# Intelligent-Microsystems-Lab/SNNQuantPrune

Measured on AMD Instinct MI355X. Metric: samples/sec/node (DVS128 T=20, 4-bit/90%-pruned), higher is better.
Workload: dtype fp6*fp4->f32 (integer-exact); 1 GPU; C3 topology: 3x(qconv3x3+BN+LIF+pool2) + qdense(32768->110)+LIF + vote, DVS128 128x128x2, T=20, bits 4/4/4/4, 90% pruned; batch_per_gpu=1024, global_batch=1024, frames=20, parallelism=dp1 (batch-sharded, all-gather logits)

## Files before the change

include/snnqp.h:

```cpp
#ifndef SNNQP_H_
#define SNNQP_H_

#include <stdint.h>

#ifdef __cplusplus
extern "C" {
#endif

typedef void *snnqp_stream_t;

enum {
  SNNQP_OK = 0,
  SNNQP_EINVAL = -1,
  SNNQP_EUNSUPPORTED = -2,
  SNNQP_EHIP = -3
};

enum { SNNQP_F32 = 0, SNNQP_U8 = 1, SNNQP_BITS = 2, SNNQP_EV1 = 3, SNNQP_EV4 = 4 };
enum { SNNQP_W_F32 = 0, SNNQP_W_I8 = 1 };
enum {
  SNNQP_NEURON_NONE = 0,
  SNNQP_NEURON_MULTI_STEP_LIF = 1,
  SNNQP_NEURON_PARAMETRIC_LEAKY_IF = 2,
  SNNQP_NEURON_LIF = 3
};
enum {
  SNNQP_SURR_FAST_SIGMOID = 0,
  SNNQP_SURR_ATAN = 1,
  SNNQP_SURR_SLAYER = 2,
  SNNQP_SURR_SMOOTH_STEP = 3,
  SNNQP_SURR_PIECEWISE_LINEAR = 4
};
enum {
  SNNQP_Q_DUQ = 0,
  SNNQP_Q_UNIFORM_STATIC = 1,
  SNNQP_Q_PARAMETRIC_D = 2,
  SNNQP_Q_PARAMETRIC_D_XMAX = 3
};
enum { SNNQP_IMPL_AUTO = 0, SNNQP_IMPL_GENERIC = 1, SNNQP_IMPL_MFMA = 2 };

enum {
  SNNQP_FLAG_CODE_OVERFLOW = 1,
  SNNQP_FLAG_MASK_NOT_BINARY = 2,
  SNNQP_FLAG_NOT_INTEGER = 4,
  SNNQP_FLAG_GT_ONE = 8,
  SNNQP_FLAG_GT_127 = 16,
  SNNQP_FLAG_GT_15 = 32
};

typedef struct {
  int32_t wtype;
  const void *w;
  float L;
  float m;
  int32_t abs_sum_max;
  int32_t code_max;
  const int32_t *col_sum;
  const void *wt_fp6;
  uint32_t min_current_bits;
  int32_t ch_stack_max;
  const int32_t *ch_slots;
  int32_t wt_cin;
} snnqp_weight_t;

#define SNNQP_BN_MEAN_ZERO 1
#define SNNQP_BN_BIAS_ZERO 2
#define SNNQP_BN_MUL_UNIFORM 4
typedef struct {
  const float *mean;
  const float *mul;
  const float *bias;
  int32_t flags;
} snnqp_bn_t;

typedef struct {
  int32_t kind;
  float k;
  float v_threshold;
  float v_reset;
  const float *decay;
} snnqp_neuron_t;

typedef struct {
  int32_t H, W, Cin, Cout;
  int32_t KH, KW;
  int32_t stride_h, stride_w;
  int32_t pad_h_lo, pad_h_hi, pad_w_lo, pad_w_hi;
  int32_t in_dil_h, in_dil_w;
  int32_t k_dil_h, k_dil_w;
  int32_t groups;
} snnqp_conv_geom_t;

typedef struct {
  int32_t D, H, W, Cin, Cout;
  int32_t KD, KH, KW;
  int32_t stride[3];
  int32_t pad_lo[3], pad_hi[3];
  int32_t in_dil[3];
  int32_t k_dil[3];
  int32_t groups;
} snnqp_conv3d_geom_t;

#define SNNQP_VERSION 505
int snnqp_version(void);
const char *snnqp_last_error(void);
const char *snnqp_build_flags(void);

int snnqp_conv_out_shape(const snnqp_conv_geom_t *g, int32_t *OH, int32_t *OW);

int snnqp_quantize(int kind, const float *w, const float *mask, int64_t n,
                   int bits, float p0, float p1, float *fq_out,
                   int8_t *codes_out, int32_t *flags, snnqp_stream_t stream);
int snnqp_quantize_ex(int kind, const float *w, const float *mask, int64_t n,
                      int bits, int sign, float p0, float p1, float *fq_out,
                      int8_t *codes_out, int32_t *flags, snnqp_stream_t stream);

int snnqp_pack_codes_mfma(const int8_t *w, int64_t K, int32_t N, int32_t Npad,
                          int8_t *wt, snnqp_stream_t stream);

int snnqp_pack_codes_fp6(const int8_t *w, int64_t K, int32_t N, int32_t Npad, void *wt6,
                         snnqp_stream_t stream);

int snnqp_inspect_f32(const float *x, int64_t n, int32_t *flags,
                      snnqp_stream_t stream);
int snnqp_inspect_u8(const uint8_t *x, int64_t n, int32_t *flags,
                     snnqp_stream_t stream);
int snnqp_f32_to_u8(const float *x, uint8_t *y, int64_t n,
                    snnqp_stream_t stream);
int snnqp_narrow_f32(const float *x, uint8_t *y, int64_t n, int32_t *flags,
                     snnqp_stream_t stream);
int snnqp_pack_frames(const uint8_t *x, int64_t frames, int32_t H, int32_t W, int fmt,
                      void *y, int32_t *flags, snnqp_stream_t stream);
int snnqp_unpack_frames(const void *x, int fmt, int64_t frames, int32_t H, int32_t W,
                        uint8_t *y, snnqp_stream_t stream);
int snnqp_pack_frames_checked(const void *x, int in_type, int64_t frames, int32_t H, int32_t W,
                              uint32_t *y, int32_t *flags, snnqp_stream_t stream);
int snnqp_pack_bits(const void *x, int in_type, int64_t rows, int32_t C,
                    uint32_t *bits, snnqp_stream_t stream);
int snnqp_pack_bits_checked(const void *x, int in_type, int64_t rows, int32_t C,
                            uint32_t *bits, int32_t *flags, snnqp_stream_t stream);
int snnqp_unpack_bits(const uint32_t *bits, int64_t rows, int32_t C, float *y,
                      snnqp_stream_t stream);

int snnqp_conv_forward(const void *x, int in_type, int64_t NB,
                       const snnqp_conv_geom_t *g, const snnqp_weight_t *w,
                       float *y, int32_t *acc, snnqp_stream_t stream);
int snnqp_conv_forward_if(const int32_t *pred, const void *x, int in_type, int64_t NB,
                          const snnqp_conv_geom_t *g, const snnqp_weight_t *w, float *y,
                          snnqp_stream_t stream);

int snnqp_conv3d_out_shape(const snnqp_conv3d_geom_t *g, int32_t *OD, int32_t *OH, int32_t *OW);
int snnqp_conv3d_lif_forward(const int32_t *pred, const void *x, int in_type, int64_t x_stride_t,
                             int64_t x_stride_b, int32_t T, int32_t B,
                             const snnqp_conv3d_geom_t *g, const snnqp_weight_t *w,
                             const snnqp_bn_t *bn, const snnqp_neuron_t *nrn, const float *u0,
                             float *u_out, void *s_out, int s_type, snnqp_stream_t stream);

int64_t snnqp_conv_gated_packed_bytes(int32_t Cin, int32_t Cout);
int snnqp_pack_codes_gated(const int8_t *w, int32_t Cin, int32_t Cout, void *packed,
                           snnqp_stream_t stream);
int64_t snnqp_conv_gated_packed_bytes_ex(int32_t Cin, int32_t Cout, int32_t code_max);
int snnqp_pack_codes_gated_ex(const int8_t *w, int32_t Cin, int32_t Cout, int32_t code_max,
                              void *packed, snnqp_stream_t stream);
int snnqp_conv_gated_forward(const uint32_t *s, const float *gate, int64_t NB,
                             const snnqp_conv_geom_t *g, const snnqp_weight_t *w,
                             const void *packed, float *y, snnqp_stream_t stream);

int64_t snnqp_dense_gated_packed_bytes(int32_t C, int32_t N);
int snnqp_pack_codes_dense_gated(const int8_t *w, int32_t C, int32_t HW, int32_t N, void *packed,
                                 snnqp_stream_t stream);
int64_t snnqp_dense_gated_packed_bytes_ex(int32_t C, int32_t N, int32_t code_max);
int snnqp_pack_codes_dense_gated_ex(const int8_t *w, int32_t C, int32_t HW, int32_t N, int32_t code_max,
                                    void *packed, snnqp_stream_t stream);
int snnqp_dense_gated_forward(const uint32_t *s, const float *gate, int64_t NB, int32_t HW,
                              int32_t C, int32_t N, const snnqp_weight_t *w,
                              const void *packed, float *y, snnqp_stream_t stream);

int snnqp_conv_lif_forward(const void *x, int in_type, int64_t x_stride_t,
                           int64_t x_stride_b, int32_t T, int32_t B,
                           const snnqp_conv_geom_t *g, const snnqp_weight_t *w,
                           const int8_t *wt, const snnqp_bn_t *bn,
                           const snnqp_neuron_t *nrn, const float *u0,
                           float *u_out, void *s_out, int s_type, int pool,
                           int impl, int x_max, int32_t *x_seen, int32_t *x_flags,
                           snnqp_stream_t stream);

int snnqp_conv_lif_forward_pred(const int32_t *pred, const void *x, int in_type, int64_t x_stride_t,
                                int64_t x_stride_b, int32_t T, int32_t B,
                                const snnqp_conv_geom_t *g, const snnqp_weight_t *w,
                                const int8_t *wt, const snnqp_bn_t *bn,
                                const snnqp_neuron_t *nrn, const float *u0,
                                float *u_out, void *s_out, int s_type, int pool,
                                int x_max, int32_t *x_seen, int32_t *x_flags,
                                snnqp_stream_t stream);

int snnqp_conv_lif_forward_if(const int32_t *pred, const void *x, int in_type, int64_t x_stride_t,
                              int64_t x_stride_b, int32_t T, int32_t B,
                              const snnqp_conv_geom_t *g, const snnqp_weight_t *w,
                              const snnqp_bn_t *bn, const snnqp_neuron_t *nrn, const float *u0,
                              float *u_out, void *s_out, int s_type, int pool,
                              snnqp_stream_t stream);

int snnqp_fallback_counts(int64_t *conv_blocks, int64_t *dense_blocks, char *reason,
                          int32_t reason_len, int reset);

#define SNNQP_STATUS_QUEUE_CORRUPT 1u
#define SNNQP_STATUS_TICKET 2u
#define SNNQP_STATUS_BOUND 4u
int snnqp_device_status(int device, uint32_t *codes, int reset);
int snnqp_workqueue_capture_mark(int device, int64_t *mark);
int snnqp_workqueue_capture_release(int device, int64_t mark_begin, int64_t mark_end);
int snnqp_workqueue_stats(int64_t *captured_static, int64_t *busy_static,
                          int64_t *dequant_fallbacks, int reset);
int snnqp_debug_workqueue_poke(int device, int64_t mark, int word, uint32_t value);

#define SNNQP_DQ_ARITH 1
#define SNNQP_DQ_ONE 2
#define SNNQP_DQ_TABLE 3
int snnqp_conv_dequant_form(const snnqp_weight_t *w, const snnqp_neuron_t *nrn);

int snnqp_current_min(const snnqp_weight_t *w, const snnqp_bn_t *bn, int32_t bound,
                      int32_t Cout, uint32_t *out_bits, snnqp_stream_t stream);

int snnqp_dense_lif_forward(const void *x, int in_type, int64_t x_stride_t,
                            int64_t x_stride_b, int32_t T, int32_t B, int32_t K,
                            int32_t N, const snnqp_weight_t *w,
                            const int8_t *wt, const snnqp_bn_t *bn,
                            const snnqp_neuron_t *nrn, const float *u0,
                            float *u_out, void *s_out, int s_type, int impl,
                            snnqp_stream_t stream);

int64_t snnqp_dense_workspace_bytes(int in_type, int32_t T, int32_t B, int32_t K, int32_t N,
                                    const snnqp_weight_t *w);
int snnqp_dense_lif_forward_ws(const void *x, int in_type, int64_t x_stride_t,
                               int64_t x_stride_b, int32_t T, int32_t B, int32_t K,
                               int32_t N, const snnqp_weight_t *w,
                               const int8_t *wt, const snnqp_bn_t *bn,
                               const snnqp_neuron_t *nrn, const float *u0,
                               float *u_out, void *s_out, int s_type, int impl,
                               int32_t *x_flags, void *ws, int64_t ws_bytes, snnqp_stream_t stream);
int snnqp_dense_lif_forward_if(const int32_t *pred, const void *x, int in_type, int64_t x_stride_t,
                               int64_t x_stride_b, int32_t T, int32_t B, int32_t K, int32_t N,
                               const snnqp_weight_t *w, const snnqp_bn_t *bn,
                               const snnqp_neuron_t *nrn, const float *u0, float *u_out,
                               void *s_out, int s_type, snnqp_stream_t stream);

int64_t snnqp_dense_head_workspace_bytes(int32_t T, int32_t B, int32_t N1);
int snnqp_dense_head_forward(const void *x, int in_type, int64_t x_stride_t,
                             int64_t x_stride_b, int32_t T, int32_t B, int32_t K,
                             int32_t N1, const snnqp_weight_t *w1, const int8_t *wt1,
                             const snnqp_neuron_t *nrn1, int32_t N2,
                             const snnqp_weight_t *w2, const int8_t *wt2,
                             const snnqp_neuron_t *nrn2, int32_t group,
                             uint32_t *s1_out, uint32_t *s2_out, float *logits,
                             int32_t *x_flags, void *ws, int64_t ws_bytes, snnqp_stream_t stream);

int snnqp_lif_forward(const float *x, int32_t T, int64_t R, int32_t C,
                      const snnqp_bn_t *bn, const snnqp_neuron_t *nrn,
                      const float *u0, float *u_out, void *s_out, int s_type,
                      snnqp_stream_t stream);

int snnqp_batchnorm_forward(const float *x, int64_t rows, int32_t C,
                            const snnqp_bn_t *bn, float *y,
                            snnqp_stream_t stream);

int snnqp_maxpool2x2(const void *x, int type, int64_t NB, int32_t H, int32_t W,
                     int32_t C, void *y, snnqp_stream_t stream);

int snnqp_spatial_mean(const void *x, int type, int64_t NB, int32_t HW, int32_t C,
                       float *y, snnqp_stream_t stream);
int snnqp_sigmoid_gate(const float *a, const float *b, int64_t n, float *g,
                       snnqp_stream_t stream);
int snnqp_apply_gate(const void *x, int type, const float *g, int64_t NB, int32_t HW,
                     int32_t C, float *y, snnqp_stream_t stream);

int snnqp_events_to_frames(const int32_t *ex, const int32_t *ey, const int32_t *ep,
                           int64_t N, int32_t T, int32_t H, int32_t W, float scale,
                           int32_t *counts, uint8_t *frames_u8, snnqp_stream_t stream);
int snnqp_density(const void *x, int type, int64_t NB, int64_t n, int32_t C, int32_t *nnz,
                  snnqp_stream_t stream);

int snnqp_vote(const void *s, int type, int32_t T, int32_t B, int32_t N,
               int32_t group, float *logits, snnqp_stream_t stream);
int snnqp_vote_if(const int32_t *pred, const void *s, int type, int32_t T, int32_t B, int32_t N,
                  int32_t group, float *logits, snnqp_stream_t stream);

int snnqp_scatter_spike_channels(const uint32_t *s, int64_t npix, int32_t cin, const int32_t *map,
                                 int32_t cout, uint32_t *out, snnqp_stream_t stream);

int snnqp_lif_forward_save(const float *x, int32_t T, int64_t R, int32_t C,
                           const snnqp_neuron_t *nrn, float *h_out, float *s_out,
                           snnqp_stream_t stream);
int snnqp_lif_backward(const float *h, const float *gs, const float *glogits, int32_t group,
                       int32_t T, int64_t R, int32_t C, const snnqp_neuron_t *nrn,
                       int surrogate, float *gI, snnqp_stream_t stream);
int snnqp_dense_weight_grad(const float *x, const float *gI, int64_t M, int32_t K, int32_t N,
                            float *gw, snnqp_stream_t stream);
int snnqp_dense_input_grad(const float *gI, const float *w, const float *mask, int64_t M,
                           int32_t K, int32_t N, float *gx, snnqp_stream_t stream);

#ifdef __cplusplus
}
#endif
#endif
```

snnquantprune_amd/_lib.py:

```python

from __future__ import annotations

import ctypes
import os
from ctypes import (POINTER, Structure, c_char_p, c_float, c_int, c_int8,
                    c_int32, c_uint32, c_int64, c_void_p)

_HERE = os.path.dirname(os.path.abspath(__file__))
LIB_PATH = os.path.join(_HERE, "csrc", "libsnnqp.so")

ABI_VERSION = 505

F32, U8, BITS, EV1, EV4 = 0, 1, 2, 3, 4
W_F32, W_I8 = 0, 1
NEURON_NONE, NEURON_MULTI_STEP_LIF, NEURON_PARAMETRIC_LEAKY_IF, NEURON_LIF = 0, 1, 2, 3
SURR_FAST_SIGMOID, SURR_ATAN, SURR_SLAYER, SURR_SMOOTH_STEP, SURR_PIECEWISE_LINEAR = 0, 1, 2, 3, 4
Q_DUQ, Q_UNIFORM_STATIC, Q_PARAMETRIC_D, Q_PARAMETRIC_D_XMAX = 0, 1, 2, 3
IMPL_AUTO, IMPL_GENERIC, IMPL_MFMA = 0, 1, 2
FLAG_CODE_OVERFLOW, FLAG_MASK_NOT_BINARY = 1, 2
FLAG_NOT_INTEGER, FLAG_GT_ONE, FLAG_GT_127, FLAG_GT_15 = 4, 8, 16, 32
OK, EINVAL, EUNSUPPORTED, EHIP = 0, -1, -2, -3
STATUS_QUEUE_CORRUPT, STATUS_TICKET, STATUS_BOUND = 1, 2, 4


class WeightT(Structure):
  _fields_ = [("wtype", c_int32), ("w", c_void_p), ("L", c_float), ("m", c_float),
              ("abs_sum_max", c_int32), ("code_max", c_int32), ("col_sum", c_void_p),
              ("wt_fp6", c_void_p), ("min_current_bits", c_uint32), ("ch_stack_max", c_int32),
              ("ch_slots", c_void_p), ("wt_cin", c_int32)]


BN_MEAN_ZERO, BN_BIAS_ZERO, BN_MUL_UNIFORM = 1, 2, 4


class BnT(Structure):
  _fields_ = [("mean", c_void_p), ("mul", c_void_p), ("bias", c_void_p), ("flags", c_int32)]


class NeuronT(Structure):
  _fields_ = [("kind", c_int32), ("k", c_float), ("v_threshold", c_float),
              ("v_reset", c_float), ("decay", c_void_p)]


class ConvGeomT(Structure):
  _fields_ = [(n, c_int32) for n in (
      "H", "W", "Cin", "Cout", "KH", "KW", "stride_h", "stride_w",
      "pad_h_lo", "pad_h_hi", "pad_w_lo", "pad_w_hi",
      "in_dil_h", "in_dil_w", "k_dil_h", "k_dil_w", "groups")]


class Conv3dGeomT(Structure):
  _fields_ = ([(n, c_int32) for n in ("D", "H", "W", "Cin", "Cout", "KD", "KH", "KW")]
              + [(n, c_int32 * 3) for n in ("stride", "pad_lo", "pad_hi", "in_dil", "k_dil")]
              + [("groups", c_int32)])


_PROTOTYPES = {
    "snnqp_version": (c_int, []),
    "snnqp_last_error": (c_char_p, []),
    "snnqp_build_flags": (c_char_p, []),
    "snnqp_conv_out_shape": (c_int, [POINTER(ConvGeomT), POINTER(c_int32),
                                     POINTER(c_int32)]),
    "snnqp_quantize": (c_int, [c_int, c_void_p, c_void_p, c_int64, c_int, c_float,
                               c_float, c_void_p, c_void_p, c_void_p, c_void_p]),
    "snnqp_quantize_ex": (c_int, [c_int, c_void_p, c_void_p, c_int64, c_int, c_int, c_float,
                                  c_float, c_void_p, c_void_p, c_void_p, c_void_p]),
    "snnqp_pack_codes_mfma": (c_int, [c_void_p, c_int64, c_int32, c_int32, c_void_p,
                                      c_void_p]),
    "snnqp_pack_codes_fp6": (c_int, [c_void_p, c_int64, c_int32, c_int32, c_void_p, c_void_p]),
    "snnqp_inspect_f32": (c_int, [c_void_p, c_int64, c_void_p, c_void_p]),
    "snnqp_inspect_u8": (c_int, [c_void_p, c_int64, c_void_p, c_void_p]),
    "snnqp_f32_to_u8": (c_int, [c_void_p, c_void_p, c_int64, c_void_p]),
    "snnqp_narrow_f32": (c_int, [c_void_p, c_void_p, c_int64, c_void_p, c_void_p]),
    "snnqp_pack_frames": (c_int, [c_void_p, c_int64, c_int32, c_int32, c_int, c_void_p, c_void_p,
                                  c_void_p]),
    "snnqp_unpack_frames": (c_int, [c_void_p, c_int, c_int64, c_int32, c_int32, c_void_p,
                                    c_void_p]),
    "snnqp_pack_bits": (c_int, [c_void_p, c_int, c_int64, c_int32, c_void_p,
                                c_void_p]),
    "snnqp_pack_bits_checked": (c_int, [c_void_p, c_int, c_int64, c_int32, c_void_p, c_void_p,
                                        c_void_p]),
    "snnqp_unpack_bits": (c_int, [c_void_p, c_int64, c_int32, c_void_p, c_void_p]),
    "snnqp_conv_forward": (c_int, [c_void_p, c_int, c_int64, POINTER(ConvGeomT),
                                   POINTER(WeightT), c_void_p, c_void_p, c_void_p]),
    "snnqp_conv_forward_if": (c_int, [c_void_p, c_void_p, c_int, c_int64, POINTER(ConvGeomT),
                                      POINTER(WeightT), c_void_p, c_void_p]),
    "snnqp_conv3d_out_shape": (c_int, [POINTER(Conv3dGeomT), POINTER(c_int32), POINTER(c_int32),
                                       POINTER(c_int32)]),
    "snnqp_conv3d_lif_forward": (c_int, [
        c_void_p, c_void_p, c_int, c_int64, c_int64, c_int32, c_int32, POINTER(Conv3dGeomT),
        POINTER(WeightT), POINTER(BnT), POINTER(NeuronT), c_void_p, c_void_p, c_void_p, c_int, c_void_p]),
    "snnqp_conv_gated_packed_bytes": (c_int64, [c_int32, c_int32]),
    "snnqp_pack_codes_gated": (c_int, [c_void_p, c_int32, c_int32, c_void_p, c_void_p]),
    "snnqp_conv_gated_packed_bytes_ex": (c_int64, [c_int32, c_int32, c_int32]),
    "snnqp_pack_codes_gated_ex": (c_int, [c_void_p, c_int32, c_int32, c_int32, c_void_p, c_void_p]),
    "snnqp_conv_gated_forward": (c_int, [c_void_p, c_void_p, c_int64, POINTER(ConvGeomT),
                                         POINTER(WeightT), c_void_p, c_void_p, c_void_p]),
    "snnqp_dense_gated_packed_bytes": (c_int64, [c_int32, c_int32]),
    "snnqp_pack_codes_dense_gated": (c_int, [c_void_p, c_int32, c_int32, c_int32, c_void_p, c_void_p]),
    "snnqp_dense_gated_packed_bytes_ex": (c_int64, [c_int32, c_int32, c_int32]),
    "snnqp_pack_codes_dense_gated_ex": (c_int, [c_void_p, c_int32, c_int32, c_int32, c_int32, c_void_p, c_void_p]),
    "snnqp_dense_gated_forward": (c_int, [c_void_p, c_void_p, c_int64, c_int32, c_int32, c_int32,
                                          POINTER(WeightT), c_void_p, c_void_p, c_void_p]),
    "snnqp_conv_lif_forward": (c_int, [
        c_void_p, c_int, c_int64, c_int64, c_int32, c_int32, POINTER(ConvGeomT),
        POINTER(WeightT), c_void_p, POINTER(BnT), POINTER(NeuronT), c_void_p,
        c_void_p, c_void_p, c_int, c_int, c_int, c_int, c_void_p, c_void_p, c_void_p]),
    "snnqp_conv_lif_forward_pred": (c_int, [
        c_void_p, c_void_p, c_int, c_int64, c_int64, c_int32, c_int32, POINTER(ConvGeomT),
        POINTER(WeightT), c_void_p, POINTER(BnT), POINTER(NeuronT), c_void_p,
        c_void_p, c_void_p, c_int, c_int, c_int, c_void_p, c_void_p, c_void_p]),
    "snnqp_pack_frames_checked": (c_int, [c_void_p, c_int, c_int64, c_int32, c_int32, c_void_p, c_void_p,
                                          c_void_p]),
    "snnqp_conv_lif_forward_if": (c_int, [
        c_void_p, c_void_p, c_int, c_int64, c_int64, c_int32, c_int32, POINTER(ConvGeomT),
        POINTER(WeightT), POINTER(BnT), POINTER(NeuronT), c_void_p, c_void_p, c_void_p, c_int, c_int,
        c_void_p]),
    "snnqp_dense_lif_forward_if": (c_int, [
        c_void_p, c_void_p, c_int, c_int64, c_int64, c_int32, c_int32, c_int32, c_int32,
        POINTER(WeightT), POINTER(BnT), POINTER(NeuronT), c_void_p, c_void_p, c_void_p, c_int,
        c_void_p]),
    "snnqp_dense_lif_forward": (c_int, [
        c_void_p, c_int, c_int64, c_int64, c_int32, c_int32, c_int32, c_int32,
        POINTER(WeightT), c_void_p, POINTER(BnT), POINTER(NeuronT), c_void_p,
        c_void_p, c_void_p, c_int, c_int, c_void_p]),
    "snnqp_dense_workspace_bytes": (c_int64, [c_int, c_int32, c_int32, c_int32, c_int32, POINTER(WeightT)]),
    "snnqp_dense_lif_forward_ws": (c_int, [
        c_void_p, c_int, c_int64, c_int64, c_int32, c_int32, c_int32, c_int32,
        POINTER(WeightT), c_void_p, POINTER(BnT), POINTER(NeuronT), c_void_p,
        c_void_p, c_void_p, c_int, c_int, c_void_p, c_void_p, c_int64, c_void_p]),
    "snnqp_dense_head_workspace_bytes": (c_int64, [c_int32, c_int32, c_int32]),
    "snnqp_dense_head_forward": (c_int, [
        c_void_p, c_int, c_int64, c_int64, c_int32, c_int32, c_int32, c_int32, POINTER(WeightT),
        c_void_p, POINTER(NeuronT), c_int32, POINTER(WeightT), c_void_p, POINTER(NeuronT), c_int32,
        c_void_p, c_void_p, c_void_p, c_void_p, c_void_p, c_int64, c_void_p]),
    "snnqp_device_status": (c_int, [c_int, POINTER(c_uint32), c_int]),
    "snnqp_workqueue_capture_mark": (c_int, [c_int, POINTER(c_int64)]),
    "snnqp_workqueue_capture_release": (c_int, [c_int, c_int64, c_int64]),
    "snnqp_workqueue_stats": (c_int, [POINTER(c_int64), POINTER(c_int64), POINTER(c_int64), c_int]),
    "snnqp_debug_workqueue_poke": (c_int, [c_int, c_int64, c_int, c_uint32]),
    "snnqp_fallback_counts": (c_int, [POINTER(c_int64), POINTER(c_int64), c_char_p, c_int32, c_int]),
    "snnqp_conv_dequant_form": (c_int, [POINTER(WeightT), POINTER(NeuronT)]),
    "snnqp_current_min": (c_int, [POINTER(WeightT), POINTER(BnT), c_int32, c_int32, c_void_p, c_void_p]),
    "snnqp_lif_forward": (c_int, [c_void_p, c_int32, c_int64, c_int32, POINTER(BnT),
                                  POINTER(NeuronT), c_void_p, c_void_p, c_void_p,
                                  c_int, c_void_p]),
    "snnqp_batchnorm_forward": (c_int, [c_void_p, c_int64, c_int32, POINTER(BnT),
                                        c_void_p, c_void_p]),
    "snnqp_maxpool2x2": (c_int, [c_void_p, c_int, c_int64, c_int32, c_int32, c_int32,
                                 c_void_p, c_void_p]),
    "snnqp_spatial_mean": (c_int, [c_void_p, c_int, c_int64, c_int32, c_int32, c_void_p,
                                   c_void_p]),
    "snnqp_sigmoid_gate": (c_int, [c_void_p, c_void_p, c_int64, c_void_p, c_void_p]),
    "snnqp_apply_gate": (c_int, [c_void_p, c_int, c_void_p, c_int64, c_int32, c_int32,
                                 c_void_p, c_void_p]),
    "snnqp_events_to_frames": (c_int, [c_void_p, c_void_p, c_void_p, c_int64, c_int32, c_int32,
                                       c_int32, c_float, c_void_p, c_void_p, c_void_p]),
    "snnqp_density": (c_int, [c_void_p, c_int, c_int64, c_int64, c_int32, c_void_p, c_void_p]),
    "snnqp_vote": (c_int, [c_void_p, c_int, c_int32, c_int32, c_int32, c_int32,
                           c_void_p, c_void_p]),
    "snnqp_vote_if": (c_int, [c_void_p, c_void_p, c_int, c_int32, c_int32, c_int32, c_int32,
                              c_void_p, c_void_p]),
    "snnqp_scatter_spike_channels": (c_int, [c_void_p, c_int64, c_int32, c_void_p, c_int32,
                                             c_void_p, c_void_p]),
    "snnqp_lif_forward_save": (c_int, [c_void_p, c_int32, c_int64, c_int32, POINTER(NeuronT),
                                       c_void_p, c_void_p, c_void_p]),
    "snnqp_lif_backward": (c_int, [c_void_p, c_void_p, c_void_p, c_int32, c_int32, c_int64,
                                   c_int32, POINTER(NeuronT), c_int, c_void_p, c_void_p]),
    "snnqp_dense_weight_grad": (c_int, [c_void_p, c_void_p, c_int64, c_int32, c_int32, c_void_p,
                                        c_void_p]),
    "snnqp_dense_input_grad": (c_int, [c_void_p, c_void_p, c_void_p, c_int64, c_int32, c_int32,
                                       c_void_p, c_void_p]),
}

EXPORTED_SYMBOLS = tuple(_PROTOTYPES)

_lib = None


class SnnqpError(RuntimeError):
  def __init__(self, code, msg):
    super().__init__("libsnnqp error %d: %s" % (code, msg))
    self.code = code


def lib():
  global _lib
  if _lib is None:
    path = os.environ.get("SNNQP_DIAG_LIB") or LIB_PATH
    if not os.path.exists(path):
      raise ImportError(
          "HIP extension %s not found: build it with `python __graft_entry__.py` "
          "(hipcc --offload-arch=gfx950); there is no CPU fallback." % path)
    import torch
    handle = ctypes.CDLL(path)
    if path != LIB_PATH:
      import sys
      print("snnquantprune_amd: DIAGNOSTIC library %s" % path, file=sys.stderr)
    for name, (res, args) in _PROTOTYPES.items():
      fn = getattr(handle, name)
      fn.restype = res
      fn.argtypes = args
    if handle.snnqp_version() != ABI_VERSION:
      raise ImportError(
          "%s has ABI version %d, this binding was written against %d (include/snnqp.h "
          "SNNQP_VERSION): rebuild it with `python __graft_entry__.py`"
          % (path, handle.snnqp_version(), ABI_VERSION))
    _lib = handle
  return _lib


def build_flags() -> str:
  return lib().snnqp_build_flags().decode("utf-8", "replace")


def require_product_build():
  flags = build_flags()
  if flags or os.environ.get("SNNQP_DIAG_LIB"):
    raise RuntimeError("libsnnqp is a diagnostic build (%s): rebuild with "
                       "`python snnquantprune_amd/csrc/build.py --force`" % (flags or "SNNQP_DIAG_LIB"))


def check(rc):
  if rc != 0:
    raise SnnqpError(rc, lib().snnqp_last_error().decode("utf-8", "replace"))
```

snnquantprune_amd/csrc/conv3x3_u8c2.hip:

```cpp
#include <atomic>
#include <map>
#include <mutex>
#include <tuple>
#include <type_traits>
#include <utility>

#include <vector>

#include "conv_tile.h"

namespace snnqp {

constexpr int HROW2 = 24;
constexpr int HCOPY2 = HALO * HROW2;
constexpr int HCONST2 = 2 * HCOPY2;
constexpr int HIMG2 = 496;
constexpr int TCHUNK = 32;
constexpr int U8C2_WPS = 4;
constexpr int STG_N = TCHUNK / 2;

typedef int v2i_a4 __attribute__((ext_vector_type(2), aligned(4)));
typedef __attribute__((address_space(3))) const v2i_a4 lds_cv2i_t;

__host__ __device__ inline int u8c2_table_bytes(int lutm, int bound, int rows) {
  const int b = lutm == LUT_CHANNEL ? rows * 128 : lutm == LUT_SHARED ? (2 * bound + 2) * 4 : 0;
  return (b + 15) & ~15;
}

#ifndef SNNQP_U8C2_EV1_WPS
#define SNNQP_U8C2_EV1_WPS 5
#endif
#ifndef SNNQP_U8C2_ONE_WPS
#define SNNQP_U8C2_ONE_WPS 4
#endif
#ifndef SNNQP_U8C2_EV1_ONE_WPS
#define SNNQP_U8C2_EV1_ONE_WPS 6
#endif
template <int NF, bool POOL, int LUTM, int IN, bool ONE>
constexpr int u8c2_waves() {
  if (IN == SNNQP_EV1 && ONE && LUTM == LUT_CHANNEL && NF == NF_MUL0 && POOL) return SNNQP_U8C2_EV1_ONE_WPS;
  if (IN == SNNQP_EV1) return SNNQP_U8C2_EV1_WPS;
  return ONE ? SNNQP_U8C2_ONE_WPS : U8C2_WPS;
}
template <int NF, bool POOL, int LUTM, int IN = SNNQP_U8, bool ONE = false>
__global__ void __launch_bounds__(256, (u8c2_waves<NF, POOL, LUTM, IN, ONE>()))
conv3x3_u8c2_kernel(ConvMfmaArgs a) {
  constexpr int FL = OutStage<POOL>::FL;
  constexpr bool EV1 = IN == SNNQP_EV1;
  constexpr bool EV4 = IN == SNNQP_EV4;
  constexpr bool F32IN = IN == SNNQP_F32;
  static_assert(TCHUNK % FL == 0, "flush period must divide the staging chunk");
  if constexpr (!EV1) {
    if (a.pred && *(const volatile int32_t *)a.pred == 0) return;
  }
  extern __shared__ __attribute__((aligned(16))) uint8_t lds[];
  const int tc = a.tchunk;
  const int lut_off = tc * HIMG2;
  uint32_t *obuf = (uint32_t *)(lds + lut_off + u8c2_table_bytes(LUTM, a.lut_bound, a.lut_rows));
  const int tid = threadIdx.x, lane = tid & 63;
  const int wave = __builtin_amdgcn_readfirstlane(tid >> 6);
  const int n = lane & 31, h = lane >> 5;
  const int cout_base = blockIdx.y * 128 + wave * 32;
  const bool wave_on = cout_base < a.Cout;
  const int cout = wave_on ? cout_base + n : n;
  const int cpar = cout < a.Cout ? cout : a.Cout - 1;
  const uint32_t cmask = chan_mask(cout_base, a.Cout);
  uint32_t *wgw = obuf + OutStage<POOL>::BYTES / 4;
  if (tid == 0) { wgw[0] = 0x7F800000u; wgw[1] = 0u; }
  typedef int v2i_a8 __attribute__((ext_vector_type(2)));
  v2i_a8 *xtab = (v2i_a8 *)(wgw + 4);
  if (EV1) {
    const uint32_t one = LUTM == LUT_CHANNEL ? 16u : LUTM == LUT_SHARED ? 4u : 0x81u;
    const uint32_t zero = LUTM == LUT_NONE ? 0x80u : 0u;
    uint32_t e[2] = {0, 0};
#pragma unroll
    for (int j = 0; j < 8; ++j) e[j >> 2] |= (((uint32_t)tid >> j) & 1u ? one : zero) << (8 * (j & 3));
    xtab[tid] = v2i_a8{(int)e[0], (int)e[1]};
  }
  if (LUTM != LUT_NONE) lds_barrier();
  if (LUTM == LUT_SHARED) {
    build_lut((float *)(lds + lut_off), a.lut_bound, a.dq, tid);
    if (NF == NF_MUL0) {
      lds_barrier();
      atomicMin(wgw, lut_bn_min_bits((const float *)(lds + lut_off), a.lut_bound, a.bn,
                                     blockIdx.y * 128, a.Cout, tid, 256));
    }
  }
  int ch_row0 = 0, ch_col = 0;
  if (LUTM == LUT_CHANNEL) {
    int pos = 0, neg = 0;
#pragma unroll
    for (int j = 0; j < 16; ++j) {
      const int k = 16 * h + j, dy = k >> 3, b = k & 7;
      if (k < 24 && b < 6 && wave_on && cout < a.Cout) {
        const int code = a.w[(int64_t)(6 * dy + b) * a.Cout + cout];
        pos += code > 0 ? code : 0;
        neg += code < 0 ? -code : 0;
      }
    }
    pos += __shfl_xor(pos, 32);
    neg += __shfl_xor(neg, 32);
    uint32_t *scr = obuf;
    int slot = 4 * n + wave;
    if (a.ch_slots) slot = a.ch_slots[blockIdx.y * 128 + wave * 32 + n] & 127;
    if (h == 0) {
      scr[slot] = (uint32_t)((pos + neg) * a.x_limit + 1);
      scr[128 + wave * 32 + n] = (uint32_t)(neg * a.x_limit);
      scr[256 + wave * 32 + n] = (uint32_t)slot;
    }
    lds_barrier();
    ch_col = slot >> 2;
    const int start = lut_column_start(scr, slot);
    int total = 0;
#pragma unroll
    for (int k = 0; k < 4; ++k) total += (int)scr[(slot & ~3) + k];
    ch_row0 = start + neg * a.x_limit;
    if (total > a.lut_rows && a.status) *(volatile uint32_t *)a.status = SNNQP_STATUS_BOUND;
    const uint32_t mb = build_lut_channel((float *)(lds + lut_off), scr, a.lut_rows, a.dq, a.bn,
                                          blockIdx.y * 128, a.Cout, tid);
    atomicMin(wgw, mb);
    lds_barrier();
  }
  if (tid < tc) {
    *(uint32_t *)(lds + tid * HIMG2 + HCONST2) = 0x7F7F7F7Fu;
    *(uint32_t *)(lds + tid * HIMG2 + HCONST2 + 4) = 0x00000001u;
  }

  float acc_off = 0.0f;
  v4i bf, bfg;
  {
    int bias = 0;
    if (LUTM == LUT_SHARED) bias = (int)lds_addr(lds) + lut_off + 4 * a.lut_bound;
    if (LUTM == LUT_CHANNEL)
      bias = (int)lds_addr(lds) + lut_off + 4 * (ch_row0 * 32 + ch_col);
    int q = bias / 127;
    const int r = bias - 127 * q;
    int wsum = 0;
    int v[4], vg[4];
#pragma unroll
    for (int d = 0; d < 4; ++d) {
      uint32_t pk = 0, pkg = 0;
#pragma unroll
      for (int j = 0; j < 4; ++j) {
        const int k = 16 * h + 4 * d + j;
        uint32_t bv = 0, bg = 0;
        if (k < 24) {
          const int dy = k >> 3, b = k & 7;
          if (b < 6 && cout < a.Cout) {
            const int code = a.w[(int64_t)(6 * dy + b) * a.Cout + cout];
            wsum += code;
            bg = (uint8_t)code;
            bv = (uint8_t)(LUTM == LUT_CHANNEL ? code * 8 : code);
          }
        } else if (k < 28) {
          const int part = q < 127 ? q : 127;
          q -= part;
          bv = (uint32_t)part;
        } else if (k == 28) {
          bv = (uint32_t)r;
        }
        pk |= bv << (8 * j);
        pkg |= bg << (8 * j);
      }
      v[d] = (int)pk;
      vg[d] = (int)pkg;
    }
    bf = v4i{v[0], v[1], v[2], v[3]};
    bfg = v4i{vg[0], vg[1], vg[2], vg[3]};
    acc_off = 128.0f * (float)(wsum + __shfl_xor(wsum, 32));
  }

  LaneConsts lc = {0.f, 1.f, 0.f, 0.f, a.nrn.vr};
  if (a.bn.mean) { lc.bmean = a.bn.mean[cpar]; lc.bmul = a.bn.mul[cpar]; lc.bbias = a.bn.bias[cpar]; }
  if (a.nrn.kind == SNNQP_NEURON_LIF) lc.dec = a.nrn.decay[cpar];

  const int ty = ((n >> 2) & 1) | ((n >> 4) << 1);
  const int tx = (n & 3) | (((n >> 3) & 1) << 2);
  const int cpy = tx & 1;
  const int px0 = (int)lds_addr(lds) + cpy * HCOPY2 + 2 * tx + 2 * cpy;
  int offA[2], offB[2];
#pragma unroll
  for (int tl = 0; tl < 2; ++tl) {
    offA[tl] = px0 + (ty + 4 * tl + (h ? 2 : 0)) * HROW2;
    offB[tl] = h ? (int)lds_addr(lds) + HCONST2 : px0 + (ty + 4 * tl + 1) * HROW2;
  }
  const uint8_t *xb = (const uint8_t *)a.x;
  const int ob0 = out_pix<POOL>(0, lane) * 4 + wave;
  const int ob1 = out_pix<POOL>(1, lane) * 4 + wave;
  const bool store_lane = POOL ? lane < 8 : lane < 32;
  uint32_t seen = 0;
  uint32_t hist[6] = {0, 0, 0, 0, 0, 0};
  const int s_pix = tid & 127;
  const bool s_task = s_pix < HALO * HALO;
  const int s_half = __builtin_amdgcn_readfirstlane(tid >> 7);
  const int s_dst = (s_pix / HALO) * HROW2 + (s_pix % HALO) * 2;

  PatchWalk pw(a);
  int r = __builtin_amdgcn_readfirstlane((int)pw.first);
  uint32_t processed = 0;
  while (r < (int)pw.count) {
    ++processed;
    int claimed = 0;
    if (pw.queue && tid == 0) claimed = (int)pw.claim();
    int b, y0, x0;
    pw.decode(a, r, b, y0, x0);

    float u[2][16];
    if constexpr (!ONE) {
      if (a.u0 && wave_on) u_io<true>(u, a, b, y0, x0, cout, h);
      else zero_u(u);
    }
    uint32_t pseen = 0;
    const int s_gy = y0 + s_pix / HALO - 1, s_gx = x0 + s_pix % HALO - 1;
    const bool s_valid = s_task && s_gy >= 0 && s_gy < a.H && s_gx >= 0 && s_gx < a.W;
    const uint32_t s_off = s_valid ? (uint32_t)(s_gy * a.W + s_gx) * (EV4 ? 1u : F32IN ? 8u : 2u) : 0u;
    const uint8_t *s_frames = xb + (int64_t)b * a.xs_b * (F32IN ? 4 : 1);
    const uint32_t e_lead = x0 > 0 ? 2u : 0u;
    const int e_hi = min(HALO - 1, a.W - x0);
    const uint32_t e_colmask = ((1u << (2 * (e_hi + 1))) - 1u) & ~((1u << (2 - (int)e_lead)) - 1u);
    const uint32_t e_fwords = (uint32_t)(((int64_t)a.H * a.W * 2 + 31) >> 5);
    const uint32_t *e_frames = (const uint32_t *)a.x + (int64_t)b * a.xs_b;

    for (int t0 = 0; t0 < a.T; t0 += tc) {
      const int nt = min(tc, a.T - t0);
      bool general = LUTM == LUT_NONE;
      if constexpr (EV1) {
        lds_barrier();
        for (int task = tid; task < nt * HALO; task += 256) {
          const int tt = task / HALO, hy = task - tt * HALO;
          const int gy = y0 + hy - 1;
          const bool rv = gy >= 0 && gy < a.H;
          const uint32_t start = (uint32_t)((rv ? gy : 0) * a.W + x0) * 2u - e_lead;
          const uint32_t wi = start >> 5;
          const uint32_t *f = e_frames + (int64_t)(t0 + tt) * a.xs_t;
          const uint32_t lo = f[wi], hi = f[min(wi + 1u, e_fwords - 1u)];
          uint32_t v = __builtin_amdgcn_alignbit(hi, lo, start & 31u);
          v = (v << (2u - e_lead)) & (rv ? e_colmask : 0u);
          const v2i_a8 d0 = xtab[v & 0xFFu], d1 = xtab[(v >> 8) & 0xFFu], d2 = xtab[(v >> 16) & 0xFu];
          uint8_t *row = lds + tt * HIMG2 + hy * HROW2;
          *(v2i_a8 *)row = d0;
          *(v2i_a8 *)(row + 8) = d1;
          *(v2i_a8 *)(row + 16) = d2;
          const uint32_t q0 = (uint32_t)d0.x, q1 = (uint32_t)d0.y, q2 = (uint32_t)d1.x,
                         q3 = (uint32_t)d1.y, q4 = (uint32_t)d2.x, q5 = (uint32_t)d2.y;
          uint8_t *row1 = row + HCOPY2;
          *(v2i_a8 *)row1 = v2i_a8{(int)(q0 << 16), (int)__builtin_amdgcn_alignbit(q1, q0, 16)};
          *(v2i_a8 *)(row1 + 8) = v2i_a8{(int)__builtin_amdgcn_alignbit(q2, q1, 16),
                                         (int)__builtin_amdgcn_alignbit(q3, q2, 16)};
          *(v2i_a8 *)(row1 + 16) = v2i_a8{(int)__builtin_amdgcn_alignbit(q4, q3, 16),
                                          (int)__builtin_amdgcn_alignbit(q5, q4, 16)};
        }
        lds_barrier();
      } else {
      uint32_t v[STG_N];
      uint32_t mx = 0;
      if constexpr (F32IN) {
        uint32_t fbad = 0;
#pragma unroll
        for (int r0 = 0; r0 < STG_N; r0 += STG_N / 2) {
          typedef float f2v __attribute__((ext_vector_type(2)));
          f2v raw[STG_N / 2];
#pragma unroll
          for (int i = r0; i < r0 + STG_N / 2; ++i) {
            const int tt = 2 * i + s_half;
            raw[i - r0] = f2v{0.0f, 0.0f};
            if (tt < nt) raw[i - r0] = *(const f2v *)(s_frames + (int64_t)(t0 + tt) * a.xs_t * 4 + s_off);
          }
#pragma unroll
          for (int i = r0; i < r0 + STG_N / 2; ++i) {
            const f2v f = raw[i - r0];
            const uint32_t ua = __float2uint_rz(f.x), ub = __float2uint_rz(f.y);
            fbad |= __float_as_uint(__uint2float_rn(ua) - f.x) | __float_as_uint(__uint2float_rn(ub) - f.y);
            fbad |= (ua | ub) >> 8;
            v[i] = (ua & 0xFFu) | ((ub & 0xFFu) << 8);
          }
        }
        fbad = s_valid ? fbad : 0u;
        if (__ballot(fbad != 0u) != 0ull && lane == 0 && a.x_flags) atomicOr(a.x_flags, SNNQP_FLAG_NOT_INTEGER);
      } else {
#pragma unroll
      for (int i = 0; i < STG_N; ++i) {
        const int tt = 2 * i + s_half;
        v[i] = 0;
        if (tt < nt) {
          if constexpr (EV4) {
            const uint32_t pb = *(s_frames + (int64_t)(t0 + tt) * a.xs_t + s_off);
            v[i] = (pb | (pb << 4)) & 0x0F0Fu;
          } else {
            v[i] = *(const uint16_t *)(s_frames + (int64_t)(t0 + tt) * a.xs_t + s_off);
          }
        }
      }
      }
#pragma unroll
      for (int i = 0; i < STG_N; ++i) {
        v[i] = s_valid ? v[i] : 0u;
        mx = max(mx, max(v[i] & 0xFFu, v[i] >> 8));
      }
#pragma unroll
      for (int off = 32; off > 0; off >>= 1) mx = max(mx, (uint32_t)__shfl_xor((int)mx, off));
      if (tid == 0) wgw[1] = 0u;
      lds_barrier();
      if (s_task) {
#pragma unroll
        for (int i = 0; i < STG_N; ++i) {
          const int tt = 2 * i + s_half;
          if (tt < nt) {
            const uint16_t val = (uint16_t)(LUTM == LUT_NONE      ? v[i] ^ 0x8080u
                                            : LUTM == LUT_CHANNEL ? v[i] << 4
                                                                  : v[i] << 2);
            uint8_t *p = lds + tt * HIMG2 + s_dst;
            *(uint16_t *)p = val;
            *(uint16_t *)(p + HCOPY2 + 2) = val;
          }
        }
      }
      if (lane == 0 && mx != 0) atomicMax(&wgw[1], mx);
      lds_barrier();
      const uint32_t cmax = (uint32_t)__builtin_amdgcn_readfirstlane((int)wgw[1]);
      seen = max(seen, cmax);
      pseen = max(pseen, cmax);
      hist[0] += cmax <= 1u;
      hist[1] += cmax == 2u;
      hist[2] += cmax > 2u && cmax <= 7u;
      hist[3] += cmax > 7u && cmax <= 31u;
      hist[4] += cmax > 31u;
      hist[5] += cmax == 3u;
      general = LUTM == LUT_NONE || cmax > (uint32_t)a.x_limit;
      if (LUTM != LUT_NONE && general) {
        if (s_task) {
#pragma unroll 1
          for (int tt = s_half; tt < nt; tt += 2) {
            uint32_t w2 = 0;
            if (s_valid) {
              if constexpr (F32IN) {
                typedef float f2v __attribute__((ext_vector_type(2)));
                const f2v f = *(const f2v *)(s_frames + (int64_t)(t0 + tt) * a.xs_t * 4 + s_off);
                w2 = (__float2uint_rz(f.x) & 0xFFu) | ((__float2uint_rz(f.y) & 0xFFu) << 8);
              } else if constexpr (EV4) {
                const uint32_t pb = *(s_frames + (int64_t)(t0 + tt) * a.xs_t + s_off);
                w2 = (pb | (pb << 4)) & 0x0F0Fu;
              } else {
                w2 = *(const uint16_t *)(s_frames + (int64_t)(t0 + tt) * a.xs_t + s_off);
              }
            }
            const uint16_t val = (uint16_t)(w2 ^ 0x8080u);
            uint8_t *p = lds + tt * HIMG2 + s_dst;
            *(uint16_t *)p = val;
            *(uint16_t *)(p + HCOPY2 + 2) = val;
          }
        }
        lds_barrier();
      }
      }
      auto run_chunk = [&](auto mode_tag, auto fma_tag) {
      constexpr int MODE = decltype(mode_tag)::value;
      constexpr bool FMA = decltype(fma_tag)::value;
      constexpr bool OFFS = MODE == LUT_NONE;
      const v4i bw = OFFS ? bfg : bf;
      for (int tf = 0; tf < nt; tf += FL) {
        const int nf = min(FL, nt - tf);
#pragma unroll 1
        for (int tt = tf; tt < (wave_on ? tf + nf : tf); ++tt) {
          const uint32_t img = (uint32_t)(tt * HIMG2);
          uint32_t words[2];
#pragma unroll
          for (int tl = 0; tl < 2; ++tl) {
            const v2i_a4 lo = *(lds_cv2i_t *)(uintptr_t)(img + (uint32_t)offA[0] + (uint32_t)(tl * 4 * HROW2));
            const v2i_a4 hi = *(lds_cv2i_t *)(uintptr_t)(img + (uint32_t)offB[tl]);
            v16i acc = splat16(0);
            acc = __builtin_amdgcn_mfma_i32_32x32x32_i8(v4i{lo.x, lo.y, hi.x, hi.y}, bw, acc,
                                                        0, 0, 0);
            if constexpr (u8c2_waves<NF, POOL, LUTM, IN, ONE>() >= 6)
              words[tl] = tile_epilogue_halves<NF, POOL, MODE, FMA, OFFS>(acc, u[tl], a.dq, lc, a.nrn,
                                                                            lane, acc_off);
            else
              words[tl] = tile_epilogue<NF, POOL, MODE, FMA, OFFS>(acc, u[tl], a.dq, lc, a.nrn,
                                                                     lane, acc_off);
          }
          if (store_lane) {
            uint32_t *o = obuf + ((t0 + tt) % FL) * (OutStage<POOL>::NPIX * 4);
            o[ob0] = words[0] & cmask;
            o[ob0 + (POOL ? 32 : 128)] = words[1] & cmask;
          }
        }
        lds_barrier();
        flush_out<POOL>(obuf, a, t0 + tf, nf, b, y0, x0, tid);
        lds_barrier();
      }
      };
      if constexpr (ONE) zero_u(u);
      if (general) {
        run_chunk(std::integral_constant<int, LUT_NONE>{}, std::false_type{});
      } else if constexpr (LUTM != LUT_NONE) {
        const bool fma_ok = NF == NF_MUL0 && pseen <= (uint32_t)a.x_limit &&
                            lif_fma_is_exact(wgw[0], a.nrn.k_log2, a.T, a.u0 != nullptr);
        if (fma_ok) run_chunk(std::integral_constant<int, LUTM>{}, std::true_type{});
        else run_chunk(std::integral_constant<int, LUTM>{}, std::false_type{});
      }
      if constexpr (ONE) break;
    }
    if (!ONE && a.u_out && wave_on) u_io<false>(u, a, b, y0, x0, cout, h);
    int r_next = r + (int)pw.stride;
    if (pw.queue) {
      if (tid == 0) wgw[2] = (uint32_t)claimed;
      lds_barrier();
      r_next = __builtin_amdgcn_readfirstlane((int)wgw[2]);
    }
    r = r_next;
  }
  if (a.x_seen && tid == 0) {
    if (seen != 0) atomicMax(a.x_seen, seen);
#pragma unroll
    for (int k = 0; k < 6; ++k)
      if (hist[k] != 0) atomicAdd((uint32_t *)a.x_seen + 1 + k, hist[k]);
  }
  if (pw.queue && tid == 0) pw.finish(processed, a.npatch, a.status);
}


__global__ void __launch_bounds__(256)
current_min_kernel(Dequant dq, BnP bn, int bound, int Cout, uint32_t *out) {
  const int c = blockIdx.x * 64 + (threadIdx.x & 63);
  uint32_t mb = 0x7F800000u;
  if (c < Cout) {
    float mean = 0.f, mul = 1.f, bias = 0.f;
    if (bn.mean) { mean = bn.mean[c]; mul = bn.mul[c]; bias = bn.bias[c]; }
    for (int i = (int)(threadIdx.x >> 6) + 4 * (int)blockIdx.y - bound; i <= bound; i += 4 * (int)gridDim.y) {
      float x = dequant_acc_nb(i, dq) - mean;
      x = x * mul;
      x = x + bias;
      const uint32_t b = __float_as_uint(x) & 0x7FFFFFFFu;
      if (b != 0 && b < mb) mb = b;
    }
  }
  for (int off = 32; off > 0; off >>= 1) {
    const uint32_t o = (uint32_t)__shfl_xor((int)mb, off);
    mb = o < mb ? o : mb;
  }
  if ((threadIdx.x & 63) == 0 && mb != 0x7F800000u) atomicMin(out, mb);
}

namespace {
struct SchedPool {
  uint32_t *words = nullptr;
  hipEvent_t busy[SCHED_SLOTS] = {};
  bool has_event[SCHED_SLOTS] = {};
  bool retired[SCHED_SLOTS] = {};
  unsigned next = 0;
  unsigned next_capture = 0;
  std::vector<int> capture_log;
  std::vector<int> capture_free;
};
std::atomic<int64_t> g_static_captured{0}, g_static_busy{0};
std::mutex g_sched_mu;
SchedPool g_sched[64];

struct DeviceGuard {
  int prev = -1;
  bool ok = true;
  explicit DeviceGuard(int dev) {
    int cur = -1;
    if (hipGetDevice(&cur) != hipSuccess) { (void)hipGetLastError(); ok = false; return; }
    if (cur == dev) return;
    if (hipSetDevice(dev) != hipSuccess) { (void)hipGetLastError(); ok = false; return; }
    prev = cur;
  }
  ~DeviceGuard() {
    if (prev >= 0 && hipSetDevice(prev) != hipSuccess) (void)hipGetLastError();
  }
};
}

uint32_t *sched_acquire(hipStream_t st, int *dev_out, int *slot_out) {
  int dev = 0;
  hipStreamCaptureStatus cap = hipStreamCaptureStatusNone;
  if (hipStreamIsCapturing(st, &cap) != hipSuccess) { (void)hipGetLastError(); return nullptr; }
  const bool capturing = cap != hipStreamCaptureStatusNone;
  hipDevice_t sdev;
  if (hipStreamGetDevice(st, &sdev) == hipSuccess) dev = (int)sdev;
  else if (hipGetDevice(&dev) != hipSuccess) return nullptr;
  if (dev < 0 || dev >= 64) return nullptr;
  std::lock_guard<std::mutex> lock(g_sched_mu);
  SchedPool &p = g_sched[dev];
  if (capturing) {
    if (!p.words) { g_static_captured.fetch_add(1, std::memory_order_relaxed); return nullptr; }
    int slot;
    if (!p.capture_free.empty()) {
      slot = p.capture_free.back();
      p.capture_free.pop_back();
    } else if (p.next_capture < (unsigned)SCHED_CAPTURE_SLOTS) {
      slot = SCHED_SLOTS + (int)p.next_capture++;
    } else {
      g_static_captured.fetch_add(1, std::memory_order_relaxed);
      return nullptr;
    }
    p.capture_log.push_back(slot);
    *dev_out = dev;
    *slot_out = slot;
    return p.words + (size_t)slot * SCHED_WORDS;
  }
  if (!p.words) {
    DeviceGuard on(dev);
    if (!on.ok) return nullptr;
    uint32_t *w = nullptr;
    if (hipMalloc((void **)&w, (size_t)(SCHED_SLOTS + SCHED_CAPTURE_SLOTS) * SCHED_WORDS *
                                   sizeof(uint32_t)) != hipSuccess) {
      (void)hipGetLastError();
      return nullptr;
    }
    if (hipMemset(w, 0, (size_t)(SCHED_SLOTS + SCHED_CAPTURE_SLOTS) * SCHED_WORDS * sizeof(uint32_t)) !=
        hipSuccess) {
      (void)hipGetLastError();
      (void)hipFree(w);
      return nullptr;
    }
    p.words = w;
  }
  const int slot = (int)(p.next++ % SCHED_SLOTS);
  if (p.retired[slot]) return nullptr;
  if (!p.has_event[slot]) {
    DeviceGuard on(dev);
    if (!on.ok || hipEventCreateWithFlags(&p.busy[slot], hipEventDisableTiming) != hipSuccess) {
      (void)hipGetLastError();
      p.retired[slot] = true;
      return nullptr;
    }
    p.has_event[slot] = true;
  } else if (hipEventQuery(p.busy[slot]) != hipSuccess) {
    (void)hipGetLastError();
    g_static_busy.fetch_add(1, std::memory_order_relaxed);
    return nullptr;
  }
  uint32_t *words = p.words + (size_t)slot * SCHED_WORDS;
  if (hipMemsetAsync(words, 0, SCHED_WORDS * sizeof(uint32_t), st) != hipSuccess) {
    (void)hipGetLastError();
    return nullptr;
  }
  *dev_out = dev;
  *slot_out = slot;
  return words;
}

void sched_release(int dev, int slot, hipStream_t st) {
  if (slot >= SCHED_SLOTS) return;
  std::lock_guard<std::mutex> lock(g_sched_mu);
  SchedPool &p = g_sched[dev];
  if (hipEventRecord(p.busy[slot], st) != hipSuccess) {
    (void)hipGetLastError();
    p.retired[slot] = true;
  }
}

int stream_device(hipStream_t st) {
  int dev = 0;
  hipDevice_t sdev;
  if (hipStreamGetDevice(st, &sdev) == hipSuccess) return (int)sdev;
  (void)hipGetLastError();
  if (hipGetDevice(&dev) != hipSuccess) { (void)hipGetLastError(); dev = 0; }
  return dev;
}

void persistent_limits(const void *kernel, int threads, size_t dyn_lds, int dev, int *cus_out,
                       int *occ_out) {
  typedef std::tuple<const void *, int, size_t, int> Key;
  static std::mutex mu;
  static std::map<Key, std::pair<int, int>> cache;
  const Key key(kernel, threads, dyn_lds, dev);
  std::lock_guard<std::mutex> lock(mu);
  auto it = cache.find(key);
  if (it == cache.end()) {
    int cus = 256, occ = 1;
    DeviceGuard on(dev);
    if (hipDeviceGetAttribute(&cus, hipDeviceAttributeMultiprocessorCount, dev) != hipSuccess) {
      (void)hipGetLastError();
      cus = 256;
    }
    if (hipOccupancyMaxActiveBlocksPerMultiprocessor(&occ, kernel, threads, dyn_lds) != hipSuccess) {
      (void)hipGetLastError();
      occ = 1;
    }
    if (occ < 1) occ = 1;
    if (occ > 8) occ = 8;
    it = cache.emplace(key, std::make_pair(cus, occ)).first;
  }
  *cus_out = it->second.first;
  *occ_out = it->second.second;
}

int run_current_min(const snnqp_weight_t *w, const snnqp_bn_t *bn, int32_t bound, int32_t Cout,
                    uint32_t *out_bits, hipStream_t st) {
  SNNQP_REQUIRE(w && out_bits && Cout > 0 && bound >= 0, SNNQP_EINVAL, "current_min: bad argument");
  SNNQP_REQUIRE(w->L >= 1.0f, SNNQP_EINVAL, "dequant L must be >= 1");
  SNNQP_CHECK_BN(bn);
  const int slices = bound >= 256 ? 16 : 1;
  hipLaunchKernelGGL(current_min_kernel, dim3((Cout + 63) / 64, slices), dim3(256), 0, st,
                     make_dequant(w->L, w->m), make_bn(bn), bound, Cout, out_bits);
  SNNQP_CHECK_LAUNCH("current_min_kernel");
  return SNNQP_OK;
}

const char *conv3x3_mfma_unsupported(int in_type, const snnqp_conv_geom_t *g,
                                     const snnqp_weight_t *w, const int8_t *wt,
                                     const snnqp_neuron_t *nrn, int s_type) {
  if (w->wtype != SNNQP_W_I8) return "weights are not int8 codes";
  if (g->KH != 3 || g->KW != 3) return "kernel is not 3x3";
  if (g->stride_h != 1 || g->stride_w != 1) return "stride is not 1";
  if (g->pad_h_lo != 1 || g->pad_h_hi != 1 || g->pad_w_lo != 1 || g->pad_w_hi != 1)
    return "padding is not ((1,1),(1,1))";
  if (g->in_dil_h != 1 || g->in_dil_w != 1 || g->k_dil_h != 1 || g->k_dil_w != 1)
    return "dilated convolution";
  if (g->groups != 1) return "grouped convolution";
  if (g->H <= 0 || g->W <= 0) return "empty image";
  if (g->Cout <= 0) return "no output channels";
  if (s_type != SNNQP_BITS) return "spike output must be bit-packed";
  if (in_type == SNNQP_BITS) {
    if (g->Cin < 1 || g->Cin > 128) return "bit input needs Cin <= 128";
  } else if (in_type == SNNQP_U8) {
    if (g->Cin != 2) return "u8 input needs Cin == 2";
    if ((int64_t)g->H * g->W * 2 >= (int64_t)1 << 31) return "u8 frame of 2 GiB or more";
  } else if (in_type == SNNQP_EV1) {
    if (g->Cin != 2) return "EV1 frames have Cin == 2";
    if ((int64_t)g->H * g->W * 2 >= (int64_t)1 << 31) return "EV1 frame of 2^31 bits or more";
  } else if (in_type == SNNQP_EV4) {
    if (g->Cin != 2) return "EV4 frames have Cin == 2";
    if ((int64_t)g->H * g->W >= (int64_t)1 << 31) return "EV4 frame of 2 GiB or more";
  } else if (in_type == SNNQP_F32) {
    if (g->Cin != 2) return "float32 input into integer codes needs Cin == 2";
    if ((int64_t)g->H * g->W * 8 >= (int64_t)1 << 31) return "float32 frame of 2 GiB or more";
  } else {
    return "input must be BITS, U8, EV1, EV4 or (Cin == 2) F32";
  }
  if (nrn->kind == SNNQP_NEURON_LIF && !nrn->decay) return "LIF without decay";
  if (in_type == SNNQP_BITS && !wt) return "MFMA-tiled codes `wt` not given";
  return nullptr;
}

int conv3x3_bits_dequant_form(const snnqp_weight_t *w, const snnqp_neuron_t *nrn) {
  if (w->L == 1.0f) return DQ_ONE;
  const bool fp6 = w->code_max > 0 && w->code_max <= 7;
  const bool tab = fp6 && neuron_form(make_neuron(nrn)) == NF_MUL0 && w->abs_sum_max > 0 &&
                   w->abs_sum_max <= DQT_MAXA;
  return tab ? DQ_TABLE : DQ_ARITH;
}

int run_conv3x3_mfma(const void *x, int in_type, int64_t xs_t, int64_t xs_b,
                     int32_t T, int32_t B, const snnqp_conv_geom_t *g,
                     const snnqp_weight_t *w, const int8_t *wt,
                     const snnqp_bn_t *bn, const snnqp_neuron_t *nrn,
                     const float *u0, float *u_out, uint32_t *s_out, int pool,
                     int x_max, int32_t *x_seen, int32_t *x_flags, hipStream_t st, const int32_t *pred) {
  SNNQP_REQUIRE(w->w && ((x && s_out) || T == 0 || B == 0), SNNQP_EINVAL, "conv3x3 mfma: null pointer");
  SNNQP_REQUIRE(!pred || in_type == SNNQP_U8 || in_type == SNNQP_F32 || in_type == SNNQP_EV4, SNNQP_EUNSUPPORTED,
                "conv3x3 mfma: only the event layer on byte / nibble / float32 frames takes a predicate");
  SNNQP_REQUIRE(in_type != SNNQP_BITS || wt, SNNQP_EINVAL,
                "conv3x3 mfma: bit input needs the MFMA-tiled codes `wt`");
  const int cin_pad = w->wt_cin ? w->wt_cin : (g->Cin + 31) / 32 * 32;
  SNNQP_REQUIRE(in_type != SNNQP_BITS || (cin_pad % 32 == 0 && cin_pad >= g->Cin && cin_pad <= 128),
                SNNQP_EINVAL, "conv3x3 mfma: wt_cin must be a multiple of 32 in [Cin, 128]");
  SNNQP_REQUIRE(T >= 0 && B >= 0, SNNQP_EINVAL, "conv3x3 mfma: negative T/B");
  SNNQP_REQUIRE(w->L >= 1.0f, SNNQP_EINVAL, "dequant L must be >= 1");
  SNNQP_CHECK_BN(bn);
  if (T == 0 || B == 0) return SNNQP_OK;
  SNNQP_REQUIRE((int64_t)B * ((g->H + 3) / 4) * ((g->W + 7) / 8) < ((int64_t)1 << 30),
                SNNQP_EUNSUPPORTED, "conv3x3 mfma: more than 2^30 patches in one launch");
  ConvMfmaArgs a;
  a.x = x; a.xs_t = xs_t; a.xs_b = xs_b; a.T = T; a.B = B;
  a.H = g->H; a.W = g->W; a.Cin = g->Cin; a.Cout = g->Cout;
  a.w = (const int8_t *)w->w;
  a.wt = wt;
  a.dq = make_dequant(w->L, w->m);
  a.bn = make_bn(bn);
  a.nrn = make_neuron(nrn);
  a.u0 = u0; a.u_out = u_out; a.s_out = s_out; a.pool = pool;
  a.x_seen = x_seen;
  a.x_flags = nullptr;
  a.pred = pred;
  if (in_type == SNNQP_F32) {
    SNNQP_REQUIRE(x_flags != nullptr && (((uintptr_t)x) & 7) == 0 && xs_t % 2 == 0 && xs_b % 2 == 0,
                  SNNQP_EINVAL, "conv3x3 mfma: float32 frames need x_flags and 8-byte aligned pixels");
    if (int rc = zero_words_async((uint32_t *)x_flags, 1, st)) return rc;
    a.x_flags = x_flags;
  }
  a.patch_h = 8;
  a.tiles_y = (g->H + 7) / 8; a.tiles_x = (g->W + 7) / 8;
  a.npatch = (int64_t)B * a.tiles_y * a.tiles_x;
  const int nf = neuron_form(a.nrn);
  const bool pl = pool == 2;
  const unsigned gy = (unsigned)((g->Cout + 127) / 128);
  const bool ev1 = in_type == SNNQP_EV1;
  const int64_t xm = (in_type == SNNQP_BITS || ev1) ? 1 : (x_max > 0 ? x_max : 1);
  a.x_limit = (int32_t)(xm > 255 ? 255 : xm);
  const int64_t bound = (int64_t)w->abs_sum_max * xm;
  const bool lut = w->abs_sum_max > 0 && xm > 0 && xm <= LUT_XMAX && bound <= LUT_CAP;
  a.lut_bound = lut ? (int32_t)bound : 0;
  a.tchunk = T >= TCHUNK ? TCHUNK : T;
  const size_t lds_fixed = (size_t)a.tchunk * HIMG2 + 16 + (ev1 ? 2048 : 0) +
                           (pl ? OutStage<true>::BYTES : OutStage<false>::BYTES);
  const int64_t stack = w->ch_stack_max > 0 ? (int64_t)w->ch_stack_max : 8 * (int64_t)w->abs_sum_max;
  const int64_t crows = stack * xm + 4;
  const bool lutc = lut && in_type != SNNQP_BITS && crows <= LUT2_ROWS && xm <= 7 &&
                    w->code_max > 0 && w->code_max <= 15;
  a.lut_rows = lutc ? (int32_t)crows : 0;
  a.ch_slots = lutc && w->ch_stack_max > 0 ? w->ch_slots : nullptr;
#define SNNQP_CONV_LAUNCH_IN(KERN, NFV, PL, LM, LDS)                               \
  do {                                                                             \
    if (ev1 && one) launch_persistent(KERN<NFV, PL, LM, SNNQP_EV1, true>, a, gy, st, LDS); \
    else if (ev1) launch_persistent(KERN<NFV, PL, LM, SNNQP_EV1>, a, gy, st, LDS);       \
    else if (in_type == SNNQP_EV4 && one) launch_persistent(KERN<NFV, PL, LM, SNNQP_EV4, true>, a, gy, st, LDS); \
    else if (in_type == SNNQP_EV4) launch_persistent(KERN<NFV, PL, LM, SNNQP_EV4>, a, gy, st, LDS); \
    else if (in_type == SNNQP_F32 && one) launch_persistent(KERN<NFV, PL, LM, SNNQP_F32, true>, a, gy, st, LDS); \
    else if (in_type == SNNQP_F32) launch_persistent(KERN<NFV, PL, LM, SNNQP_F32>, a, gy, st, LDS); \
    else if (one) launch_persistent(KERN<NFV, PL, LM, SNNQP_U8, true>, a, gy, st, LDS);            \
    else launch_persistent(KERN<NFV, PL, LM, SNNQP_U8>, a, gy, st, LDS);            \
  } while (0)
#define SNNQP_CONV_LAUNCH_NF(KERN, NFV, LM, LDS)                                   \
  do {                                                                             \
    if (pl) SNNQP_CONV_LAUNCH_IN(KERN, NFV, true, LM, LDS);                         \
    else SNNQP_CONV_LAUNCH_IN(KERN, NFV, false, LM, LDS);                           \
  } while (0)
#define SNNQP_CONV_LAUNCH(KERN, LM, LDS)                                           \
  do {                                                                             \
    if (nf == NF_MUL0) SNNQP_CONV_LAUNCH_NF(KERN, NF_MUL0, LM, LDS);                \
    else if (nf == NF_MUL) SNNQP_CONV_LAUNCH_NF(KERN, NF_MUL, LM, LDS);             \
    else if (nf == NF_DIV) SNNQP_CONV_LAUNCH_NF(KERN, NF_DIV, LM, LDS);             \
    else SNNQP_CONV_LAUNCH_NF(KERN, NF_DECAY, LM, LDS);                             \
  } while (0)
  if (in_type == SNNQP_BITS) {
    const bool fma = nf == NF_MUL0 && w->min_current_bits != 0 && w->abs_sum_max > 0 &&
                     lif_fma_is_exact(w->min_current_bits, a.nrn.k_log2, T, u0 != nullptr);
    const bool i8 = !(w->code_max > 0 && w->code_max <= 7);
    int dq = conv3x3_bits_dequant_form(w, nrn);
    if (dq == DQ_TABLE && !dq_table_trusted(stream_device(st), st)) dq = DQ_ARITH;
    const bool tab = dq == DQ_TABLE;
    const bool bnf = (a.bn.flags & (SNNQP_BN_MEAN_ZERO | SNNQP_BN_BIAS_ZERO)) ==
                     (SNNQP_BN_MEAN_ZERO | SNNQP_BN_BIAS_ZERO);
    a.lut_bound = tab ? (int32_t)w->abs_sum_max : 0;
    if (tab) check_code_bound_once(stream_device(st), (const int8_t *)w->w, (int64_t)9 * g->Cin, g->Cout,
                                   w->abs_sum_max, st);
    launch_conv3x3_bits(a, cin_pad, i8, nf, pl, dq, fma, bnf, gy, st);
  } else {
    const int lm = lutc ? LUT_CHANNEL : lut ? LUT_SHARED : LUT_NONE;
    if (lut) check_code_bound_once(stream_device(st), (const int8_t *)w->w, (int64_t)9 * g->Cin, g->Cout,
                                   w->abs_sum_max, st);
    const size_t lds_rest = lds_fixed - (size_t)a.tchunk * HIMG2 + u8c2_table_bytes(lm, a.lut_bound, a.lut_rows);
    for (int wgs = 4; wgs >= 2; --wgs) {
      const size_t per_wg = (size_t)(160 * 1024) / wgs - 512;
      int tc = a.tchunk;
      while (tc > 16 && (size_t)tc * HIMG2 + lds_rest > per_wg) tc -= 1;
      if ((size_t)tc * HIMG2 + lds_rest <= per_wg) {
        a.tchunk = tc;
        break;
      }
    }
    const size_t ldsb = (size_t)a.tchunk * HIMG2 + lds_rest;
    const bool one = !a.u0 && !a.u_out && a.T <= a.tchunk;
    if (lutc) SNNQP_CONV_LAUNCH(conv3x3_u8c2_kernel, LUT_CHANNEL, ldsb);
    else if (lut) SNNQP_CONV_LAUNCH(conv3x3_u8c2_kernel, LUT_SHARED, ldsb);
    else SNNQP_CONV_LAUNCH(conv3x3_u8c2_kernel, LUT_NONE, ldsb);
  }
#undef SNNQP_CONV_LAUNCH
#undef SNNQP_CONV_LAUNCH_NF
#undef SNNQP_CONV_LAUNCH_IN
  SNNQP_CHECK_LAUNCH("conv3x3 mfma kernel");
  return SNNQP_OK;
}

}

extern "C" int snnqp_workqueue_capture_mark(int device, int64_t *mark) {
  using namespace snnqp;
  SNNQP_REQUIRE(device >= 0 && device < 64 && mark, SNNQP_EINVAL, "workqueue_capture_mark: bad argument");
  std::lock_guard<std::mutex> lock(g_sched_mu);
  *mark = (int64_t)g_sched[device].capture_log.size();
  return SNNQP_OK;
}

extern "C" int snnqp_workqueue_capture_release(int device, int64_t mark_begin, int64_t mark_end) {
  using namespace snnqp;
  SNNQP_REQUIRE(device >= 0 && device < 64, SNNQP_EINVAL, "workqueue_capture_release: bad device");
  std::lock_guard<std::mutex> lock(g_sched_mu);
  SchedPool &p = g_sched[device];
  SNNQP_REQUIRE(0 <= mark_begin && mark_begin <= mark_end && mark_end <= (int64_t)p.capture_log.size(),
                SNNQP_EINVAL, "workqueue_capture_release: marks out of range");
  for (int64_t i = mark_begin; i < mark_end; ++i) {
    const int slot = p.capture_log[(size_t)i];
    if (slot < 0) continue;
    p.capture_free.push_back(slot);
    p.capture_log[(size_t)i] = -1;
  }
  return SNNQP_OK;
}

extern "C" int snnqp_workqueue_stats(int64_t *captured_static, int64_t *busy_static,
                                     int64_t *dequant_fallbacks, int reset) {
  using namespace snnqp;
  if (captured_static) *captured_static = g_static_captured.load(std::memory_order_relaxed);
  if (busy_static) *busy_static = g_static_busy.load(std::memory_order_relaxed);
  if (dequant_fallbacks) *dequant_fallbacks = dq_table_fallbacks(reset != 0);
  if (reset) { g_static_captured = 0; g_static_busy = 0; }
  return SNNQP_OK;
}

extern "C" int snnqp_debug_workqueue_poke(int device, int64_t mark, int word, uint32_t value) {
  using namespace snnqp;
  SNNQP_REQUIRE(device >= 0 && device < 64 && word >= 0 && word < SCHED_WORDS, SNNQP_EINVAL,
                "debug_workqueue_poke: bad argument");
  std::lock_guard<std::mutex> lock(g_sched_mu);
  SchedPool &p = g_sched[device];
  SNNQP_REQUIRE(p.words && mark >= 0 && mark < (int64_t)p.capture_log.size() && p.capture_log[(size_t)mark] >= 0,
                SNNQP_EINVAL, "debug_workqueue_poke: no live capture slot at mark %lld", (long long)mark);
  SNNQP_HIP(hipMemcpy(p.words + (size_t)p.capture_log[(size_t)mark] * SCHED_WORDS + word, &value, 4,
                      hipMemcpyHostToDevice));
  return SNNQP_OK;
}
```

snnquantprune_amd/csrc/conv_tile.h:

```cpp
#pragma once
#include "kernels.h"

namespace snnqp {


typedef int v4i __attribute__((ext_vector_type(4)));
typedef int v16i __attribute__((ext_vector_type(16)));
struct v2f {
  float x, y;
};
__device__ __forceinline__ v2f operator+(v2f a, v2f b) { return v2f{a.x + b.x, a.y + b.y}; }
__device__ __forceinline__ v2f operator-(v2f a, v2f b) { return v2f{a.x - b.x, a.y - b.y}; }
__device__ __forceinline__ v2f operator*(v2f a, v2f b) { return v2f{a.x * b.x, a.y * b.y}; }
__device__ __forceinline__ v2f operator+(v2f a, float b) { return v2f{a.x + b, a.y + b}; }
__device__ __forceinline__ v2f operator-(v2f a, float b) { return v2f{a.x - b, a.y - b}; }
__device__ __forceinline__ v2f operator*(v2f a, float b) { return v2f{a.x * b, a.y * b}; }
__device__ __forceinline__ v2f operator-(v2f a) { return v2f{-a.x, -a.y}; }
__device__ __forceinline__ v2f fma2(v2f a, v2f b, v2f c) {
  return v2f{__builtin_fmaf(a.x, b.x, c.x), __builtin_fmaf(a.y, b.y, c.y)};
}


enum { LUT_NONE = 0, LUT_SHARED = 1, LUT_CHANNEL = 2 };
constexpr int LUT_CAP = 4095;
constexpr int LUT2_ROWS = 256;
constexpr int LUT_XMAX = 31;

constexpr int HALO = 10;
constexpr int HPITCH = 12;
constexpr int HPLANE = HALO * HPITCH * 32;

struct ConvMfmaArgs {
  const void *x;
  int64_t xs_t, xs_b;
  int32_t T, B, H, W, Cin, Cout;
  const int8_t *w;
  const int8_t *wt;
  Dequant dq;
  BnP bn;
  NeuronP nrn;
  const float *u0;
  float *u_out;
  uint32_t *s_out;
  int32_t pool;
  int32_t tiles_y, tiles_x;
  int64_t npatch;
  int32_t lut_bound;
  int32_t lut_rows;
  const int32_t *ch_slots;
  int32_t x_limit;
  int32_t *x_seen;
  int32_t *x_flags;
  int32_t xcd_split;
  int32_t tchunk;
  uint32_t *sched;
  uint32_t *status;
  int32_t patch_h;
  const int32_t *pred;
};

constexpr int SCHED_Y = 8;
constexpr int SCHED_WORDS = SCHED_Y * 16;
constexpr int SCHED_SLOTS = 64;
constexpr int SCHED_CAPTURE_SLOTS = 960;

template <bool X4>
__device__ __forceinline__ v4i expand16(uint32_t b) {
  constexpr uint32_t MUL = X4 ? 0x00810204u : 0x00204081u;
  constexpr uint32_t AND = X4 ? 0x04040404u : 0x01010101u;
  v4i o;
  o.x = (int)((((b >> 0) & 0xFu) * MUL) & AND);
  o.y = (int)((((b >> 4) & 0xFu) * MUL) & AND);
  o.z = (int)((((b >> 8) & 0xFu) * MUL) & AND);
  o.w = (int)((((b >> 12) & 0xFu) * MUL) & AND);
  return o;
}

struct PatchWalk {
  int64_t first, count, stride;
  int ppb, xcd;
  bool split;
  uint32_t *queue;
  uint32_t *done;
  __device__ __forceinline__ explicit PatchWalk(const ConvMfmaArgs &a) {
    ppb = a.tiles_y * a.tiles_x;
    split = a.xcd_split != 0;
    if (split) {
      xcd = blockIdx.x & 7;
      first = blockIdx.x >> 3;
      stride = gridDim.x >> 3;
      count = (int64_t)((a.B - xcd + 7) >> 3) * ppb;
    } else {
      xcd = 0;
      first = blockIdx.x;
      stride = gridDim.x;
      count = a.npatch;
    }
    queue = a.sched ? a.sched + blockIdx.y * 16 + xcd : nullptr;
    done = a.sched ? a.sched + blockIdx.y * 16 + 8 : nullptr;
  }
  __device__ __forceinline__ int64_t claim() const {
    const int64_t r = stride + (int64_t)atomicAdd(queue, 1u);
    return r < count ? r : count;
  }
  __device__ __forceinline__ void finish(uint32_t processed, int64_t npatch, uint32_t *status) const {
    atomicAdd(done + 1, processed);
    __threadfence();
    const uint32_t total = gridDim.x;
    if (atomicAdd(done, 1u) + 1u == total) {
      __threadfence();
      const uint32_t tally = atomicAdd(done + 1, 0u);
      if (tally != (uint32_t)npatch && status) *(volatile uint32_t *)status = SNNQP_STATUS_QUEUE_CORRUPT;
      for (int i = 0; i < 8; ++i) done[i - 8] = 0u;
      done[1] = 0u;
      __threadfence();
      *done = 0u;
    }
  }
  __device__ __forceinline__ void decode(const ConvMfmaArgs &a, int64_t r, int &b, int &y0,
                                         int &x0) const {
    const int within = (int)(r % ppb);
    const int bi = (int)(r / ppb);
    b = split ? xcd + 8 * bi : bi;
    y0 = (within / a.tiles_x) * a.patch_h;
    x0 = (within % a.tiles_x) * 8;
  }
};

__device__ __forceinline__ void lds_barrier() {
  __builtin_amdgcn_fence(__ATOMIC_RELEASE, "workgroup", "local");
  __builtin_amdgcn_s_barrier();
  __builtin_amdgcn_fence(__ATOMIC_ACQUIRE, "workgroup", "local");
}

extern "C" __device__ uint32_t snnqp_writelane_i32(uint32_t, uint32_t, uint32_t)
    __asm("llvm.amdgcn.writelane.i32");
__device__ __forceinline__ uint32_t writelane_u32(uint32_t val, int lane, uint32_t old) {
  return snnqp_writelane_i32(val, (uint32_t)lane, old);
}

__device__ __forceinline__ float reset_where(float u, unsigned long long mask) {
  float r;
  asm("v_cndmask_b32_e64 %0, %1, 0, %2" : "=v"(r) : "v"(u), "s"(mask));
  return r;
}

struct LaneConsts {
  float bmean, bmul, bbias, dec;
  float vr;
};

__device__ __forceinline__ uint32_t chan_mask(int cout_base, int Cout) {
  const int valid = Cout - cout_base;
  return valid >= 32 ? 0xFFFFFFFFu : valid <= 0 ? 0u : (1u << valid) - 1u;
}

enum { NF_MUL0 = 1, NF_MUL = 2, NF_DIV = 3, NF_DECAY = 4 };

__host__ inline int neuron_form(const NeuronP &n) {
  if (n.kind == SNNQP_NEURON_LIF) return NF_DECAY;
  if (n.inv_k == 0.0f) return NF_DIV;
  return n.vr == 0.0f ? NF_MUL0 : NF_MUL;
}

typedef __attribute__((address_space(3))) const float lds_cfloat_t;
typedef __attribute__((address_space(3))) const uint8_t lds_cu8_t;
__device__ __forceinline__ uint32_t lds_addr(const void *p) {
  return (uint32_t)(uintptr_t)(lds_cu8_t *)p;
}
__device__ __forceinline__ float lds_read_f32(uint32_t addr) {
  return *(lds_cfloat_t *)(uintptr_t)addr;
}

__device__ __forceinline__ void build_lut(float *lut, int bound, const Dequant &dq,
                                          int tid, int nthreads = 256) {
  for (int i = tid; i <= 2 * bound; i += nthreads) lut[i] = dequant_acc_nb(i - bound, dq);
}

__device__ __forceinline__ int lut_column_start(const uint32_t *scr, int slot) {
  int st = 0;
  for (int k = 0; k < (slot & 3); ++k) st += (int)scr[(slot & ~3) + k];
  return st;
}
__device__ __forceinline__ uint32_t build_lut_channel(float *lut, const uint32_t *scr, int max_rows,
                                                      const Dequant &dq, const BnP &bn, int cout0,
                                                      int Cout, int tid) {
  uint32_t minbits = 0x7F800000u;
  const int c = tid & 127, hf = tid >> 7;
  const int slot = (int)scr[256 + c], col = slot >> 2;
  const int st = lut_column_start(scr, slot);
  const int rows = (int)scr[slot], negx = (int)scr[128 + c];
  if (st + rows > max_rows) return minbits;
  const int co = cout0 + c < Cout ? cout0 + c : Cout - 1;
  float bm = 0.f, bmul = 1.f, bb = 0.f;
  if (bn.mean) { bm = bn.mean[co]; bmul = bn.mul[co]; bb = bn.bias[co]; }
  for (int i = hf; i < rows; i += 2) {
    const float y = bn_apply(dequant_acc_nb(i - negx, dq), bm, bmul, bb);
    lut[(st + i) * 32 + col] = y;
    const uint32_t mag = __float_as_uint(y) & 0x7FFFFFFFu;
    if (mag != 0u && mag < minbits) minbits = mag;
  }
  return minbits;
}

__host__ __device__ __forceinline__ bool lif_fma_is_exact(uint32_t min_x_bits, int j, int T, bool has_u0) {
  if (has_u0 || j < 0) return false;
  const long long e = (long long)j * (T + 1) - 126;
  if (e > 100) return false;
  const uint32_t need = e <= -126 ? 0x00800000u : (uint32_t)(e + 127) << 23;
  return min_x_bits >= need;
}

__device__ __forceinline__ uint32_t lut_bn_min_bits(const float *lut, int bound, const BnP &bn,
                                                    int cout0, int Cout, int tid, int nthreads) {
  int c = cout0 + (tid & 127);
  if (c >= Cout) c = Cout - 1;
  float mean = 0.f, mul = 1.f, bias = 0.f;
  if (bn.mean) { mean = bn.mean[c]; mul = bn.mul[c]; bias = bn.bias[c]; }
  uint32_t mb = 0x7F800000u;
  for (int i = tid >> 7; i <= 2 * bound; i += nthreads >> 7) {
    float x = lut[i] - mean;
    x = x * mul;
    x = x + bias;
    const uint32_t b = __float_as_uint(x) & 0x7FFFFFFFu;
    if (b != 0 && b < mb) mb = b;
  }
  return mb;
}

template <int LUTM, bool OFFS = false>
__device__ __forceinline__ v2f dequant_pair(int a0, int a1, const Dequant &dq, float off = 0.0f) {
  if (LUTM != LUT_NONE) return v2f{lds_read_f32((uint32_t)a0), lds_read_f32((uint32_t)a1)};
  v2f a = {(float)a0, (float)a1};
  if (OFFS) a = a + off;
  const v2f q = fma2(a, v2f{dq.rL, dq.rL}, a * dq.rLlo);
  return q * dq.m;
}

template <int NF, bool FMA = false, bool PACKED = true>
__device__ __forceinline__ v2f neuron_update(v2f x, v2f u, const LaneConsts &lc,
                                             const NeuronP &nrn) {
  if (NF == NF_DECAY) {
    const v2f ud = u * lc.dec;
    return ud + x;
  }
  if (FMA && PACKED) {
    typedef float v2fp __attribute__((ext_vector_type(2)));
    const v2fp up = {u.x, u.y}, xp = {x.x, x.y};
    const v2fp dp = NF == NF_MUL0 ? xp - up : xp - (up - lc.vr);
    const v2fp r = __builtin_elementwise_fma(dp, v2fp{nrn.inv_k, nrn.inv_k}, up);
    return v2f{r.x, r.y};
  }
  const v2f d = NF == NF_MUL0 ? x - u : x - (u - lc.vr);
  if (NF == NF_DIV) return u + v2f{d.x / nrn.k, d.y / nrn.k};
  if (FMA) return fma2(d, v2f{nrn.inv_k, nrn.inv_k}, u);
  const v2f dk = d * nrn.inv_k;
  return u + dk;
}

template <int NF>
__device__ __forceinline__ float neuron_reset(float u, unsigned long long mask,
                                              const LaneConsts &lc) {
  if (NF == NF_MUL0) return reset_where(u, mask);
  float r;
  asm("v_cndmask_b32_e64 %0, %1, %2, %3" : "=v"(r) : "v"(u), "v"(lc.vr), "s"(mask));
  return r;
}

template <int NF, bool BNDONE, bool FMA = false>
__device__ __forceinline__ void neuron_pair(v2f y, float &u0, float &u1,
                                            const LaneConsts &lc, const NeuronP &nrn,
                                            unsigned long long &m0,
                                            unsigned long long &m1) {
  v2f x = y;
  if (!BNDONE) {
    x = x - lc.bmean;
    x = x * lc.bmul;
    x = x + lc.bbias;
  }
  const v2f uu = neuron_update<NF, FMA>(x, v2f{u0, u1}, lc, nrn);
  m0 = __ballot(uu.x >= nrn.vth);
  m1 = __ballot(uu.y >= nrn.vth);
  u0 = neuron_reset<NF>(uu.x, m0, lc);
  u1 = neuron_reset<NF>(uu.y, m1, lc);
}

template <int NF, bool POOL, bool BNDONE, bool FMA = false>
__device__ __forceinline__ uint32_t tile_neurons(const v2f (&y)[8], float (&u)[16],
                                                 const LaneConsts &lc, const NeuronP &nrn) {
  uint32_t myw = 0;
#pragma unroll
  for (int i = 0; i < 16; i += 2) {
    unsigned long long m0, m1;
    neuron_pair<NF, BNDONE, FMA>(y[i >> 1], u[i], u[i + 1], lc, nrn, m0, m1);
    if (POOL) {
      const unsigned long long o = m0 | m1;
      const uint32_t pw = (uint32_t)o | (uint32_t)(o >> 32);
      myw = writelane_u32(pw, i >> 1, myw);
    } else {
      const int r0 = (i & 3) + 8 * (i >> 2);
      myw = writelane_u32((uint32_t)m0, r0, myw);
      myw = writelane_u32((uint32_t)(m0 >> 32), r0 + 4, myw);
      myw = writelane_u32((uint32_t)m1, r0 + 1, myw);
      myw = writelane_u32((uint32_t)(m1 >> 32), r0 + 5, myw);
    }
  }
  return myw;
}

template <int NF, bool POOL, int LUTM, bool FMA = false, bool OFFS = false>
__device__ __forceinline__ uint32_t tile_epilogue(const v16i &acc, float (&u)[16],
                                                  const Dequant &dq,
                                                  const LaneConsts &lc,
                                                  const NeuronP &nrn, int lane,
                                                  float off = 0.0f) {
  v2f y[8];
#pragma unroll
  for (int j = 0; j < 8; ++j) y[j] = dequant_pair<LUTM, OFFS>(acc[2 * j], acc[2 * j + 1], dq, off);
  return tile_neurons<NF, POOL, LUTM == LUT_CHANNEL, FMA>(y, u, lc, nrn);
}

template <int NF, bool POOL, int LUTM, bool FMA = false, bool OFFS = false>
__device__ __forceinline__ uint32_t tile_epilogue_halves(const v16i &acc, float (&u)[16],
                                                         const Dequant &dq, const LaneConsts &lc,
                                                         const NeuronP &nrn, int lane, float off = 0.0f) {
  uint32_t myw = 0;
#pragma unroll
  for (int g = 0; g < 2; ++g) {
    v2f y[4];
#pragma unroll
    for (int j = 0; j < 4; ++j) y[j] = dequant_pair<LUTM, OFFS>(acc[8 * g + 2 * j], acc[8 * g + 2 * j + 1], dq, off);
#pragma unroll
    for (int j = 0; j < 4; ++j) {
      const int i = 8 * g + 2 * j;
      unsigned long long m0, m1;
      neuron_pair<NF, LUTM == LUT_CHANNEL, FMA>(y[j], u[i], u[i + 1], lc, nrn, m0, m1);
      if (POOL) {
        const unsigned long long o = m0 | m1;
        const uint32_t pw = (uint32_t)o | (uint32_t)(o >> 32);
        myw = writelane_u32(pw, i >> 1, myw);
      } else {
        const int r0 = (i & 3) + 8 * (i >> 2);
        myw = writelane_u32((uint32_t)m0, r0, myw);
        myw = writelane_u32((uint32_t)(m0 >> 32), r0 + 4, myw);
        myw = writelane_u32((uint32_t)m1, r0 + 1, myw);
        myw = writelane_u32((uint32_t)(m1 >> 32), r0 + 5, myw);
      }
    }
    __builtin_amdgcn_sched_barrier(0);
  }
  return myw;
}

template <bool POOL>
struct OutStage {
  static constexpr int NPIX = POOL ? 16 : 64;
  static constexpr int FL = POOL ? 32 : 8;
  static constexpr int BYTES = FL * NPIX * 16;
};

template <bool POOL>
__device__ __forceinline__ int out_pix(int tl, int lane) {
  if (POOL) return (tl * 2 + ((lane >> 2) & 1)) * 4 + (lane & 3);
  const int ty = ((lane >> 2) & 1) | (((lane >> 4) & 1) << 1);
  const int tx = (lane & 3) | (((lane >> 3) & 1) << 2);
  return (tl * 4 + ty) * 8 + tx;
}

template <bool POOL, int SLOTS, int NT, int NPIX = OutStage<POOL>::NPIX>
__device__ __forceinline__ void flush_ring(const uint32_t *obuf, const ConvMfmaArgs &a,
                                           int t0, int n, int b, int y0, int x0, int tid) {
  constexpr int PW = POOL ? 4 : 8;
  const int CW = (a.Cout + 31) >> 5;
  const int cwb = blockIdx.y * 4;
  const int nw = min(4, CW - cwb);
  const int OH = POOL ? a.H >> 1 : a.H, OW = POOL ? a.W >> 1 : a.W;
  const int oy0 = POOL ? y0 >> 1 : y0, ox0 = POOL ? x0 >> 1 : x0;
  for (int i = tid; i < n * NPIX; i += NT) {
    const int slot = i / NPIX, pix = i % NPIX;
    const int t = t0 + slot;
    const uint32_t *src = obuf + ((t % SLOTS) * NPIX + pix) * 4;
    const int oy = oy0 + pix / PW, ox = ox0 + pix % PW;
    if (oy >= OH || ox >= OW) continue;
    uint32_t *dst = a.s_out + ((((int64_t)t * a.B + b) * OH + oy) * OW + ox) * CW + cwb;
    if (nw == 4 && (CW & 3) == 0) {
      *(v4i *)dst = *(const v4i *)src;
    } else {
      for (int w = 0; w < nw; ++w) dst[w] = src[w];
    }
  }
}

template <bool POOL>
__device__ __forceinline__ void flush_out(const uint32_t *obuf, const ConvMfmaArgs &a,
                                          int t0, int n, int b, int y0, int x0, int tid) {
  flush_ring<POOL, OutStage<POOL>::FL, 256>(obuf, a, t0, n, b, y0, x0, tid);
}

template <bool LOAD>
__device__ __forceinline__ void u_io_tile(float (&u)[16], const ConvMfmaArgs &a, int b,
                                          int y0, int x0, int cout, int h, int tl) {
  float *uo = a.u_out;
  const float *ui = a.u0;
#pragma unroll
  for (int i = 0; i < 16; ++i) {
    const int y = y0 + tl * 4 + (h | ((i >> 3) << 1));
    const int x = x0 + (i & 7);
    const int64_t o = (((int64_t)b * a.H + y) * a.W + x) * a.Cout + cout;
    const bool in = y < a.H && x < a.W && cout < a.Cout;
    if (LOAD) u[i] = in ? ui[o] : 0.0f;
    else if (in) uo[o] = u[i];
  }
}

template <bool LOAD>
__device__ __forceinline__ void u_io(float (&u)[2][16], const ConvMfmaArgs &a,
                                     int b, int y0, int x0, int cout, int h) {
  float *uo = a.u_out;
  const float *ui = a.u0;
#pragma unroll
  for (int tl = 0; tl < 2; ++tl)
#pragma unroll
    for (int i = 0; i < 16; ++i) {
      const int y = y0 + tl * 4 + (h | ((i >> 3) << 1));
      const int x = x0 + (i & 7);
      const int64_t o = (((int64_t)b * a.H + y) * a.W + x) * a.Cout + cout;
      const bool in = y < a.H && x < a.W && cout < a.Cout;
      if (LOAD) u[tl][i] = in ? ui[o] : 0.0f;
      else if (in) uo[o] = u[tl][i];
    }
}

__device__ __forceinline__ void zero_u(float (&u)[2][16]) {
#pragma unroll
  for (int tl = 0; tl < 2; ++tl)
#pragma unroll
    for (int i = 0; i < 16; ++i) u[tl][i] = 0.0f;
}

__device__ __forceinline__ v16i splat16(int v) {
  return v16i{v, v, v, v, v, v, v, v, v, v, v, v, v, v, v, v};
}

uint32_t *sched_acquire(hipStream_t st, int *dev, int *slot);
void sched_release(int dev, int slot, hipStream_t st);
uint32_t *device_status_word(int dev);

void persistent_limits(const void *kernel, int threads, size_t dyn_lds, int dev, int *cus, int *occ);
int stream_device(hipStream_t st);

template <typename K>
static inline void launch_persistent(K kernel, ConvMfmaArgs a, unsigned gy, hipStream_t st,
                                     size_t dyn_lds = 0, int threads = 256) {
  int dev = 0, cus = 256, occ = 2, slot = -1;
  a.sched = gy <= (unsigned)SCHED_Y ? sched_acquire(st, &dev, &slot) : nullptr;
  if (!a.sched) dev = stream_device(st);
  a.status = a.sched ? device_status_word(dev) : nullptr;
  persistent_limits((const void *)kernel, threads, dyn_lds, dev, &cus, &occ);
  const int64_t gmax = (int64_t)cus * occ;
  unsigned gx = (unsigned)(a.npatch < gmax ? a.npatch : gmax);
  a.xcd_split = 0;
  if (gx >= 64 && a.B >= 8) {
    gx &= ~7u;
    a.xcd_split = 1;
  }
  hipLaunchKernelGGL(kernel, dim3(gx, gy), dim3(threads), dyn_lds, st, a);
  if (a.sched) sched_release(dev, slot, st);
}

enum { DQ_ARITH = 1, DQ_ONE = 2, DQ_TABLE = 3 };
constexpr int DQT_MAXA = 2047;
void launch_conv3x3_bits(const ConvMfmaArgs &a, int cin_pad, bool i8, int nf, bool pool, int dq,
                         bool fma, bool bnf, unsigned gy, hipStream_t st);

}
```

snnquantprune_amd/linen.py:

```python

from __future__ import annotations

import dataclasses
import functools
import hashlib
import math
import threading
from collections.abc import MutableMapping
from typing import Any, Callable, Dict, Iterable, Optional, Sequence

import torch

_tls = threading.local()


def _stack():
  if not hasattr(_tls, "stack"):
    _tls.stack = []
  return _tls.stack


class ConfigDict(MutableMapping):

  def __init__(self, *args, **kwargs):
    object.__setattr__(self, "_d", {})
    for k, v in dict(*args, **kwargs).items():
      self[k] = v

  def __getitem__(self, k):
    return self._d[k]

  def __setitem__(self, k, v):
    if isinstance(v, dict):
      v = ConfigDict(v)
    self._d[k] = v

  def __delitem__(self, k):
    del self._d[k]

  def __iter__(self):
    return iter(self._d)

  def __len__(self):
    return len(self._d)

  def __contains__(self, k):
    return k in self._d

  def __getattr__(self, k):
    try:
      return self._d[k]
    except KeyError:
      raise AttributeError(k)

  def __setattr__(self, k, v):
    self[k] = v

  def __delattr__(self, k):
    del self._d[k]

  def __hash__(self):
    return id(self)

  def __eq__(self, other):
    return self is other

  def __repr__(self):
    return "ConfigDict(%r)" % (self._d,)

  def to_dict(self):
    return {k: (v.to_dict() if isinstance(v, ConfigDict) else v)
            for k, v in self._d.items()}


FrozenConfigDict = ConfigDict



_DTYPE_POLICY = "strict"
_dtype_warned = False


def set_compute_dtype_policy(policy: str):
  global _DTYPE_POLICY
  if policy not in ("strict", "float32"):
    raise ValueError("compute dtype policy must be 'strict' or 'float32'")
  _DTYPE_POLICY = policy


_CHANNEL_COMPACTION = True


def set_channel_compaction(enabled: bool):
  global _CHANNEL_COMPACTION
  _CHANNEL_COMPACTION = bool(enabled)


def channel_compaction() -> bool:
  return _CHANNEL_COMPACTION


_CONV_KPACK = True


def set_conv_kpack(enabled: bool):
  global _CONV_KPACK
  _CONV_KPACK = bool(enabled)


def conv_kpack() -> bool:
  return _CONV_KPACK


def check_compute_dtype(dtype, who: str):
  global _dtype_warned
  if dtype in (torch.float32, None, "float32"):
    return
  if _DTYPE_POLICY == "float32":
    if not _dtype_warned:
      import sys
      print("snnquantprune_amd: %s asked for %r; computing in float32 (nn.set_compute_dtype_policy)"
            % (who, dtype), file=sys.stderr)
      _dtype_warned = True
    return
  raise NotImplementedError(
      "%s computes in float32 (got %r); nn.set_compute_dtype_policy('float32') runs such a "
      "request in float32 instead of refusing it" % (who, dtype))




def _default_device():
  return torch.device("cuda") if torch.cuda.is_available() else torch.device("cpu")


def zeros(key, shape, dtype=torch.float32):
  return torch.zeros(tuple(shape), dtype=dtype, device=_default_device())


def ones(key, shape, dtype=torch.float32):
  return torch.ones(tuple(shape), dtype=dtype, device=_default_device())


def constant(value):
  def init(key, shape, dtype=torch.float32):
    return torch.full(tuple(shape), float(value), dtype=dtype, device=_default_device())
  return init


def lecun_normal():
  def init(key, shape, dtype=torch.float32):
    shape = tuple(shape)
    fan_in = 1
    for d in shape[:-1]:
      fan_in *= d
    std = math.sqrt(1.0 / max(fan_in, 1)) / 0.87962566103423978
    w = torch.empty(shape, dtype=torch.float32)
    torch.nn.init.trunc_normal_(w, mean=0.0, std=std, a=-2 * std, b=2 * std,
                                generator=key)
    return w.to(dtype).to(_default_device())
  return init


class Variable:
  def __init__(self, module, col, name):
    self._m, self._col, self._name = module, col, name

  @property
  def value(self):
    return self._m._get(self._col, self._name)

  @value.setter
  def value(self, v):
    root = self._m._root
    if not (root.initializing or self._col in root.mutable):
      raise RuntimeError("collection %r is immutable" % self._col)
    self._m._set(self._col, self._name, v)


class _Root:
  def __init__(self, variables, mutable, initializing, rngs):
    self.variables = variables
    self.mutable = set(mutable)
    self.initializing = initializing
    self.rngs = rngs
    self.rng_count = 0


def _seed_of(rngs, name):
  key = None
  if isinstance(rngs, dict):
    key = rngs.get(name, rngs.get("params"))
  else:
    key = rngs
  if key is None:
    return 0
  if isinstance(key, torch.Generator):
    return key.initial_seed()
  if isinstance(key, torch.Tensor):
    return int(key.reshape(-1)[0].item())
  return int(key)


class Module:

  name: Optional[str] = dataclasses.field(default=None, kw_only=True)

  def __init_subclass__(cls, **kw):
    super().__init_subclass__(**kw)
    if "__call__" in cls.__dict__:
      cls.__call__ = _wrap_call(cls.__dict__["__call__"])
    dataclasses.dataclass(cls, eq=False, repr=False)

  def __post_init__(self):
    object.__setattr__(self, "_parent", None)
    object.__setattr__(self, "_root", None)
    object.__setattr__(self, "_path", None)
    object.__setattr__(self, "_autoname", {})
    st = _stack()
    if st:
      self._adopt(st[-1], None)

  def _adopt(self, parent, attr_name):
    name = self.name or attr_name
    if name is None:
      base = type(self).__name__
      idx = parent._autoname.get(base, 0)
      parent._autoname[base] = idx + 1
      name = "%s_%d" % (base, idx)
    object.__setattr__(self, "_parent", parent)
    object.__setattr__(self, "_root", parent._root)
    object.__setattr__(self, "_path", parent._path + (name,))

  def _bind_root(self, root):
    object.__setattr__(self, "_parent", None)
    object.__setattr__(self, "_root", root)
    object.__setattr__(self, "_path", ())

  @property
  def is_bound(self):
    return self._root is not None

  def _node(self, col, create):
    d = self._root.variables
    if col not in d:
      if not create:
        return None
      d[col] = {}
    d = d[col]
    for p in self._path:
      if p not in d:
        if not create:
          return None
        d[p] = {}
      d = d[p]
    return d

  def _get(self, col, name):
    node = self._node(col, False)
    if node is None or name not in node:
      raise KeyError("no variable %s/%s/%s" % (col, "/".join(self._path), name))
    return node[name]

  def _set(self, col, name, value):
    self._node(col, True)[name] = value

  def has_variable(self, col, name):
    node = self._node(col, False)
    return node is not None and name in node

  def make_rng(self, name="params"):
    root = self._root
    root.rng_count += 1
    h = hashlib.sha256(("%d/%s/%s/%d" % (_seed_of(root.rngs, name), name,
                                         "/".join(self._path), root.rng_count)
                        ).encode()).digest()
    g = torch.Generator()
    g.manual_seed(int.from_bytes(h[:8], "little") & ((1 << 63) - 1))
    return g

  def param(self, name, init_fn, *init_args):
    if not self.is_bound:
      raise RuntimeError("module %s is not bound; use init()/apply()" % type(self).__name__)
    if not self.has_variable("params", name):
      if not self._root.initializing:
        raise KeyError("parameter %s/%s not found in variables" %
                       ("/".join(self._path), name))
      self._set("params", name, init_fn(self.make_rng("params"), *init_args))
    return self._get("params", name)

  def variable(self, col, name, init_fn=None, *init_args):
    if not self.has_variable(col, name):
      if not (self._root.initializing or col in self._root.mutable):
        raise KeyError("variable %s/%s/%s not found" % (col, "/".join(self._path), name))
      self._set(col, name, init_fn(*init_args) if init_fn is not None else None)
    return Variable(self, col, name)

  def is_mutable_collection(self, col):
    return self._root.initializing or col in self._root.mutable

  def sow(self, col, name, value):
    if not self.is_bound or not (col in self._root.mutable):
      return False
    node = self._node(col, True)
    node[name] = tuple(node.get(name, ())) + (value,)
    return True

  def init(self, rngs, *args, **kwargs):
    root = _Root({}, mutable=(), initializing=True, rngs=rngs)
    return self._run(root, args, kwargs)[1]

  def init_with_output(self, rngs, *args, **kwargs):
    root = _Root({}, mutable=(), initializing=True, rngs=rngs)
    return self._run(root, args, kwargs)

  def apply(self, variables, *args, rngs=None, mutable=False, **kwargs):
    if mutable is True:
      mcols = set(variables.keys()) | {"intermediates"}
    elif not mutable:
      mcols = set()
    elif isinstance(mutable, str):
      mcols = {mutable}
    else:
      mcols = set(mutable)
    vars_copy = {c: (_copy_tree(v) if c in mcols else v) for c, v in variables.items()}
    root = _Root(vars_copy, mutable=mcols, initializing=False, rngs=rngs)
    out, allvars = self._run(root, args, kwargs)
    if mutable:
      return out, {c: allvars.get(c, {}) for c in mcols if c in allvars}
    return out

  def _run(self, root, args, kwargs):
    saved = (self._parent, self._root, self._path)
    st = _stack()
    saved_stack = list(st)
    del st[:]
    self._bind_root(root)
    try:
      out = self(*args, **kwargs)
    finally:
      object.__setattr__(self, "_parent", saved[0])
      object.__setattr__(self, "_root", saved[1])
      object.__setattr__(self, "_path", saved[2])
      st[:] = saved_stack
    return out, root.variables

  def __repr__(self):
    fs = ", ".join("%s=%r" % (f.name, getattr(self, f.name))
                   for f in dataclasses.fields(self)
                   if f.name != "name" and not isinstance(getattr(self, f.name), Module))
    return "%s(%s)" % (type(self).__name__, fs)


dataclasses.dataclass(Module, eq=False, repr=False)


def _copy_tree(t):
  if isinstance(t, dict):
    return {k: _copy_tree(v) for k, v in t.items()}
  return t


def _wrap_call(fn):
  @functools.wraps(fn)
  def wrapped(self, *args, **kwargs):
    st = _stack()
    if not self.is_bound:
      if not st:
        raise RuntimeError(
            "%s called outside init()/apply(): modules are stateless, use "
            "module.apply(variables, ...)" % type(self).__name__)
      parent = st[-1]
      attr = None
      for f in dataclasses.fields(parent):
        if getattr(parent, f.name, None) is self:
          attr = f.name
          break
      self._adopt(parent, attr)
    elif st and self._root is not st[-1]._root:
      parent = st[-1]
      object.__setattr__(self, "_root", parent._root)
    self._autoname.clear()
    st.append(self)
    try:
      return fn(self, *args, **kwargs)
    finally:
      st.pop()
  return wrapped


def compact(fn):
  return fn


compact_method = _wrap_call



from ._cache import TensorCache

_bn_cache = TensorCache(256)


class BatchNorm(Module):
  use_running_average: Optional[bool] = None
  axis: int = -1
  momentum: float = 0.99
  epsilon: float = 1e-5
  dtype: Any = torch.float32
  use_bias: bool = True
  use_scale: bool = True

  @compact_method
  def coeffs(self, features: int):
    from . import ops
    import numpy as np
    feat = (int(features),)
    mean = self.variable("batch_stats", "mean", lambda: zeros(None, feat)).value
    var = self.variable("batch_stats", "var", lambda: ones(None, feat)).value
    scale = self.param("scale", ones, feat) if self.use_scale else None
    bias = self.param("bias", zeros, feat) if self.use_bias else None
    hit = _bn_cache.get((mean, var, scale, bias), float(self.epsilon))
    if hit is not None:
      return hit
    dev = mean.device
    m = mean.detach().cpu().numpy().astype(np.float32)
    v = var.detach().cpu().numpy().astype(np.float32)
    mul = np.float32(1) / np.sqrt(v + np.float32(self.epsilon))
    if scale is not None:
      mul = mul * scale.detach().cpu().numpy().astype(np.float32)
    b = (bias.detach().cpu().numpy().astype(np.float32) if bias is not None
         else np.zeros_like(m))
    from . import _lib as L
    flags = (0 if m.any() else L.BN_MEAN_ZERO) | (0 if b.any() else L.BN_BIAS_ZERO)
    mul32 = mul.astype(np.float32)
    if mul32.size and np.all(mul32.view(np.uint32) == mul32.view(np.uint32).flat[0]) and np.isfinite(mul32.flat[0]):
      flags |= L.BN_MUL_UNIFORM
    out = ops.BnCoeffs(torch.from_numpy(m).to(dev),
                       torch.from_numpy(mul.astype(np.float32)).to(dev),
                       torch.from_numpy(b).to(dev), flags)
    return _bn_cache.put((mean, var, scale, bias), float(self.epsilon), out)

  def __call__(self, x, use_running_average: Optional[bool] = None):
    from . import ops
    ura = self.use_running_average if use_running_average is None else use_running_average
    if ura is None:
      raise ValueError("BatchNorm needs use_running_average")
    if not ura:
      raise NotImplementedError(
          "BatchNorm batch statistics (training mode) are out of scope: this "
          "package implements the eval forward pass")
    if self.axis not in (-1, x.ndim - 1):
      raise NotImplementedError("BatchNorm over a non-last axis")
    return ops.batchnorm_forward(x, self.coeffs(x.shape[-1]))




class CapturedApply:

  def __init__(self, module, variables, example, **kwargs):
    from . import ops
    self._ops = ops
    dev = example.device if not isinstance(example, torch.Tensor) else example.device
    if torch.device(dev).type != "cuda":
      raise RuntimeError("capture needs the inputs on the GPU")
    self.static_input = self._clone(example)
    self._stream = torch.cuda.Stream(device=dev)
    self._graph = torch.cuda.CUDAGraph()
    cur = torch.cuda.current_stream(dev)
    self._stream.wait_stream(cur)
    self._device = torch.device(dev)
    self._slots = None
    with torch.cuda.stream(self._stream):
      for _ in range(2):
        module.apply(variables, self.static_input, **kwargs)
      self._stream.synchronize()
      mark = ops.workqueue_capture_mark(self._device)
      self._workspaces, outer = [], ops._CAPTURE_KEEP
      ops._CAPTURE_KEEP = self._workspaces
      try:
        with torch.cuda.graph(self._graph, stream=self._stream):
          self.static_output = module.apply(variables, self.static_input, **kwargs)
      finally:
        ops._CAPTURE_KEEP = outer
        self._slots = (mark, ops.workqueue_capture_mark(self._device))
    cur.wait_stream(self._stream)

  def close(self):
    slots, self._slots = self._slots, None
    if slots is None or slots[0] == slots[1]:
      self._graph = None
      return
    try:
      torch.cuda.synchronize(self._device)
      self._graph = None
      self._ops.workqueue_capture_release(self._device, slots[0], slots[1])
    except Exception:
      pass

  def __del__(self):
    self.close()

  def _clone(self, x):
    ops = self._ops
    if isinstance(x, ops.PackedFrames):
      return ops.PackedFrames(x.data.clone(), x.H, x.W, x.fmt)
    if isinstance(x, ops.PackedSpikes):
      return ops.PackedSpikes(x.bits.clone(), x.channels)
    return x.clone()

  def _raw(self, x):
    ops = self._ops
    return x.data if isinstance(x, ops.PackedFrames) else x.bits if isinstance(x, ops.PackedSpikes) else x

  def __call__(self, inputs=None):
    if inputs is not None and inputs is not self.static_input:
      src, dst = self._raw(inputs), self._raw(self.static_input)
      if src.shape != dst.shape or src.dtype != dst.dtype:
        raise ValueError("captured for inputs %s %s, got %s %s"
                         % (tuple(dst.shape), dst.dtype, tuple(src.shape), src.dtype))
      dst.copy_(src, non_blocking=True)
    if self._graph is None:
      raise RuntimeError("this CapturedApply has been closed")
    self._graph.replay()
    return self.static_output


def capture(module, variables, example, **kwargs) -> CapturedApply:
  return CapturedApply(module, variables, example, **kwargs)




def tree_map(fn, tree):
  if isinstance(tree, dict):
    return {k: tree_map(fn, v) for k, v in tree.items()}
  if isinstance(tree, (tuple, list)):
    return type(tree)(tree_map(fn, v) for v in tree)
  return fn(tree)


def tree_to_device(tree, device):
  return tree_map(lambda x: x.to(device) if isinstance(x, torch.Tensor) else x, tree)


def tree_from_numpy(tree, device=None):
  import numpy as np
  device = device or _default_device()
  return tree_map(lambda x: torch.as_tensor(np.asarray(x)).to(device)
                  if not isinstance(x, torch.Tensor) else x.to(device), tree)
```

snnquantprune_amd/ops.py:

```python

from __future__ import annotations

import ctypes
from dataclasses import dataclass
from typing import Optional, Sequence, Tuple

import torch

from . import _lib as L




class PackedSpikes:

  def __init__(self, bits: torch.Tensor, channels: int):
    assert bits.dtype == torch.int32 and bits.is_contiguous()
    assert bits.shape[-1] == (channels + 31) // 32
    self.bits = bits
    self.channels = int(channels)
    self.flat_perm = None
    self.chan_map = None

  @property
  def shape(self):
    return tuple(self.bits.shape[:-1]) + (self.channels,)

  @property
  def device(self):
    return self.bits.device

  @property
  def ndim(self):
    return self.bits.ndim

  def __getitem__(self, idx):
    if not isinstance(idx, tuple):
      idx = (idx,)
    assert len(idx) < self.bits.ndim, "cannot index the packed channel axis"
    out = PackedSpikes(self.bits[idx].contiguous(), self.channels)
    out.chan_map = self.chan_map
    return out

  def reshape_leading(self, *lead):
    out = PackedSpikes(self.bits.reshape(*lead, self.bits.shape[-1]), self.channels)
    out.chan_map = self.chan_map
    return out

  def to_dense(self) -> torch.Tensor:
    return unpack_bits(self)

  def __repr__(self):
    return "PackedSpikes(shape=%s, device=%s)" % (self.shape, self.device)


class PackedFrames:

  def __init__(self, data: torch.Tensor, H: int, W: int, fmt: int):
    assert fmt in (L.EV1, L.EV4), fmt
    unit = frame_units(H, W, fmt)
    assert data.dtype == (torch.int32 if fmt == L.EV1 else torch.uint8), data.dtype
    assert data.shape[-1] == unit and data.is_contiguous(), (tuple(data.shape), unit)
    self.data, self.H, self.W, self.fmt = data, int(H), int(W), int(fmt)

  @property
  def shape(self):
    return tuple(self.data.shape[:-1]) + (self.H, self.W, 2)

  @property
  def device(self):
    return self.data.device

  @property
  def ndim(self):
    return self.data.ndim + 2

  @property
  def dtype(self):
    return torch.uint8

  @property
  def is_cuda(self):
    return self.data.is_cuda

  def __getitem__(self, idx):
    if not isinstance(idx, tuple):
      idx = (idx,)
    assert len(idx) < self.data.ndim, "cannot index inside a packed frame"
    return PackedFrames(self.data[idx].contiguous(), self.H, self.W, self.fmt)

  def narrow(self, dim, start, length):
    assert dim < self.data.ndim - 1
    return PackedFrames(self.data.narrow(dim, start, length).contiguous(), self.H, self.W, self.fmt)

  def to(self, device, non_blocking=False):
    return PackedFrames(self.data.to(device, non_blocking=non_blocking), self.H, self.W, self.fmt)

  def to_u8(self) -> torch.Tensor:
    return unpack_frames(self)

  def __repr__(self):
    return "PackedFrames(%s, shape=%s, device=%s)" % (
        "EV1" if self.fmt == L.EV1 else "EV4", self.shape, self.device)


class GatedSpikes:

  def __init__(self, spikes: "PackedSpikes", gate: torch.Tensor, flat: bool = False):
    assert isinstance(spikes, PackedSpikes) and spikes.ndim == 5, "spikes [T, B, H, W, C], bit-packed"
    assert gate.dtype == torch.float32 and tuple(gate.shape) == (spikes.shape[0], spikes.shape[1], spikes.channels)
    self.spikes, self.gate = spikes, gate.contiguous()
    self.flat = bool(flat)

  @property
  def shape(self):
    if self.flat:
      T, B, H, W, C = self.spikes.shape
      return (T, B, C * H * W)
    return self.spikes.shape

  @property
  def ndim(self):
    return 3 if self.flat else 5

  @property
  def device(self):
    return self.spikes.device

  def flattened(self) -> "GatedSpikes":
    return GatedSpikes(self.spikes, self.gate, flat=True)

  def to_dense(self) -> torch.Tensor:
    x = apply_gate(self.spikes, self.gate)
    if self.flat:
      x = x.permute(0, 1, 4, 2, 3)
      x = x.reshape(x.shape[0], x.shape[1], x.shape[2] * x.shape[3] * x.shape[4]).contiguous()
    return x


class ChannelMap:

  def __init__(self, index, live, full: int):
    import numpy as np
    self.index = np.asarray(index, np.int64)
    self.live = np.asarray(live, bool)
    self.full = int(full)
    self._dev = {}

  def device_index(self, device) -> torch.Tensor:
    key = str(device)
    t = self._dev.get(key)
    if t is None:
      t = self._dev[key] = torch.from_numpy(self.index.astype("int32")).to(device)
    return t

  def __repr__(self):
    return "ChannelMap(%d of %d, %d live)" % (self.index.size, self.full, int(self.live.sum()))


def scatter_spike_channels(s: "PackedSpikes", channel_map: torch.Tensor, cout: int) -> "PackedSpikes":
  bits = s.bits.contiguous()
  _require_gpu(bits, channel_map)
  assert channel_map.dtype == torch.int32 and channel_map.numel() == s.channels
  cw = (int(cout) + 31) // 32
  npix = bits.numel() // max(bits.shape[-1], 1) if bits.ndim else 0
  out = torch.empty(tuple(bits.shape[:-1]) + (cw,), dtype=torch.int32, device=bits.device)
  L.check(L.lib().snnqp_scatter_spike_channels(_ptr(bits), npix, s.channels,
                                                _ptr(channel_map.contiguous()), int(cout), _ptr(out),
                                                _stream()))
  return PackedSpikes(out, int(cout))


def expand_channels(x):
  cm = getattr(x, "chan_map", None)
  if cm is None:
    return x
  flat = x.flat_perm
  if flat is not None:
    c, h, w = flat
    lead = tuple(x.bits.shape[:-1])
    blk = PackedSpikes(x.bits.reshape(*lead, h, w, c // 32).contiguous(), c)
    full = scatter_spike_channels(blk, cm.device_index(x.device), cm.full)
    out = PackedSpikes(full.bits.reshape(*lead, h * w * ((cm.full + 31) // 32)), h * w * cm.full)
    out.flat_perm = (cm.full, h, w)
    return out
  return scatter_spike_channels(x, cm.device_index(x.device), cm.full)


def frame_units(H: int, W: int, fmt: int) -> int:
  return (H * W * 2 + 31) // 32 if fmt == L.EV1 else H * W


def pack_frames_host(x, fmt: int) -> PackedFrames:
  import numpy as np
  a = x.numpy() if isinstance(x, torch.Tensor) else np.asarray(x)
  if a.dtype != np.uint8 or a.ndim < 3 or a.shape[-1] != 2:
    raise ValueError("event frames must be uint8 [..., H, W, 2], got %s %s" % (a.dtype, a.shape))
  H, W = a.shape[-3], a.shape[-2]
  lead = a.shape[:-3]
  limit = 1 if fmt == L.EV1 else 15
  if a.size and int(a.max()) > limit:
    raise ValueError("event count %d does not fit the %s frame format (max %d)"
                     % (int(a.max()), "EV1" if fmt == L.EV1 else "EV4", limit))
  if fmt == L.EV1:
    flat = np.ascontiguousarray(a).reshape(lead + (H * W * 2,))
    b = np.packbits(flat, axis=-1, bitorder="little")
    nbytes = frame_units(H, W, fmt) * 4
    if b.shape[-1] != nbytes:
      b = np.concatenate([b, np.zeros(lead + (nbytes - b.shape[-1],), np.uint8)], -1)
    data = torch.from_numpy(np.ascontiguousarray(b).view(np.int32))
  else:
    data = torch.from_numpy(np.ascontiguousarray(a[..., 0] | (a[..., 1] << 4)).reshape(lead + (H * W,)))
  return PackedFrames(data, H, W, fmt)


def pack_frames(x: torch.Tensor, fmt: int, flags: Optional[torch.Tensor] = None) -> PackedFrames:
  _require_gpu(x, flags)
  assert x.dtype == torch.uint8 and x.shape[-1] == 2 and x.ndim >= 3, (x.dtype, tuple(x.shape))
  x = x.contiguous()
  H, W = x.shape[-3], x.shape[-2]
  lead = tuple(x.shape[:-3])
  frames = 1
  for d in lead:
    frames *= d
  data = torch.empty(lead + (frame_units(H, W, fmt),),
                     dtype=torch.int32 if fmt == L.EV1 else torch.uint8, device=x.device)
  L.check(L.lib().snnqp_pack_frames(_ptr(x), frames, H, W, fmt, _ptr(data), _ptr(flags), _stream()))
  return PackedFrames(data, H, W, fmt)


def pack_frames_checked(x: torch.Tensor) -> Tuple[PackedFrames, torch.Tensor]:
  _require_gpu(x)
  assert x.dtype in (torch.uint8, torch.float32) and x.shape[-1] == 2 and x.ndim >= 3, (x.dtype, tuple(x.shape))
  x = x.contiguous()
  H, W = x.shape[-3], x.shape[-2]
  lead = tuple(x.shape[:-3])
  frames = 1
  for d in lead:
    frames *= d
  data = torch.empty(lead + (frame_units(H, W, L.EV1),), dtype=torch.int32, device=x.device)
  flags = torch.empty(1, dtype=torch.int32, device=x.device)
  L.check(L.lib().snnqp_pack_frames_checked(_ptr(x), L.U8 if x.dtype == torch.uint8 else L.F32, frames, H, W,
                                            _ptr(data), _ptr(flags), _stream()))
  return PackedFrames(data, H, W, L.EV1), flags


def unpack_frames(p: PackedFrames) -> torch.Tensor:
  _require_gpu(p.data)
  lead = tuple(p.data.shape[:-1])
  frames = 1
  for d in lead:
    frames *= d
  y = torch.empty(lead + (p.H, p.W, 2), dtype=torch.uint8, device=p.device)
  L.check(L.lib().snnqp_unpack_frames(_ptr(p.data), p.fmt, frames, p.H, p.W, _ptr(y), _stream()))
  return y




def _stream():
  return ctypes.c_void_p(torch.cuda.current_stream().cuda_stream)


def _ptr(t: Optional[torch.Tensor]):
  return None if t is None else ctypes.c_void_p(t.data_ptr())


def _require_gpu(*ts):
  for t in ts:
    if t is None:
      continue
    if not t.is_cuda:
      raise RuntimeError(
          "snnquantprune_amd ops run on the GPU only (tensor on %s); there is no "
          "CPU fallback" % t.device)


def _f32c(t: torch.Tensor) -> torch.Tensor:
  if t.dtype != torch.float32:
    t = t.to(torch.float32)
  return t.contiguous()


def is_pow2(x: float) -> bool:
  import math
  if not (x > 0) or math.isinf(x):
    return False
  m, _ = math.frexp(x)
  return m == 0.5


@dataclass
class Weight:
  wtype: int
  w: torch.Tensor
  L: float = 1.0
  m: float = 1.0
  wt: Optional[torch.Tensor] = None
  abs_sum_max: int = 0
  code_max: int = 0
  min_current_bits: int = 0
  col_sum: Optional[torch.Tensor] = None
  wt6: Optional[torch.Tensor] = None
  ch_stack_max: int = 0
  ch_slots: Optional[torch.Tensor] = None
  wt_cin: int = 0

  def struct(self) -> L.WeightT:
    st = self.__dict__.get("_cstruct")
    if st is None:
      st = L.WeightT(self.wtype, self.w.data_ptr(), float(self.L), float(self.m),
                     int(self.abs_sum_max), int(self.code_max),
                     None if self.col_sum is None else self.col_sum.data_ptr(),
                     None if self.wt6 is None else self.wt6.data_ptr(),
                     int(self.min_current_bits), int(self.ch_stack_max),
                     None if self.ch_slots is None else self.ch_slots.data_ptr(), int(self.wt_cin))
      self.__dict__["_cstruct"] = st
    return st

  @property
  def is_int(self):
    return self.wtype == L.W_I8


@dataclass
class Neuron:
  kind: int
  k: float = 2.0
  v_threshold: float = 1.0
  v_reset: float = 0.0
  decay: Optional[torch.Tensor] = None

  def struct(self) -> L.NeuronT:
    return L.NeuronT(self.kind, float(self.k), float(self.v_threshold),
                     float(self.v_reset),
                     None if self.decay is None else self.decay.data_ptr())


@dataclass
class BnCoeffs:
  mean: torch.Tensor
  mul: torch.Tensor
  bias: torch.Tensor
  flags: int = 0

  def struct(self) -> L.BnT:
    return L.BnT(self.mean.data_ptr(), self.mul.data_ptr(), self.bias.data_ptr(), int(self.flags))


@dataclass
class ConvGeom:
  H: int
  W: int
  Cin: int
  Cout: int
  KH: int
  KW: int
  stride: Tuple[int, int] = (1, 1)
  pad: Tuple[Tuple[int, int], Tuple[int, int]] = ((0, 0), (0, 0))
  in_dil: Tuple[int, int] = (1, 1)
  k_dil: Tuple[int, int] = (1, 1)
  groups: int = 1

  def struct(self) -> L.ConvGeomT:
    return L.ConvGeomT(self.H, self.W, self.Cin, self.Cout, self.KH, self.KW,
                       self.stride[0], self.stride[1], self.pad[0][0],
                       self.pad[0][1], self.pad[1][0], self.pad[1][1],
                       self.in_dil[0], self.in_dil[1], self.k_dil[0],
                       self.k_dil[1], self.groups)

  def tag(self) -> str:
    return "%dx%dx%d->%d" % (self.H, self.W, self.Cin, self.Cout)

  def out_hw(self) -> Tuple[int, int]:
    oh, ow = ctypes.c_int32(), ctypes.c_int32()
    g = self.struct()
    L.check(L.lib().snnqp_conv_out_shape(ctypes.byref(g), ctypes.byref(oh),
                                         ctypes.byref(ow)))
    return oh.value, ow.value


@dataclass(frozen=True)
class Conv3dGeom:
  D: int
  H: int
  W: int
  Cin: int
  Cout: int
  KD: int
  KH: int
  KW: int
  stride: Tuple[int, int, int] = (1, 1, 1)
  pad: Tuple[Tuple[int, int], Tuple[int, int], Tuple[int, int]] = ((0, 0), (0, 0), (0, 0))
  in_dil: Tuple[int, int, int] = (1, 1, 1)
  k_dil: Tuple[int, int, int] = (1, 1, 1)
  groups: int = 1

  def struct(self) -> L.Conv3dGeomT:
    i3 = ctypes.c_int32 * 3
    return L.Conv3dGeomT(self.D, self.H, self.W, self.Cin, self.Cout, self.KD, self.KH, self.KW,
                         i3(*self.stride), i3(*[p[0] for p in self.pad]), i3(*[p[1] for p in self.pad]),
                         i3(*self.in_dil), i3(*self.k_dil), self.groups)

  def tag(self) -> str:
    return "%dx%dx%dx%d->%d" % (self.D, self.H, self.W, self.Cin, self.Cout)

  def out_dhw(self) -> Tuple[int, int, int]:
    od, oh, ow = ctypes.c_int32(), ctypes.c_int32(), ctypes.c_int32()
    g = self.struct()
    L.check(L.lib().snnqp_conv3d_out_shape(ctypes.byref(g), ctypes.byref(od), ctypes.byref(oh), ctypes.byref(ow)))
    return od.value, oh.value, ow.value


def _in_desc(x):
  if isinstance(x, PackedSpikes):
    return x.bits, L.BITS
  if isinstance(x, PackedFrames):
    return x.data, x.fmt
  if x.dtype == torch.uint8:
    return x, L.U8
  if x.dtype == torch.float32:
    return x, L.F32
  raise TypeError("activation dtype %s not supported (float32, uint8 or "
                  "PackedSpikes)" % x.dtype)




def quantize(kind: int, w: torch.Tensor, mask: Optional[torch.Tensor], bits: int,
             p0: float, p1: float = 0.0, want_fq: bool = True,
             want_codes: bool = False, sign: bool = True):
  w = _f32c(w)
  _require_gpu(w, mask)
  if mask is not None:
    mask = _f32c(mask)
    assert mask.shape == w.shape
  fq = torch.empty_like(w) if want_fq else None
  codes = torch.empty(w.shape, dtype=torch.int8, device=w.device) if want_codes else None
  flags = torch.zeros(1, dtype=torch.int32, device=w.device) if (
      want_codes or mask is not None) else None
  L.check(L.lib().snnqp_quantize_ex(kind, _ptr(w), _ptr(mask), w.numel(), int(bits), 1 if sign else 0,
                                    float(p0), float(p1), _ptr(fq), _ptr(codes),
                                    _ptr(flags), _stream()))
  return fq, codes, flags


def pack_codes_mfma(codes: torch.Tensor, n_pad: Optional[int] = None) -> torch.Tensor:
  _require_gpu(codes)
  assert codes.dtype == torch.int8
  c2 = codes.reshape(-1, codes.shape[-1]).contiguous()
  K, N = c2.shape
  n_pad = (N + 31) // 32 * 32 if n_pad is None else n_pad
  if K % 32:
    raise ValueError("MFMA tiling needs K % 32 == 0 (K = %d)" % K)
  wt = torch.empty((n_pad // 32, K // 32, 64, 16), dtype=torch.int8, device=codes.device)
  L.check(L.lib().snnqp_pack_codes_mfma(_ptr(c2), K, N, n_pad, _ptr(wt), _stream()))
  return wt


def pack_codes_fp6(codes: torch.Tensor, n_pad: Optional[int] = None) -> torch.Tensor:
  _require_gpu(codes)
  assert codes.dtype == torch.int8
  c2 = codes.reshape(-1, codes.shape[-1]).contiguous()
  K, N = c2.shape
  n_pad = (N + 31) // 32 * 32 if n_pad is None else n_pad
  wt6 = torch.empty((n_pad // 32, (K + 63) // 64, 1536), dtype=torch.uint8, device=codes.device)
  L.check(L.lib().snnqp_pack_codes_fp6(_ptr(c2), K, N, n_pad, _ptr(wt6), _stream()))
  return wt6




class NotCapturable(RuntimeError):
  """The step needs a value on the host and is being recorded into a hipGraph, which cannot wait
  for one.  (Nothing in this package does any more -- float32 inputs are checked on the device,
  snnqp.h x_flags -- the class stays for callers that catch it.)"""


@dataclass
class FloatFallback:
  weight: "Weight"
  x: Optional[torch.Tensor] = None
  pred: Optional[torch.Tensor] = None


def forget_inputs():
  """Kept for callers of earlier versions (bench.py called it each step to drop cached facts about
  the last batch): nothing about an activation tensor is cached on the host any more."""


class CountHint:

  BOUNDS = (1, 2, 3, 7, 31)
  COST = (1.0, 1.0, 1.0, 1.19, 1.19)
  GENERAL = 1.85

  def __init__(self, device):
    self.value = 1
    self.word = torch.zeros(8, dtype=torch.int32, device=device)
    self._host = torch.zeros(8, dtype=torch.int32).pin_memory()
    self._event = None
    self.max_seen = 0
    self.saw_counts = False

  def binary_so_far(self) -> bool:
    return self.current() == 1 and not self.saw_counts

  @staticmethod
  def capturing() -> bool:
    return torch.cuda.is_current_stream_capturing()

  @classmethod
  def choose(cls, words) -> int:
    w = list(words) + [0] * (6 - len(words))
    hist = [w[0], w[1], w[5], w[2] - w[5], w[3], w[4]]
    total = sum(hist)
    if total == 0:
      return 1
    best, best_cost = 255, cls.GENERAL * total
    below = 0
    for k, (bound, cost) in enumerate(zip(cls.BOUNDS, cls.COST)):
      below += hist[k]
      c = cost * below + cls.GENERAL * (total - below)
      if c < best_cost - 1e-9:
        best, best_cost = bound, c
    return best

  def current(self) -> int:
    if self.capturing():
      return self.value
    if self._event is not None and self._event.query():
      self._event = None
      words = [int(v) for v in self._host]
      self.max_seen = words[0]
      if self.max_seen > 1:
        self.saw_counts = True
      if sum(words[1:6]) > 0:
        self.value = max(1, min(self.choose(words[1:7]), self.max_seen))
    return self.value

  def seen_word(self):
    return None if self.capturing() else self.word

  def launched(self):
    if self.capturing():
      return
    if self._event is None:
      self._host.copy_(self.word, non_blocking=True)
      self.word.zero_()
      self._event = torch.cuda.Event()
      self._event.record()


_count_hints = {}


def count_hint(device) -> CountHint:
  key = torch.device(device).index if torch.device(device).index is not None else torch.cuda.current_device()
  h = _count_hints.get(key)
  if h is None:
    h = _count_hints[key] = CountHint(device)
  return h


def reset_count_hints(device=None):
  if device is None:
    _count_hints.clear()
  else:
    d = torch.device(device)
    _count_hints.pop(d.index if d.index is not None else torch.cuda.current_device(), None)


def f32_to_u8(x: torch.Tensor) -> torch.Tensor:
  x = _f32c(x)
  _require_gpu(x)
  y = torch.empty(x.shape, dtype=torch.uint8, device=x.device)
  L.check(L.lib().snnqp_f32_to_u8(_ptr(x), _ptr(y), x.numel(), _stream()))
  return y


def narrow_f32_async(x: torch.Tensor):
  x = _f32c(x)
  _require_gpu(x)
  y = torch.empty(x.shape, dtype=torch.uint8, device=x.device)
  flags = torch.zeros(2, dtype=torch.int32, device=x.device)
  L.check(L.lib().snnqp_narrow_f32(_ptr(x), _ptr(y), x.numel(), _ptr(flags), _stream()))
  return y, flags[1:2]


def pack_bits_checked(x: torch.Tensor):
  _require_gpu(x)
  if x.dtype not in (torch.float32, torch.uint8):
    x = x.to(torch.float32)
  x = x.contiguous()
  C = x.shape[-1]
  rows = x.numel() // C if C else 0
  bits = torch.empty(tuple(x.shape[:-1]) + ((C + 31) // 32,), dtype=torch.int32, device=x.device)
  flags = torch.zeros(1, dtype=torch.int32, device=x.device)
  L.check(L.lib().snnqp_pack_bits_checked(_ptr(x), L.F32 if x.dtype == torch.float32 else L.U8,
                                          rows, C, _ptr(bits), _ptr(flags), _stream()))
  return PackedSpikes(bits, C), flags


def pack_bits(x: torch.Tensor) -> PackedSpikes:
  _require_gpu(x)
  if x.dtype not in (torch.float32, torch.uint8):
    x = x.to(torch.float32)
  x = x.contiguous()
  C = x.shape[-1]
  rows = x.numel() // C if C else 0
  bits = torch.empty(tuple(x.shape[:-1]) + ((C + 31) // 32,), dtype=torch.int32,
                     device=x.device)
  L.check(L.lib().snnqp_pack_bits(_ptr(x), L.F32 if x.dtype == torch.float32 else L.U8,
                                  rows, C, _ptr(bits), _stream()))
  return PackedSpikes(bits, C)


def unpack_bits(s: PackedSpikes) -> torch.Tensor:
  _require_gpu(s.bits)
  y = torch.empty(s.shape, dtype=torch.float32, device=s.device)
  rows = y.numel() // s.channels
  L.check(L.lib().snnqp_unpack_bits(_ptr(s.bits), rows, s.channels, _ptr(y), _stream()))
  return y




def fseq_gemm_supported(geom: ConvGeom) -> bool:
  (pt, pb), (pl, pr) = geom.pad
  return (geom.groups == 1 and tuple(geom.stride) == (1, 1) and tuple(geom.in_dil) == (1, 1)
          and tuple(geom.k_dil) == (1, 1)
          and pt + pb == geom.KH - 1 and pl + pr == geom.KW - 1)


def conv_forward(x, geom: ConvGeom, weight: Weight, want_acc: bool = False):
  xt, in_type = _in_desc(x)
  xt = xt.contiguous()
  _require_gpu(xt, weight.w)
  NB = xt.shape[0]
  OH, OW = geom.out_hw()
  y = torch.empty((NB, OH, OW, geom.Cout), dtype=torch.float32, device=xt.device)
  acc = torch.empty(y.shape, dtype=torch.int32, device=xt.device) if want_acc else None
  g, w = geom.struct(), weight.struct()
  L.check(L.lib().snnqp_conv_forward(_ptr(xt), in_type, NB, ctypes.byref(g),
                                     ctypes.byref(w), _ptr(y), _ptr(acc), _stream()))
  return (y, acc) if want_acc else y


def conv3d_lif_forward(x, geom: Conv3dGeom, weight: Weight, neuron: Optional[Neuron] = None,
                       bn: Optional[BnCoeffs] = None, u0: Optional[torch.Tensor] = None, want_u: bool = True,
                       packed_out: bool = False, pred: Optional[torch.Tensor] = None, out=None):
  xt, in_type = _in_desc(x)
  xt = xt.contiguous()
  _require_gpu(xt, weight.w, u0)
  OD, OH, OW = geom.out_dhw()
  dev = xt.device
  unit = geom.D * geom.H * geom.W * xt.shape[-1]
  g, w = geom.struct(), weight.struct()
  b = bn.struct() if bn is not None else None
  if neuron is None:
    NB = xt.shape[0]
    y = out if out is not None else torch.empty((NB, OD, OH, OW, geom.Cout), dtype=torch.float32, device=dev)
    with _timed("conv3d[%s]" % geom.tag()):
      L.check(L.lib().snnqp_conv3d_lif_forward(_ptr(pred), _ptr(xt), in_type, 0, unit, 1, NB, ctypes.byref(g),
                                               ctypes.byref(w), None, None, None, None, _ptr(y), L.F32, _stream()))
    return y
  T, B = xt.shape[0], xt.shape[1]
  if out is not None:
    u_out, s = out
    s = s.bits if isinstance(s, PackedSpikes) else s
  else:
    u_out = torch.empty((B, OD, OH, OW, geom.Cout), dtype=torch.float32, device=dev) if want_u else None
    oshape = (T, B, OD, OH, OW)
    s = torch.empty(oshape + (((geom.Cout + 31) // 32,) if packed_out else (geom.Cout,)),
                    dtype=torch.int32 if packed_out else torch.float32, device=dev)
  if u0 is not None:
    u0 = _f32c(u0)
    assert tuple(u0.shape) == (B, OD, OH, OW, geom.Cout), (u0.shape, (B, OD, OH, OW, geom.Cout))
  _zero_step_carry(u_out, u0, T)
  n = neuron.struct()
  with _timed("conv3d[%s]" % geom.tag()):
    L.check(L.lib().snnqp_conv3d_lif_forward(_ptr(pred), _ptr(xt), in_type, B * unit, unit, T, B, ctypes.byref(g),
                                             ctypes.byref(w), ctypes.byref(b) if b is not None else None,
                                             ctypes.byref(n), _ptr(u0), _ptr(u_out), _ptr(s),
                                             L.BITS if packed_out else L.F32, _stream()))
  return u_out, (PackedSpikes(s, geom.Cout) if packed_out else s)


def conv_forward_speculative(x: torch.Tensor, geom: ConvGeom, int_weight: Weight, float_weight: Weight):
  x = _f32c(x)
  x8, pred = narrow_f32_async(x)
  y = conv_forward(x8, geom, int_weight)
  g, w = geom.struct(), float_weight.struct()
  L.check(L.lib().snnqp_conv_forward_if(_ptr(pred), _ptr(x), L.F32, x.shape[0], ctypes.byref(g), ctypes.byref(w),
                                        _ptr(y), _stream()))
  return y


def pack_codes_gated(codes: torch.Tensor, code_max: int = 7) -> torch.Tensor:
  _require_gpu(codes)
  assert codes.dtype == torch.int8 and codes.ndim == 4 and tuple(codes.shape[:2]) == (3, 3)
  codes = codes.contiguous()
  cin, cout = codes.shape[2], codes.shape[3]
  out = torch.empty(int(L.lib().snnqp_conv_gated_packed_bytes_ex(cin, cout, int(code_max))), dtype=torch.uint8,
                    device=codes.device)
  L.check(L.lib().snnqp_pack_codes_gated_ex(_ptr(codes), cin, cout, int(code_max), _ptr(out), _stream()))
  return out


def conv_gated_forward(x: GatedSpikes, geom: ConvGeom, weight: Weight, packed: torch.Tensor) -> torch.Tensor:
  bits, gate = x.spikes.bits.contiguous(), x.gate
  _require_gpu(bits, gate, weight.w, packed)
  T, B, H, W, _ = x.shape
  assert (H, W, x.spikes.channels) == (geom.H, geom.W, geom.Cin), (x.shape, geom)
  y = torch.empty((T, B, H, W, geom.Cout), dtype=torch.float32, device=bits.device)
  g, w = geom.struct(), weight.struct()
  with _timed("conv[gated %s]" % geom.tag()):
    L.check(L.lib().snnqp_conv_gated_forward(_ptr(bits), _ptr(gate), T * B, ctypes.byref(g), ctypes.byref(w),
                                             _ptr(packed), _ptr(y), _stream()))
  return y


def pack_codes_dense_gated(codes: torch.Tensor, C: int, HW: int, code_max: int = 7) -> torch.Tensor:
  _require_gpu(codes)
  assert codes.dtype == torch.int8 and codes.ndim == 2 and codes.shape[0] == C * HW
  codes = codes.contiguous()
  N = codes.shape[1]
  out = torch.empty(int(L.lib().snnqp_dense_gated_packed_bytes_ex(C, N, int(code_max))), dtype=torch.uint8,
                    device=codes.device)
  L.check(L.lib().snnqp_pack_codes_dense_gated_ex(_ptr(codes), C, HW, N, int(code_max), _ptr(out), _stream()))
  return out


def dense_gated_forward(x: GatedSpikes, weight: Weight, packed: torch.Tensor) -> torch.Tensor:
  bits, gate = x.spikes.bits.contiguous(), x.gate
  _require_gpu(bits, gate, weight.w, packed)
  T, B, H, W, C = x.spikes.shape
  N = weight.w.shape[-1]
  assert weight.w.shape[0] == C * H * W, (tuple(weight.w.shape), x.spikes.shape)
  y = torch.empty((T, B, N), dtype=torch.float32, device=bits.device)
  w = weight.struct()
  with _timed("dense[gated K=%d N=%d]" % (C * H * W, N)):
    L.check(L.lib().snnqp_dense_gated_forward(_ptr(bits), _ptr(gate), T * B, H * W, C, N, ctypes.byref(w),
                                              _ptr(packed), _ptr(y), _stream()))
  return y



_PROFILE = None
PROFILE_NOTES = {}


def profile_start():
  global _PROFILE
  _PROFILE = {}
  PROFILE_NOTES.clear()


def profile_stop():
  global _PROFILE
  prof, _PROFILE = _PROFILE or {}, None
  torch.cuda.synchronize()
  return {tag: (len(evs), sum(a.elapsed_time(b) for a, b in evs))
          for tag, evs in prof.items()}


class _timed:
  def __init__(self, tag):
    self.tag = tag

  def __enter__(self):
    if _PROFILE is not None:
      self.a = torch.cuda.Event(enable_timing=True)
      self.b = torch.cuda.Event(enable_timing=True)
      self.a.record()

  def __exit__(self, *exc):
    if _PROFILE is not None and exc[0] is None:
      self.b.record()
      _PROFILE.setdefault(self.tag, []).append((self.a, self.b))
    return False




_current_min_cache = None


def current_min_bits(weight: Weight, bn: Optional[BnCoeffs], bound: int, cout: int) -> int:
  global _current_min_cache
  if _current_min_cache is None:
    from ._cache import TensorCache
    _current_min_cache = TensorCache(64)
  key = (weight.w,) + ((bn.mean, bn.mul, bn.bias) if bn is not None else (None, None, None))
  extra = (int(bound), int(cout), float(weight.L), float(weight.m))
  v = _current_min_cache.get(key, extra)
  if v is None:
    _require_gpu(weight.w)
    out = torch.full((1,), 0x7F800000, dtype=torch.int32, device=weight.w.device)
    w = weight.struct()
    b = bn.struct() if bn is not None else None
    L.check(L.lib().snnqp_current_min(ctypes.byref(w), ctypes.byref(b) if b is not None else None,
                                      int(bound), int(cout), _ptr(out), _stream()))
    v = int(out.item()) & 0xFFFFFFFF
    _current_min_cache.put(key, extra, v)
  return v


def _tb_strides(x, T, B, time_major: bool, unit: int):
  if time_major:
    return B * unit, unit
  return unit, T * unit


def _zero_step_carry(u_out: Optional[torch.Tensor], u0: Optional[torch.Tensor], T: int):
  if u_out is not None and T == 0:
    if u0 is None:
      u_out.zero_()
    else:
      u_out.copy_(u0)


def conv_lif_forward(x, geom: ConvGeom, weight: Weight, neuron: Neuron,
                     bn: Optional[BnCoeffs] = None, u0: Optional[torch.Tensor] = None,
                     want_u: bool = True, packed_out: bool = False, pool: int = 1,
                     impl: int = L.IMPL_AUTO, time_major: bool = True, x_max: int = 0,
                     x_seen: Optional[torch.Tensor] = None,
                     fallback: Optional[FloatFallback] = None, binary_first: bool = False,
                     logical: Optional[Tuple[int, int, int]] = None):
  xt, in_type = _in_desc(x)
  xt = xt.contiguous()
  _require_gpu(xt, weight.w, u0)
  x_flags = None
  if in_type == L.F32 and weight.is_int:
    if fallback is None:
      raise ValueError("float32 input into integer codes needs a FloatFallback (the float32 kernel)")
    x_flags = torch.empty(1, dtype=torch.int32, device=xt.device)
  if x_seen is not None:
    assert x_seen.dtype == torch.int32 and x_seen.numel() >= 8 and x_seen.is_cuda, \
        "x_seen: eight int32 device words (snnqp.h)"
  T, B = (xt.shape[0], xt.shape[1]) if time_major else (xt.shape[1], xt.shape[0])
  if isinstance(x, PackedFrames):
    assert (x.H, x.W, 2) == (geom.H, geom.W, geom.Cin) and xt.ndim == 3, (x.shape, geom)
    unit = xt.shape[-1]
  else:
    unit = geom.H * geom.W * (xt.shape[-1])
  xs_t, xs_b = _tb_strides(xt, T, B, time_major, unit)
  OH, OW = geom.out_hw()
  dev = xt.device
  u_out = torch.empty((B, OH, OW, geom.Cout), dtype=torch.float32, device=dev) \
      if want_u else None
  if u0 is not None:
    u0 = _f32c(u0)
    assert tuple(u0.shape) == (B, OH, OW, geom.Cout), (u0.shape, (B, OH, OW, geom.Cout))
  _zero_step_carry(u_out, u0, T)
  oshape = (T, B, OH // pool, OW // pool)
  if packed_out:
    s = torch.empty(oshape + ((geom.Cout + 31) // 32,), dtype=torch.int32, device=dev)
  else:
    s = torch.empty(oshape + (geom.Cout,), dtype=torch.float32, device=dev)
  g, w, n = geom.struct(), weight.struct(), neuron.struct()
  b = bn.struct() if bn is not None else None
  cin_l, cout_l = (geom.Cin, geom.Cout) if logical is None else logical[:2]
  tag = "conv%dx%d[%dx%dx%d->%d]" % (geom.KH, geom.KW, geom.H, geom.W, cin_l, cout_l)
  if _PROFILE is not None and in_type == L.BITS and weight.is_int and "dequant" not in PROFILE_NOTES.get(tag, {}):
    PROFILE_NOTES.setdefault(tag, {})["dequant"] = conv_dequant_form(weight, neuron)
  if _PROFILE is not None and logical is not None:
    PROFILE_NOTES.setdefault(tag, {})["channels"] = {
        "cin": geom.Cin, "cout": geom.Cout, "live_out": int(logical[2])}
  speculate = (binary_first and packed_out and not isinstance(x, (PackedFrames, PackedSpikes))
               and in_type in (L.U8, L.F32) and geom.Cin == 2 and weight.is_int and impl != L.IMPL_GENERIC
               and xt.ndim == 5)
  with _timed(tag):
    if speculate:
      pf, not_binary = pack_frames_checked(xt)
      ps_t, ps_b = _tb_strides(pf.data, T, B, time_major, pf.data.shape[-1])
      try:
        L.check(L.lib().snnqp_conv_lif_forward(
            _ptr(pf.data), L.EV1, ps_t, ps_b, T, B, ctypes.byref(g), ctypes.byref(w),
            _ptr(weight.wt), ctypes.byref(b) if b is not None else None, ctypes.byref(n),
            _ptr(u0), _ptr(u_out), _ptr(s), L.BITS, pool, impl, 1, None, None, _stream()))
      except L.SnnqpError as e:
        if e.code != L.EUNSUPPORTED:
          raise
        speculate = False
    if speculate:
      L.check(L.lib().snnqp_conv_lif_forward_pred(
          _ptr(not_binary), _ptr(xt), in_type, xs_t, xs_b, T, B, ctypes.byref(g), ctypes.byref(w),
          _ptr(weight.wt), ctypes.byref(b) if b is not None else None, ctypes.byref(n),
          _ptr(u0), _ptr(u_out), _ptr(s), L.BITS, pool,
          int(x_max), _ptr(x_seen), _ptr(x_flags), _stream()))
    else:
      L.check(L.lib().snnqp_conv_lif_forward(
          _ptr(xt), in_type, xs_t, xs_b, T, B, ctypes.byref(g), ctypes.byref(w),
          _ptr(weight.wt), ctypes.byref(b) if b is not None else None, ctypes.byref(n),
          _ptr(u0), _ptr(u_out), _ptr(s), L.BITS if packed_out else L.F32, pool, impl,
          int(x_max), _ptr(x_seen), _ptr(x_flags), _stream()))
  if fallback is not None:
    xf = _f32c(xt if fallback.x is None else fallback.x)
    pred = x_flags if fallback.pred is None else fallback.pred
    fw = fallback.weight.struct()
    fs_t, fs_b = _tb_strides(xf, T, B, time_major, geom.H * geom.W * geom.Cin)
    L.check(L.lib().snnqp_conv_lif_forward_if(
        _ptr(pred), _ptr(xf), L.F32, fs_t, fs_b, T, B, ctypes.byref(g), ctypes.byref(fw),
        ctypes.byref(b) if b is not None else None, ctypes.byref(n), _ptr(u0), _ptr(u_out), _ptr(s),
        L.BITS if packed_out else L.F32, pool, _stream()))
  return u_out, (PackedSpikes(s, geom.Cout) if packed_out else s)


def dense_lif_forward(x, weight: Weight, K: int, N: int, neuron: Neuron,
                      bn: Optional[BnCoeffs] = None, u0: Optional[torch.Tensor] = None,
                      want_u: bool = True, packed_out: bool = False,
                      impl: int = L.IMPL_AUTO, time_major: bool = True,
                      fallback: Optional[FloatFallback] = None):
  xt, in_type = _in_desc(x)
  xt = xt.contiguous()
  _require_gpu(xt, weight.w, u0)
  x_flags = None
  if in_type == L.F32 and weight.is_int:
    if fallback is None:
      raise ValueError("float32 rows into integer codes need a FloatFallback (the float32 kernel)")
    x_flags = torch.empty(1, dtype=torch.int32, device=xt.device)
  T, B = (xt.shape[0], xt.shape[1]) if time_major else (xt.shape[1], xt.shape[0])
  xs_t, xs_b = _tb_strides(xt, T, B, time_major, xt.shape[-1])
  dev = xt.device
  u_out = torch.empty((B, N), dtype=torch.float32, device=dev) if want_u else None
  if u0 is not None:
    u0 = _f32c(u0)
    assert tuple(u0.shape) == (B, N)
  _zero_step_carry(u_out, u0, T)
  if packed_out:
    s = torch.empty((T, B, (N + 31) // 32), dtype=torch.int32, device=dev)
  else:
    s = torch.empty((T, B, N), dtype=torch.float32, device=dev)
  w, n = weight.struct(), neuron.struct()
  b = bn.struct() if bn is not None else None
  ws = _dense_workspace(dev, int(L.lib().snnqp_dense_workspace_bytes(in_type, T, B, K, N, ctypes.byref(w)))) \
      if (packed_out and impl != L.IMPL_GENERIC) else None
  with _timed("dense[%d->%d]" % (K, N)):
    L.check(L.lib().snnqp_dense_lif_forward_ws(
        _ptr(xt), in_type, xs_t, xs_b, T, B, K, N, ctypes.byref(w), _ptr(weight.wt),
        ctypes.byref(b) if b is not None else None, ctypes.byref(n), _ptr(u0),
        _ptr(u_out), _ptr(s), L.BITS if packed_out else L.F32, impl, _ptr(x_flags),
        _ptr(ws), 0 if ws is None else ws.numel(), _stream()))
  if fallback is not None:
    xf = _f32c(xt if fallback.x is None else fallback.x)
    pred = x_flags if fallback.pred is None else fallback.pred
    fw = fallback.weight.struct()
    L.check(L.lib().snnqp_dense_lif_forward_if(
        _ptr(pred), _ptr(xf), L.F32, xs_t, xs_b, T, B, K, N, ctypes.byref(fw),
        ctypes.byref(b) if b is not None else None, ctypes.byref(n), _ptr(u0), _ptr(u_out), _ptr(s),
        L.BITS if packed_out else L.F32, _stream()))
  return u_out, (PackedSpikes(s, N) if packed_out else s)


_dense_ws = {}
_CAPTURE_KEEP = None


def _dense_workspace(dev, nbytes: int):
  if nbytes <= 0:
    return None
  if torch.cuda.is_current_stream_capturing():
    ws = torch.empty(nbytes, dtype=torch.uint8, device=dev)
    if _CAPTURE_KEEP is not None:
      _CAPTURE_KEEP.append(ws)
    return ws
  key = (torch.device(dev).index, torch.cuda.current_stream(dev).cuda_stream)
  ws = _dense_ws.get(key)
  if ws is None or ws.numel() < nbytes:
    ws = _dense_ws[key] = torch.zeros(nbytes, dtype=torch.uint8, device=dev)
  return ws


def dense_head_forward(x, w1: Weight, K: int, N1: int, nrn1: Neuron, w2: Weight, N2: int,
                       nrn2: Neuron, group: int = 10, want_s1: bool = False,
                       want_s2: bool = False, time_major: bool = True,
                       fallback: Optional[FloatFallback] = None):
  xt, in_type = _in_desc(x)
  xt = xt.contiguous()
  _require_gpu(xt, w1.w, w2.w)
  T, B = (xt.shape[0], xt.shape[1]) if time_major else (xt.shape[1], xt.shape[0])
  xs_t, xs_b = _tb_strides(xt, T, B, time_major, xt.shape[-1])
  dev = xt.device
  if N2 % group:
    raise ValueError("vote: %d features not divisible by group %d" % (N2, group))
  logits = torch.empty((B, N2 // group), dtype=torch.float32, device=dev)
  x_flags = None
  if in_type == L.F32:
    if fallback is None or fallback.x is not None:
      raise ValueError("float32 rows into the fused head need a FloatFallback of the first block")
    x_flags = torch.empty(1, dtype=torch.int32, device=dev)
  elif fallback is not None:
    raise ValueError("a FloatFallback goes with float32 rows; uint8 / bit-packed rows have nothing to redo")
  redo = in_type == L.F32
  s1 = torch.empty((T, B, (N1 + 31) // 32), dtype=torch.int32, device=dev) if (want_s1 or redo) else None
  s2 = torch.empty((T, B, (N2 + 31) // 32), dtype=torch.int32, device=dev) if (want_s2 or redo) else None
  a, b, n1, n2 = w1.struct(), w2.struct(), nrn1.struct(), nrn2.struct()
  nws = _head_ws_bytes.get((T, B, N1))
  if nws is None:
    nws = _head_ws_bytes[(T, B, N1)] = int(L.lib().snnqp_dense_head_workspace_bytes(T, B, N1))
  ws = _dense_workspace(dev, nws)
  with _timed("dense_head[%d->%d->%d]" % (K, N1, N2)):
    L.check(L.lib().snnqp_dense_head_forward(
        _ptr(xt), in_type, xs_t, xs_b, T, B, K, N1, ctypes.byref(a), _ptr(w1.wt), ctypes.byref(n1),
        N2, ctypes.byref(b), _ptr(w2.wt), ctypes.byref(n2), int(group),
        _ptr(s1) if (want_s1 or redo) else None, _ptr(s2) if (want_s2 or redo) else None,
        _ptr(logits), _ptr(x_flags), _ptr(ws), 0 if ws is None else ws.numel(), _stream()))
  if redo:
    fw = fallback.weight.struct()
    lib = L.lib()
    L.check(lib.snnqp_dense_lif_forward_if(_ptr(x_flags), _ptr(xt), L.F32, xs_t, xs_b, T, B, K, N1,
                                           ctypes.byref(fw), None, ctypes.byref(n1), None, None, _ptr(s1),
                                           L.BITS, _stream()))
    cw1 = (N1 + 31) // 32
    L.check(lib.snnqp_dense_lif_forward_if(_ptr(x_flags), _ptr(s1), L.BITS, B * cw1, cw1, T, B, N1, N2,
                                           ctypes.byref(b), None, ctypes.byref(n2), None, None, _ptr(s2),
                                           L.BITS, _stream()))
    L.check(lib.snnqp_vote_if(_ptr(x_flags), _ptr(s2), L.BITS, T, B, N2, int(group), _ptr(logits), _stream()))
  return (logits, PackedSpikes(s1, N1) if want_s1 else None,
          PackedSpikes(s2, N2) if want_s2 else None)


_head_ws_bytes = {}


def fallback_counts(reset: bool = False) -> dict:
  conv, dense = ctypes.c_int64(), ctypes.c_int64()
  buf = ctypes.create_string_buffer(256)
  L.check(L.lib().snnqp_fallback_counts(ctypes.byref(conv), ctypes.byref(dense), buf, 256,
                                        1 if reset else 0))
  return {"conv_blocks": conv.value, "dense_blocks": dense.value,
          "last_reason": buf.value.decode("utf-8", "replace")}


def device_status(device=None, reset: bool = False) -> int:
  dev = torch.cuda.current_device() if device is None else torch.device(device).index
  code = ctypes.c_uint32()
  L.check(L.lib().snnqp_device_status(int(dev or 0), ctypes.byref(code), 1 if reset else 0))
  return int(code.value)


def workqueue_stats(reset: bool = False) -> dict:
  a, b, c = ctypes.c_int64(), ctypes.c_int64(), ctypes.c_int64()
  L.check(L.lib().snnqp_workqueue_stats(ctypes.byref(a), ctypes.byref(b), ctypes.byref(c), 1 if reset else 0))
  return {"captured_static_walks": a.value, "busy_static_walks": b.value, "dequant_table_fallbacks": c.value}


def workqueue_capture_mark(device) -> int:
  m = ctypes.c_int64()
  L.check(L.lib().snnqp_workqueue_capture_mark(int(torch.device(device).index or 0), ctypes.byref(m)))
  return int(m.value)


def workqueue_capture_release(device, begin: int, end: int):
  L.check(L.lib().snnqp_workqueue_capture_release(int(torch.device(device).index or 0), int(begin), int(end)))


DQ_FORMS = {1: "arith", 2: "one", 3: "table"}


def conv_dequant_form(w: Weight, nrn: Neuron) -> str:
  ws, ns = w.struct(), nrn.struct()
  rc = L.lib().snnqp_conv_dequant_form(ctypes.byref(ws), ctypes.byref(ns))
  if rc < 0:
    L.check(rc)
  return DQ_FORMS[rc]




def lif_forward(x: torch.Tensor, neuron: Neuron, bn: Optional[BnCoeffs] = None,
                u0: Optional[torch.Tensor] = None, want_u: bool = True,
                packed_out: bool = False):
  x = _f32c(x)
  _require_gpu(x, u0)
  T, C = x.shape[0], x.shape[-1]
  R = (x.numel() // (T * C)) if T * C else 0
  u_out = torch.empty(x.shape[1:], dtype=torch.float32, device=x.device) if want_u else None
  if u0 is not None:
    u0 = _f32c(u0)
    assert tuple(u0.shape) == tuple(x.shape[1:])
  _zero_step_carry(u_out, u0, T)
  if packed_out:
    s = torch.empty(tuple(x.shape[:-1]) + ((C + 31) // 32,), dtype=torch.int32,
                    device=x.device)
  else:
    s = torch.empty_like(x)
  n = neuron.struct()
  b = bn.struct() if bn is not None else None
  L.check(L.lib().snnqp_lif_forward(
      _ptr(x), T, R, C, ctypes.byref(b) if b is not None else None, ctypes.byref(n),
      _ptr(u0), _ptr(u_out), _ptr(s), L.BITS if packed_out else L.F32, _stream()))
  return u_out, (PackedSpikes(s, C) if packed_out else s)


def batchnorm_forward(x: torch.Tensor, bn: BnCoeffs) -> torch.Tensor:
  x = _f32c(x)
  _require_gpu(x)
  C = x.shape[-1]
  y = torch.empty_like(x)
  b = bn.struct()
  L.check(L.lib().snnqp_batchnorm_forward(_ptr(x), x.numel() // C if C else 0, C,
                                          ctypes.byref(b), _ptr(y), _stream()))
  return y


def maxpool2x2(x):
  if isinstance(x, PackedSpikes):
    bits = x.bits
    _require_gpu(bits)
    H, W = bits.shape[-3], bits.shape[-2]
    lead = tuple(bits.shape[:-3])
    NB = 1
    for d in lead:
      NB *= d
    y = torch.empty(lead + (H // 2, W // 2, bits.shape[-1]), dtype=torch.int32,
                    device=bits.device)
    L.check(L.lib().snnqp_maxpool2x2(_ptr(bits), L.BITS, NB, H, W, x.channels, _ptr(y),
                                     _stream()))
    return PackedSpikes(y, x.channels)
  x = _f32c(x)
  _require_gpu(x)
  H, W, C = x.shape[-3:]
  lead = tuple(x.shape[:-3])
  NB = 1
  for d in lead:
    NB *= d
  y = torch.empty(lead + (H // 2, W // 2, C), dtype=torch.float32, device=x.device)
  L.check(L.lib().snnqp_maxpool2x2(_ptr(x), L.F32, NB, H, W, C, _ptr(y), _stream()))
  return y


def spatial_mean(x) -> torch.Tensor:
  if isinstance(x, PackedSpikes):
    t, typ, C = x.bits, L.BITS, x.channels
  else:
    t, typ, C = _f32c(x), L.F32, x.shape[-1]
  _require_gpu(t)
  lead = tuple(t.shape[:-3])
  HW = t.shape[-3] * t.shape[-2]
  NB = 1
  for d in lead:
    NB *= d
  y = torch.empty(lead + (C,), dtype=torch.float32, device=t.device)
  L.check(L.lib().snnqp_spatial_mean(_ptr(t), typ, NB, HW, C, _ptr(y), _stream()))
  return y


def sigmoid_gate(a: torch.Tensor, b: torch.Tensor) -> torch.Tensor:
  a, b = _f32c(a), _f32c(b)
  _require_gpu(a, b)
  assert a.shape == b.shape
  g = torch.empty_like(a)
  L.check(L.lib().snnqp_sigmoid_gate(_ptr(a), _ptr(b), a.numel(), _ptr(g), _stream()))
  return g


def apply_gate(x, g: torch.Tensor) -> torch.Tensor:
  if isinstance(x, PackedSpikes):
    t, typ, C = x.bits, L.BITS, x.channels
  else:
    t, typ, C = _f32c(x), L.F32, x.shape[-1]
  g = _f32c(g)
  _require_gpu(t, g)
  lead = tuple(t.shape[:-3])
  H, W = t.shape[-3], t.shape[-2]
  assert tuple(g.shape) == lead + (C,), (g.shape, lead, C)
  NB = 1
  for d in lead:
    NB *= d
  y = torch.empty(lead + (H, W, C), dtype=torch.float32, device=t.device)
  L.check(L.lib().snnqp_apply_gate(_ptr(t), typ, _ptr(g), NB, H * W, C, _ptr(y), _stream()))
  return y


def events_to_frames(x, y, p, T: int, H: int, W: int, scale: float = 1.0, as_u8=True):
  x = x.to(torch.int32).contiguous()
  y = y.to(torch.int32).contiguous()
  p = p.to(torch.int32).contiguous()
  _require_gpu(x, y, p)
  counts = torch.empty((T, H, W, 2), dtype=torch.int32, device=x.device)
  u8 = torch.empty((T, H, W, 2), dtype=torch.uint8, device=x.device) if as_u8 else None
  L.check(L.lib().snnqp_events_to_frames(_ptr(x), _ptr(y), _ptr(p), x.numel(), T, H, W,
                                         float(scale), _ptr(counts), _ptr(u8), _stream()))
  return u8 if as_u8 else counts


def density(x, lead_dims: int = 2, counts: bool = False) -> torch.Tensor:
  if isinstance(x, PackedFrames):
    x = unpack_frames(x)
  if isinstance(x, GatedSpikes):
    x = x.to_dense()
  if isinstance(x, PackedSpikes):
    t, typ, C, shape = x.bits, L.BITS, x.channels, x.shape
  elif x.dtype == torch.uint8:
    t, typ, C, shape = x.contiguous(), L.U8, x.shape[-1], tuple(x.shape)
  else:
    t, typ, C, shape = _f32c(x), L.F32, x.shape[-1], tuple(x.shape)
  _require_gpu(t)
  lead = tuple(shape[:lead_dims])
  NB = 1
  for d in lead:
    NB *= d
  n = 1
  for d in shape[lead_dims:]:
    n *= d
  nnz = torch.empty(lead, dtype=torch.int32, device=t.device)
  L.check(L.lib().snnqp_density(_ptr(t), typ, NB, n, C, _ptr(nnz), _stream()))
  if counts:
    return nnz
  return nnz.to(torch.float32) / float(n)


def vote(s, group: int = 10) -> torch.Tensor:
  if isinstance(s, PackedSpikes):
    t, typ, N = s.bits, L.BITS, s.channels
  else:
    t, typ, N = _f32c(s), L.F32, s.shape[-1]
  _require_gpu(t)
  T, B = t.shape[0], t.shape[1]
  if N % group:
    raise ValueError("vote: %d features not divisible by group %d" % (N, group))
  out = torch.empty((B, N // group), dtype=torch.float32, device=t.device)
  L.check(L.lib().snnqp_vote(_ptr(t), typ, T, B, N, group, _ptr(out), _stream()))
  return out




def lif_forward_save(x: torch.Tensor, neuron: Neuron):
  x = _f32c(x)
  _require_gpu(x)
  T, C = x.shape[0], x.shape[-1]
  R = (x.numel() // (T * C)) if T * C else 0
  h = torch.empty_like(x)
  s = torch.empty_like(x)
  L.check(L.lib().snnqp_lif_forward_save(_ptr(x), T, R, C, ctypes.byref(neuron.struct()),
                                         _ptr(h), _ptr(s), _stream()))
  return h, s


def lif_backward(h: torch.Tensor, neuron: Neuron, surrogate: int, gs: Optional[torch.Tensor] = None,
                 glogits: Optional[torch.Tensor] = None, group: int = 10) -> torch.Tensor:
  h = _f32c(h)
  gs = None if gs is None else _f32c(gs)
  glogits = None if glogits is None else _f32c(glogits)
  _require_gpu(h, gs, glogits)
  T, C = h.shape[0], h.shape[-1]
  R = (h.numel() // (T * C)) if T * C else 0
  gI = torch.empty_like(h)
  L.check(L.lib().snnqp_lif_backward(_ptr(h), _ptr(gs), _ptr(glogits), int(group), T, R, C,
                                     ctypes.byref(neuron.struct()), int(surrogate), _ptr(gI),
                                     _stream()))
  return gI


def dense_weight_grad(x: torch.Tensor, gI: torch.Tensor) -> torch.Tensor:
  x, gI = _f32c(x), _f32c(gI)
  _require_gpu(x, gI)
  M, K = x.shape
  N = gI.shape[1]
  assert gI.shape[0] == M
  gw = torch.empty((K, N), dtype=torch.float32, device=x.device)
  L.check(L.lib().snnqp_dense_weight_grad(_ptr(x), _ptr(gI), M, K, N, _ptr(gw), _stream()))
  return gw


def dense_input_grad(gI: torch.Tensor, w: torch.Tensor, mask: Optional[torch.Tensor] = None) -> torch.Tensor:
  gI, w = _f32c(gI), _f32c(w)
  mask = None if mask is None else _f32c(mask)
  _require_gpu(gI, w, mask)
  M, N = gI.shape
  K = w.shape[0]
  assert w.shape[1] == N and (mask is None or tuple(mask.shape) == (M, K))
  gx = torch.empty((M, K), dtype=torch.float32, device=gI.device)
  L.check(L.lib().snnqp_dense_input_grad(_ptr(gI), _ptr(w), _ptr(mask), M, K, N, _ptr(gx),
                                         _stream()))
  return gx
```

Baseline: 94410 samples/s.

## Add three-wave workgroup variant of event-input first conv for 96-channel layers

For bit-packed event input with per-channel LUTs and 65-96 output channels, the first conv layer now launches 192-thread workgroups (three waves) instead of 256, so no fourth wave idles on padded channels. The output ring is sized to the actual waves and time-slot count, and a smaller nibble table replaces the 2 KB byte expansion table. Together these shrink LDS per workgroup so more workgroups fit per CU, and the halo fetch now handles two tasks per thread. The path is skipped when the occupancy query misses its target, and new plan/launch-info entry points plus profiling notes are added.

```diff
diff --git a/include/snnqp.h b/include/snnqp.h
--- a/include/snnqp.h
+++ b/include/snnqp.h
@@ -101,7 +101,7 @@
   int32_t groups;
 } snnqp_conv3d_geom_t;
 
-#define SNNQP_VERSION 505
+#define SNNQP_VERSION 506
 int snnqp_version(void);
 const char *snnqp_last_error(void);
 const char *snnqp_build_flags(void);
@@ -212,6 +212,9 @@
 int snnqp_workqueue_capture_release(int device, int64_t mark_begin, int64_t mark_end);
 int snnqp_workqueue_stats(int64_t *captured_static, int64_t *busy_static,
                           int64_t *dequant_fallbacks, int reset);
+int snnqp_set_event_waves(int three);
+int snnqp_event_layer_plan(int32_t T, int32_t pool, int32_t lut_rows, int32_t wgs_per_cu, int32_t *plan);
+int snnqp_event_launch_info(int32_t *info);
 int snnqp_debug_workqueue_poke(int device, int64_t mark, int word, uint32_t value);
 
 #define SNNQP_DQ_ARITH 1
diff --git a/snnquantprune_amd/_lib.py b/snnquantprune_amd/_lib.py
--- a/snnquantprune_amd/_lib.py
+++ b/snnquantprune_amd/_lib.py
@@ -9,7 +9,7 @@
 _HERE = os.path.dirname(os.path.abspath(__file__))
 LIB_PATH = os.path.join(_HERE, "csrc", "libsnnqp.so")
 
-ABI_VERSION = 505
+ABI_VERSION = 506
 
 F32, U8, BITS, EV1, EV4 = 0, 1, 2, 3, 4
 W_F32, W_I8 = 0, 1
@@ -139,6 +139,9 @@
     "snnqp_workqueue_capture_release": (c_int, [c_int, c_int64, c_int64]),
     "snnqp_workqueue_stats": (c_int, [POINTER(c_int64), POINTER(c_int64), POINTER(c_int64), c_int]),
     "snnqp_debug_workqueue_poke": (c_int, [c_int, c_int64, c_int, c_uint32]),
+    "snnqp_set_event_waves": (c_int, [c_int]),
+    "snnqp_event_layer_plan": (c_int, [c_int32, c_int32, c_int32, c_int32, POINTER(c_int32)]),
+    "snnqp_event_launch_info": (c_int, [POINTER(c_int32)]),
     "snnqp_fallback_counts": (c_int, [POINTER(c_int64), POINTER(c_int64), c_char_p, c_int32, c_int]),
     "snnqp_conv_dequant_form": (c_int, [POINTER(WeightT), POINTER(NeuronT)]),
     "snnqp_current_min": (c_int, [POINTER(WeightT), POINTER(BnT), c_int32, c_int32, c_void_p, c_void_p]),
diff --git a/snnquantprune_amd/csrc/conv3x3_u8c2.hip b/snnquantprune_amd/csrc/conv3x3_u8c2.hip
--- a/snnquantprune_amd/csrc/conv3x3_u8c2.hip
+++ b/snnquantprune_amd/csrc/conv3x3_u8c2.hip
@@ -42,11 +42,16 @@
   if (IN == SNNQP_EV1) return SNNQP_U8C2_EV1_WPS;
   return ONE ? SNNQP_U8C2_ONE_WPS : U8C2_WPS;
 }
-template <int NF, bool POOL, int LUTM, int IN = SNNQP_U8, bool ONE = false>
-__global__ void __launch_bounds__(256, (u8c2_waves<NF, POOL, LUTM, IN, ONE>()))
+constexpr int u8c2_wgs_per_cu(int waves_per_simd, int nw) { return waves_per_simd * 4 / nw; }
+constexpr int u8c2_xtab_bytes(int nw) { return nw == 4 ? 2048 : 64; }
+template <int NF, bool POOL, int LUTM, int IN = SNNQP_U8, bool ONE = false, int NW = 4>
+__global__ void __launch_bounds__(64 * NW, (u8c2_waves<NF, POOL, LUTM, IN, ONE>()))
 conv3x3_u8c2_kernel(ConvMfmaArgs a) {
   constexpr int FL = OutStage<POOL>::FL;
   constexpr bool EV1 = IN == SNNQP_EV1;
+  constexpr int NT = 64 * NW;
+  static_assert(NW == 4 || (NW == 3 && EV1 && LUTM == LUT_CHANNEL),
+                "three waves: bit-packed frames on per-channel tables only");
   constexpr bool EV4 = IN == SNNQP_EV4;
   constexpr bool F32IN = IN == SNNQP_F32;
   static_assert(TCHUNK % FL == 0, "flush period must divide the staging chunk");
@@ -61,15 +66,24 @@
   const int wave = __builtin_amdgcn_readfirstlane(tid >> 6);
   const int n = lane & 31, h = lane >> 5;
   const int cout_base = blockIdx.y * 128 + wave * 32;
-  const bool wave_on = cout_base < a.Cout;
+  const bool wave_on = NW == 3 || cout_base < a.Cout;
   const int cout = wave_on ? cout_base + n : n;
   const int cpar = cout < a.Cout ? cout : a.Cout - 1;
   const uint32_t cmask = chan_mask(cout_base, a.Cout);
-  uint32_t *wgw = obuf + OutStage<POOL>::BYTES / 4;
+  uint32_t *wgw = obuf + a.ring_bytes / 4;
   if (tid == 0) { wgw[0] = 0x7F800000u; wgw[1] = 0u; }
   typedef int v2i_a8 __attribute__((ext_vector_type(2)));
   v2i_a8 *xtab = (v2i_a8 *)(wgw + 4);
-  if (EV1) {
+  uint32_t *ntab = wgw + 4;
+  if (EV1 && NW == 3) {
+    if (tid < 16) {
+      uint32_t e = 0;
+#pragma unroll
+      for (int j = 0; j < 4; ++j) e |= (((uint32_t)tid >> j) & 1u ? 16u : 0u) << (8 * j);
+      ntab[tid] = e;
+    }
+    if (tid < 128) obuf[tid] = 0u;
+  } else if (EV1) {
     const uint32_t one = LUTM == LUT_CHANNEL ? 16u : LUTM == LUT_SHARED ? 4u : 0x81u;
     const uint32_t zero = LUTM == LUT_NONE ? 0x80u : 0u;
     uint32_t e[2] = {0, 0};
@@ -116,8 +130,8 @@
     for (int k = 0; k < 4; ++k) total += (int)scr[(slot & ~3) + k];
     ch_row0 = start + neg * a.x_limit;
     if (total > a.lut_rows && a.status) *(volatile uint32_t *)a.status = SNNQP_STATUS_BOUND;
-    const uint32_t mb = build_lut_channel((float *)(lds + lut_off), scr, a.lut_rows, a.dq, a.bn,
-                                          blockIdx.y * 128, a.Cout, tid);
+    const uint32_t mb = build_lut_channel<NW>((float *)(lds + lut_off), scr, a.lut_rows, a.dq, a.bn,
+                                              blockIdx.y * 128, a.Cout, tid);
     atomicMin(wgw, mb);
     lds_barrier();
   }
@@ -185,8 +199,7 @@
     offB[tl] = h ? (int)lds_addr(lds) + HCONST2 : px0 + (ty + 4 * tl + 1) * HROW2;
   }
   const uint8_t *xb = (const uint8_t *)a.x;
-  const int ob0 = out_pix<POOL>(0, lane) * 4 + wave;
-  const int ob1 = out_pix<POOL>(1, lane) * 4 + wave;
+  const int ob0 = out_pix<POOL>(0, lane) * NW + wave;
   const bool store_lane = POOL ? lane < 8 : lane < 32;
   uint32_t seen = 0;
   uint32_t hist[6] = {0, 0, 0, 0, 0, 0};
@@ -226,7 +239,7 @@
       bool general = LUTM == LUT_NONE;
       if constexpr (EV1) {
         lds_barrier();
-        for (int task = tid; task < nt * HALO; task += 256) {
+        auto fetch = [&](int task) -> uint32_t {
           const int tt = task / HALO, hy = task - tt * HALO;
           const int gy = y0 + hy - 1;
           const bool rv = gy >= 0 && gy < a.H;
@@ -234,21 +247,40 @@
           const uint32_t wi = start >> 5;
           const uint32_t *f = e_frames + (int64_t)(t0 + tt) * a.xs_t;
           const uint32_t lo = f[wi], hi = f[min(wi + 1u, e_fwords - 1u)];
-          uint32_t v = __builtin_amdgcn_alignbit(hi, lo, start & 31u);
-          v = (v << (2u - e_lead)) & (rv ? e_colmask : 0u);
-          const v2i_a8 d0 = xtab[v & 0xFFu], d1 = xtab[(v >> 8) & 0xFFu], d2 = xtab[(v >> 16) & 0xFu];
+          const uint32_t v = __builtin_amdgcn_alignbit(hi, lo, start & 31u);
+          return (v << (2u - e_lead)) & (rv ? e_colmask : 0u);
+        };
+        auto put = [&](int task, uint32_t q0, uint32_t q1, uint32_t q2, uint32_t q3, uint32_t q4, uint32_t q5) {
+          const int tt = task / HALO, hy = task - tt * HALO;
           uint8_t *row = lds + tt * HIMG2 + hy * HROW2;
-          *(v2i_a8 *)row = d0;
-          *(v2i_a8 *)(row + 8) = d1;
-          *(v2i_a8 *)(row + 16) = d2;
-          const uint32_t q0 = (uint32_t)d0.x, q1 = (uint32_t)d0.y, q2 = (uint32_t)d1.x,
-                         q3 = (uint32_t)d1.y, q4 = (uint32_t)d2.x, q5 = (uint32_t)d2.y;
+          *(v2i_a8 *)row = v2i_a8{(int)q0, (int)q1};
+          *(v2i_a8 *)(row + 8) = v2i_a8{(int)q2, (int)q3};
+          *(v2i_a8 *)(row + 16) = v2i_a8{(int)q4, (int)q5};
           uint8_t *row1 = row + HCOPY2;
           *(v2i_a8 *)row1 = v2i_a8{(int)(q0 << 16), (int)__builtin_amdgcn_alignbit(q1, q0, 16)};
           *(v2i_a8 *)(row1 + 8) = v2i_a8{(int)__builtin_amdgcn_alignbit(q2, q1, 16),
                                          (int)__builtin_amdgcn_alignbit(q3, q2, 16)};
           *(v2i_a8 *)(row1 + 16) = v2i_a8{(int)__builtin_amdgcn_alignbit(q4, q3, 16),
                                           (int)__builtin_amdgcn_alignbit(q5, q4, 16)};
+        };
+        if constexpr (NW == 3) {
+          auto put_nib = [&](int task, uint32_t v) {
+            put(task, ntab[v & 0xFu], ntab[(v >> 4) & 0xFu], ntab[(v >> 8) & 0xFu], ntab[(v >> 12) & 0xFu],
+                ntab[(v >> 16) & 0xFu], 0u);
+          };
+          for (int task = tid; task < nt * HALO; task += 2 * NT) {
+            const bool two = task + NT < nt * HALO;
+            const uint32_t va = fetch(task);
+            const uint32_t vb = two ? fetch(task + NT) : 0u;
+            put_nib(task, va);
+            if (two) put_nib(task + NT, vb);
+          }
+        } else {
+        for (int task = tid; task < nt * HALO; task += NT) {
+          const uint32_t v = fetch(task);
+          const v2i_a8 d0 = xtab[v & 0xFFu], d1 = xtab[(v >> 8) & 0xFFu], d2 = xtab[(v >> 16) & 0xFu];
+          put(task, (uint32_t)d0.x, (uint32_t)d0.y, (uint32_t)d1.x, (uint32_t)d1.y, (uint32_t)d2.x, (uint32_t)d2.y);
+        }
         }
         lds_barrier();
       } else {
@@ -379,13 +411,13 @@
                                                                      lane, acc_off);
           }
           if (store_lane) {
-            uint32_t *o = obuf + ((t0 + tt) % FL) * (OutStage<POOL>::NPIX * 4);
+            uint32_t *o = obuf + ((t0 + tt) % FL) * (OutStage<POOL>::NPIX * NW);
             o[ob0] = words[0] & cmask;
-            o[ob0 + (POOL ? 32 : 128)] = words[1] & cmask;
+            o[ob0 + (POOL ? 8 : 32) * NW] = words[1] & cmask;
           }
         }
         lds_barrier();
-        flush_out<POOL>(obuf, a, t0 + tf, nf, b, y0, x0, tid);
+        flush_out<POOL, NW>(obuf, a, t0 + tf, nf, b, y0, x0, tid);
         lds_barrier();
       }
       };
@@ -453,6 +485,8 @@
   std::vector<int> capture_free;
 };
 std::atomic<int64_t> g_static_captured{0}, g_static_busy{0};
+std::atomic<int> g_event_three_waves{1};
+std::atomic<int32_t> g_event_launch[4] = {{0}, {0}, {0}, {0}};
 std::mutex g_sched_mu;
 SchedPool g_sched[64];
 
@@ -642,6 +676,35 @@
   const bool tab = fp6 && neuron_form(make_neuron(nrn)) == NF_MUL0 && w->abs_sum_max > 0 &&
                    w->abs_sum_max <= DQT_MAXA;
   return tab ? DQ_TABLE : DQ_ARITH;
+}
+
+bool u8c2_three_waves(int in_type, int lutm, int Cout) {
+  return in_type == SNNQP_EV1 && lutm == LUT_CHANNEL && Cout > 64 && Cout <= 96;
+}
+
+int u8c2_fit_chunk(int tc0, size_t rest, size_t per_wg) {
+  int tc = tc0;
+  while (tc > 16 && (size_t)tc * HIMG2 + rest > per_wg) tc -= 1;
+  return (size_t)tc * HIMG2 + rest <= per_wg ? tc : 0;
+}
+
+struct U8c2Plan {
+  int tchunk, ring_bytes;
+  size_t lds_bytes;
+};
+bool u8c2_plan_three(int T, bool pool, size_t table_bytes, int wgs, U8c2Plan *p) {
+  p->ring_bytes = pool ? u8c2_ring_bytes<true>(T, 3, true) : u8c2_ring_bytes<false>(T, 3, true);
+  const size_t rest = table_bytes + (size_t)p->ring_bytes + 16 + u8c2_xtab_bytes(3);
+  p->tchunk = u8c2_fit_chunk(T >= TCHUNK ? TCHUNK : T, rest, (size_t)(160 * 1024) / wgs);
+  p->lds_bytes = (size_t)p->tchunk * HIMG2 + rest;
+  return p->tchunk != 0;
+}
+
+static void event_launch_note(int nw, int occ, size_t ldsb, int tchunk) {
+  g_event_launch[0].store(nw, std::memory_order_relaxed);
+  g_event_launch[1].store(occ, std::memory_order_relaxed);
+  g_event_launch[2].store((int32_t)ldsb, std::memory_order_relaxed);
+  g_event_launch[3].store(tchunk, std::memory_order_relaxed);
 }
 
 int run_conv3x3_mfma(const void *x, int in_type, int64_t xs_t, int64_t xs_b,
@@ -695,8 +758,7 @@
   const bool lut = w->abs_sum_max > 0 && xm > 0 && xm <= LUT_XMAX && bound <= LUT_CAP;
   a.lut_bound = lut ? (int32_t)bound : 0;
   a.tchunk = T >= TCHUNK ? TCHUNK : T;
-  const size_t lds_fixed = (size_t)a.tchunk * HIMG2 + 16 + (ev1 ? 2048 : 0) +
-                           (pl ? OutStage<true>::BYTES : OutStage<false>::BYTES);
+  a.ring_bytes = 0;
   const int64_t stack = w->ch_stack_max > 0 ? (int64_t)w->ch_stack_max : 8 * (int64_t)w->abs_sum_max;
   const int64_t crows = stack * xm + 4;
   const bool lutc = lut && in_type != SNNQP_BITS && crows <= LUT2_ROWS && xm <= 7 &&
@@ -705,14 +767,14 @@
   a.ch_slots = lutc && w->ch_stack_max > 0 ? w->ch_slots : nullptr;
 #define SNNQP_CONV_LAUNCH_IN(KERN, NFV, PL, LM, LDS)                               \
   do {                                                                             \
-    if (ev1 && one) launch_persistent(KERN<NFV, PL, LM, SNNQP_EV1, true>, a, gy, st, LDS); \
-    else if (ev1) launch_persistent(KERN<NFV, PL, LM, SNNQP_EV1>, a, gy, st, LDS);       \
-    else if (in_type == SNNQP_EV4 && one) launch_persistent(KERN<NFV, PL, LM, SNNQP_EV4, true>, a, gy, st, LDS); \
-    else if (in_type == SNNQP_EV4) launch_persistent(KERN<NFV, PL, LM, SNNQP_EV4>, a, gy, st, LDS); \
-    else if (in_type == SNNQP_F32 && one) launch_persistent(KERN<NFV, PL, LM, SNNQP_F32, true>, a, gy, st, LDS); \
-    else if (in_type == SNNQP_F32) launch_persistent(KERN<NFV, PL, LM, SNNQP_F32>, a, gy, st, LDS); \
-    else if (one) launch_persistent(KERN<NFV, PL, LM, SNNQP_U8, true>, a, gy, st, LDS);            \
-    else launch_persistent(KERN<NFV, PL, LM, SNNQP_U8>, a, gy, st, LDS);            \
+    if (ev1 && one) occ = launch_persistent(KERN<NFV, PL, LM, SNNQP_EV1, true>, a, gy, st, LDS); \
+    else if (ev1) occ = launch_persistent(KERN<NFV, PL, LM, SNNQP_EV1>, a, gy, st, LDS);       \
+    else if (in_type == SNNQP_EV4 && one) occ = launch_persistent(KERN<NFV, PL, LM, SNNQP_EV4, true>, a, gy, st, LDS); \
+    else if (in_type == SNNQP_EV4) occ = launch_persistent(KERN<NFV, PL, LM, SNNQP_EV4>, a, gy, st, LDS); \
+    else if (in_type == SNNQP_F32 && one) occ = launch_persistent(KERN<NFV, PL, LM, SNNQP_F32, true>, a, gy, st, LDS); \
+    else if (in_type == SNNQP_F32) occ = launch_persistent(KERN<NFV, PL, LM, SNNQP_F32>, a, gy, st, LDS); \
+    else if (one) occ = launch_persistent(KERN<NFV, PL, LM, SNNQP_U8, true>, a, gy, st, LDS);            \
+    else occ = launch_persistent(KERN<NFV, PL, LM, SNNQP_U8>, a, gy, st, LDS);            \
   } while (0)
 #define SNNQP_CONV_LAUNCH_NF(KERN, NFV, LM, LDS)                                   \
   do {                                                                             \
@@ -743,12 +805,42 @@
     const int lm = lutc ? LUT_CHANNEL : lut ? LUT_SHARED : LUT_NONE;
     if (lut) check_code_bound_once(stream_device(st), (const int8_t *)w->w, (int64_t)9 * g->Cin, g->Cout,
                                    w->abs_sum_max, st);
-    const size_t lds_rest = lds_fixed - (size_t)a.tchunk * HIMG2 + u8c2_table_bytes(lm, a.lut_bound, a.lut_rows);
+    int occ = -1, nw = 4;
+    const size_t tbl = u8c2_table_bytes(lm, a.lut_bound, a.lut_rows);
+    if (g_event_three_waves.load(std::memory_order_relaxed) && u8c2_three_waves(in_type, lm, g->Cout)) {
+      const int tc0 = a.tchunk;
+      for (int wgs = 8; wgs >= 6 && occ < 0; wgs -= 2) {
+        U8c2Plan plan;
+        if (!u8c2_plan_three(T, pl, tbl, wgs, &plan)) continue;
+        const int tc = plan.tchunk;
+        const size_t ldsb = plan.lds_bytes;
+        const bool one = !a.u0 && !a.u_out && a.T <= tc;
+        const int want = u8c2_wgs_per_cu(one && nf == NF_MUL0 && pl ? SNNQP_U8C2_EV1_ONE_WPS : SNNQP_U8C2_EV1_WPS, 3);
+        if (wgs != want) continue;
+        a.tchunk = tc;
+        a.ring_bytes = plan.ring_bytes;
+#define SNNQP_CONV_LAUNCH3(NFV, PL)                                                              \
+  do {                                                                                           \
+    if (one) occ = launch_persistent(conv3x3_u8c2_kernel<NFV, PL, LUT_CHANNEL, SNNQP_EV1, true, 3>, a, gy, st, \
+                                     ldsb, 192, want);                                           \
+    else occ = launch_persistent(conv3x3_u8c2_kernel<NFV, PL, LUT_CHANNEL, SNNQP_EV1, false, 3>, a, gy, st,   \
+                                 ldsb, 192, want);                                               \
+  } while (0)
+        if (nf == NF_MUL0) { if (pl) SNNQP_CONV_LAUNCH3(NF_MUL0, true); else SNNQP_CONV_LAUNCH3(NF_MUL0, false); }
+        else if (nf == NF_MUL) { if (pl) SNNQP_CONV_LAUNCH3(NF_MUL, true); else SNNQP_CONV_LAUNCH3(NF_MUL, false); }
+        else if (nf == NF_DIV) { if (pl) SNNQP_CONV_LAUNCH3(NF_DIV, true); else SNNQP_CONV_LAUNCH3(NF_DIV, false); }
+        else { if (pl) SNNQP_CONV_LAUNCH3(NF_DECAY, true); else SNNQP_CONV_LAUNCH3(NF_DECAY, false); }
+#undef SNNQP_CONV_LAUNCH3
+        if (occ >= 0) { nw = 3; event_launch_note(3, occ, ldsb, tc); }
+      }
+      if (occ < 0) a.tchunk = tc0;
+    }
+    if (occ < 0) {
+    a.ring_bytes = pl ? u8c2_ring_bytes<true>(T, 4, lutc) : u8c2_ring_bytes<false>(T, 4, lutc);
+    const size_t lds_rest = tbl + (size_t)a.ring_bytes + 16 + (ev1 ? u8c2_xtab_bytes(4) : 0);
     for (int wgs = 4; wgs >= 2; --wgs) {
-      const size_t per_wg = (size_t)(160 * 1024) / wgs - 512;
-      int tc = a.tchunk;
-      while (tc > 16 && (size_t)tc * HIMG2 + lds_rest > per_wg) tc -= 1;
-      if ((size_t)tc * HIMG2 + lds_rest <= per_wg) {
+      const int tc = u8c2_fit_chunk(a.tchunk, lds_rest, (size_t)(160 * 1024) / wgs - 512);
+      if (tc) {
         a.tchunk = tc;
         break;
       }
@@ -758,6 +850,8 @@
     if (lutc) SNNQP_CONV_LAUNCH(conv3x3_u8c2_kernel, LUT_CHANNEL, ldsb);
     else if (lut) SNNQP_CONV_LAUNCH(conv3x3_u8c2_kernel, LUT_SHARED, ldsb);
     else SNNQP_CONV_LAUNCH(conv3x3_u8c2_kernel, LUT_NONE, ldsb);
+    if (!pred) event_launch_note(nw, occ, ldsb, a.tchunk);
+    }
   }
 #undef SNNQP_CONV_LAUNCH
 #undef SNNQP_CONV_LAUNCH_NF
@@ -792,6 +886,31 @@
   return SNNQP_OK;
 }
 
+extern "C" int snnqp_set_event_waves(int three) {
+  snnqp::g_event_three_waves.store(three != 0, std::memory_order_relaxed);
+  return SNNQP_OK;
+}
+
+extern "C" int snnqp_event_layer_plan(int32_t T, int32_t pool, int32_t lut_rows, int32_t wgs_per_cu,
+                                      int32_t *plan) {
+  using namespace snnqp;
+  SNNQP_REQUIRE(plan && T > 0 && lut_rows >= 0 && wgs_per_cu > 0 && (pool == 1 || pool == 2), SNNQP_EINVAL,
+                "event_layer_plan: bad argument");
+  U8c2Plan p;
+  u8c2_plan_three(T, pool == 2, (size_t)u8c2_table_bytes(LUT_CHANNEL, 0, lut_rows), wgs_per_cu, &p);
+  plan[0] = p.tchunk;
+  plan[1] = p.ring_bytes;
+  plan[2] = (int32_t)p.lds_bytes;
+  return SNNQP_OK;
+}
+
+extern "C" int snnqp_event_launch_info(int32_t *info) {
+  using namespace snnqp;
+  SNNQP_REQUIRE(info, SNNQP_EINVAL, "event_launch_info: null pointer");
+  for (int i = 0; i < 4; ++i) info[i] = g_event_launch[i].load(std::memory_order_relaxed);
+  return SNNQP_OK;
+}
+
 extern "C" int snnqp_workqueue_stats(int64_t *captured_static, int64_t *busy_static,
                                      int64_t *dequant_fallbacks, int reset) {
   using namespace snnqp;
diff --git a/snnquantprune_amd/csrc/conv_tile.h b/snnquantprune_amd/csrc/conv_tile.h
--- a/snnquantprune_amd/csrc/conv_tile.h
+++ b/snnquantprune_amd/csrc/conv_tile.h
@@ -57,6 +57,7 @@
   uint32_t *status;
   int32_t patch_h;
   const int32_t *pred;
+  int32_t ring_bytes;
 };
 
 constexpr int SCHED_Y = 8;
@@ -182,11 +183,12 @@
   for (int k = 0; k < (slot & 3); ++k) st += (int)scr[(slot & ~3) + k];
   return st;
 }
+template <int NW = 4>
 __device__ __forceinline__ uint32_t build_lut_channel(float *lut, const uint32_t *scr, int max_rows,
                                                       const Dequant &dq, const BnP &bn, int cout0,
                                                       int Cout, int tid) {
   uint32_t minbits = 0x7F800000u;
-  const int c = tid & 127, hf = tid >> 7;
+  const int c = tid % (32 * NW), hf = tid / (32 * NW);
   const int slot = (int)scr[256 + c], col = slot >> 2;
   const int st = lut_column_start(scr, slot);
   const int rows = (int)scr[slot], negx = (int)scr[128 + c];
@@ -360,6 +362,13 @@
 };
 
 template <bool POOL>
+__host__ __device__ constexpr int u8c2_ring_bytes(int T, int wpp, bool lut_channel) {
+  const int slots = T < OutStage<POOL>::FL ? T : OutStage<POOL>::FL;
+  const int b = slots * OutStage<POOL>::NPIX * wpp * 4;
+  return lut_channel && b < 384 * 4 ? 384 * 4 : b;
+}
+
+template <bool POOL>
 __device__ __forceinline__ int out_pix(int tl, int lane) {
   if (POOL) return (tl * 2 + ((lane >> 2) & 1)) * 4 + (lane & 3);
   const int ty = ((lane >> 2) & 1) | (((lane >> 4) & 1) << 1);
@@ -367,34 +376,37 @@
   return (tl * 4 + ty) * 8 + tx;
 }
 
-template <bool POOL, int SLOTS, int NT, int NPIX = OutStage<POOL>::NPIX>
+template <bool POOL, int SLOTS, int NT, int NPIX = OutStage<POOL>::NPIX, int WPP = 4>
 __device__ __forceinline__ void flush_ring(const uint32_t *obuf, const ConvMfmaArgs &a,
                                            int t0, int n, int b, int y0, int x0, int tid) {
   constexpr int PW = POOL ? 4 : 8;
   const int CW = (a.Cout + 31) >> 5;
   const int cwb = blockIdx.y * 4;
-  const int nw = min(4, CW - cwb);
+  const int nw = min(WPP, CW - cwb);
   const int OH = POOL ? a.H >> 1 : a.H, OW = POOL ? a.W >> 1 : a.W;
   const int oy0 = POOL ? y0 >> 1 : y0, ox0 = POOL ? x0 >> 1 : x0;
   for (int i = tid; i < n * NPIX; i += NT) {
     const int slot = i / NPIX, pix = i % NPIX;
     const int t = t0 + slot;
-    const uint32_t *src = obuf + ((t % SLOTS) * NPIX + pix) * 4;
+    const uint32_t *src = obuf + ((t % SLOTS) * NPIX + pix) * WPP;
     const int oy = oy0 + pix / PW, ox = ox0 + pix % PW;
     if (oy >= OH || ox >= OW) continue;
     uint32_t *dst = a.s_out + ((((int64_t)t * a.B + b) * OH + oy) * OW + ox) * CW + cwb;
-    if (nw == 4 && (CW & 3) == 0) {
+    if (WPP == 4 && nw == 4 && (CW & 3) == 0) {
       *(v4i *)dst = *(const v4i *)src;
+    } else if (WPP == 3 && nw == 3) {
+      const uint32_t w0 = src[0], w1 = src[1], w2 = src[2];
+      dst[0] = w0; dst[1] = w1; dst[2] = w2;
     } else {
       for (int w = 0; w < nw; ++w) dst[w] = src[w];
     }
   }
 }
 
-template <bool POOL>
+template <bool POOL, int NW = 4>
 __device__ __forceinline__ void flush_out(const uint32_t *obuf, const ConvMfmaArgs &a,
                                           int t0, int n, int b, int y0, int x0, int tid) {
-  flush_ring<POOL, OutStage<POOL>::FL, 256>(obuf, a, t0, n, b, y0, x0, tid);
+  flush_ring<POOL, OutStage<POOL>::FL, 64 * NW, OutStage<POOL>::NPIX, NW>(obuf, a, t0, n, b, y0, x0, tid);
 }
 
 template <bool LOAD>
@@ -450,9 +462,13 @@
 int stream_device(hipStream_t st);
 
 template <typename K>
-static inline void launch_persistent(K kernel, ConvMfmaArgs a, unsigned gy, hipStream_t st,
-                                     size_t dyn_lds = 0, int threads = 256) {
+static inline int launch_persistent(K kernel, ConvMfmaArgs a, unsigned gy, hipStream_t st,
+                                    size_t dyn_lds = 0, int threads = 256, int min_occ = 0) {
   int dev = 0, cus = 256, occ = 2, slot = -1;
+  if (min_occ > 0) {
+    persistent_limits((const void *)kernel, threads, dyn_lds, stream_device(st), &cus, &occ);
+    if (occ < min_occ) return -1;
+  }
   a.sched = gy <= (unsigned)SCHED_Y ? sched_acquire(st, &dev, &slot) : nullptr;
   if (!a.sched) dev = stream_device(st);
   a.status = a.sched ? device_status_word(dev) : nullptr;
@@ -466,6 +482,7 @@
   }
   hipLaunchKernelGGL(kernel, dim3(gx, gy), dim3(threads), dyn_lds, st, a);
   if (a.sched) sched_release(dev, slot, st);
+  return occ;
 }
 
 enum { DQ_ARITH = 1, DQ_ONE = 2, DQ_TABLE = 3 };
diff --git a/snnquantprune_amd/linen.py b/snnquantprune_amd/linen.py
--- a/snnquantprune_amd/linen.py
+++ b/snnquantprune_amd/linen.py
@@ -110,6 +110,20 @@
 
 def conv_kpack() -> bool:
   return _CONV_KPACK
+
+
+_EVENT_WAVES = True
+
+
+def set_event_waves(enabled: bool):
+  global _EVENT_WAVES
+  from . import _lib
+  _lib.check(_lib.lib().snnqp_set_event_waves(1 if enabled else 0))
+  _EVENT_WAVES = bool(enabled)
+
+
+def event_waves() -> bool:
+  return _EVENT_WAVES
 
 
 def check_compute_dtype(dtype, who: str):
diff --git a/snnquantprune_amd/ops.py b/snnquantprune_amd/ops.py
--- a/snnquantprune_amd/ops.py
+++ b/snnquantprune_amd/ops.py
@@ -896,6 +896,8 @@
           _ptr(weight.wt), ctypes.byref(b) if b is not None else None, ctypes.byref(n),
           _ptr(u0), _ptr(u_out), _ptr(s), L.BITS if packed_out else L.F32, pool, impl,
           int(x_max), _ptr(x_seen), _ptr(x_flags), _stream()))
+  if _PROFILE is not None and geom.Cin == 2 and weight.is_int and in_type != L.BITS and impl != L.IMPL_GENERIC:
+    PROFILE_NOTES.setdefault(tag, {})["event_launch"] = event_launch_info()
   if fallback is not None:
     xf = _f32c(xt if fallback.x is None else fallback.x)
     pred = x_flags if fallback.pred is None else fallback.pred
@@ -906,6 +908,19 @@
         ctypes.byref(b) if b is not None else None, ctypes.byref(n), _ptr(u0), _ptr(u_out), _ptr(s),
         L.BITS if packed_out else L.F32, pool, _stream()))
   return u_out, (PackedSpikes(s, geom.Cout) if packed_out else s)
+
+
+def event_launch_info() -> dict:
+  info = (ctypes.c_int32 * 4)()
+  L.check(L.lib().snnqp_event_launch_info(info))
+  return {"waves": int(info[0]), "workgroups_per_cu": int(info[1]), "lds_bytes": int(info[2]),
+          "tchunk": int(info[3])}
+
+
+def event_layer_plan(T: int, pool: int, lut_rows: int, workgroups_per_cu: int) -> dict:
+  plan = (ctypes.c_int32 * 3)()
+  L.check(L.lib().snnqp_event_layer_plan(int(T), int(pool), int(lut_rows), int(workgroups_per_cu), plan))
+  return {"tchunk": int(plan[0]), "ring_bytes": int(plan[1]), "lds_bytes": int(plan[2])}
 
 
 def dense_lif_forward(x, weight: Weight, K: int, N: int, neuron: Neuron,
```

Result: slower. 92340 samples/s (median of 2 runs) (-2.2%).
